# defineZYP/ADT

Measured on AMD Instinct MI355X. Metric: train sequences/sec, SASRec-ADT ml-1m (seq_len=200, d=64, 2 blocks), higher is better.
Workload: dtype bf16; 1 GPU; SASRec-ADT ml-1m shape, 2 blocks d=64 H=2 seq_len=200, global batch 256 (256 sequences on this GPU), dropout 0.5, full train step (fwd+loss+bwd+clip+Adam), ids resident in HBM; global_batch=256, seq_len=200, parallelism=dp1, hip_graph=True, table_gradients=sorted segmented sums, bit-reproducible (ADT_ITEM_SORT=1), world_size=1

## Files before the change

adt_amd/csrc/adt_attn_args.h:

```cpp
#pragma once
#include "adt_common.cuh"

namespace adt {

struct AttnArgs {
  const float* Q; int ldq;
  const float* K; int ldk;
  const float* V; int ldv;
  float* O; int ldo;
  float* LSE;
  int B, H, L;
  int causal;
  float scale;
  DropCfg drop;
  uint32_t bh_offset;
  const float* dO; int lddo;
  float* dQ; int lddq;
  float* dK; int lddk;
  float* dV; int lddv;
  uint32_t* mask;
  unsigned long long* stamps;
  int in_bf16;
  int out_bf16;
};

}
```

adt_amd/csrc/adt_bwdchain_args.h:

```cpp
#pragma once
#include "adt_common.cuh"

namespace adt {

struct BwdChainArgs {
  int T, L, B;
  const int* ids;
  DropCfg drop; uint32_t site1, site2; uint32_t row_offset;
  float ln_eps;
  const float* gy;
  const float* u;
  const float* xin;
  const float* o;
  const float* dqkv; int lddqkv;
  const float* dkv2;
  int grad_bf16;
  const float* dh;
  const float* f;
  const float* W0; const float* W1; const float* W2; const float* W3;
  const float* gamma; const float* beta;
  float* out0; int acc0;
  float* out1; int acc1;
  float* dW0; float* dW1; float* dW2; float* dW3;
  float* db0; float* db1; float* db2; float* db3;
  float* dgamma; float* dbeta;
  const float* rec; const float* drec; const float* Ws; float* dWs; float* dbs; int H;
  int ablate;
  int nrep; size_t rep_stride;
  float gy_scale;
  float* part[4]; size_t part_stride;
  int saved_bf16;
  unsigned long long* stamps;
  const float* wp_base; const void* wp_img;
  float* vpart;
  const float* lnl_x; const float* lnl_gamma; float lnl_eps; float* vpart2; float* lnl_dgamma; float* lnl_dbeta;
  int nsplit;
};

}
```

adt_amd/csrc/adt_sasrec.hip:

```cpp
#include "adt_host.h"
#include <string.h>
#include <mutex>
#include "adt_bwdchain_args.h"
#include "adt_fwdchain_args.h"
#include "adt_seq_args.h"
#include "adt_seqbwd_args.h"

namespace {

constexpr float LN_EPS = 1e-8f;
constexpr int NREPP = 16;
constexpr int LN_PART_BLOCKS = 1024;
constexpr int NREP = 16;

struct Layout {
  int64_t off[4 + 30 * 16];
  int64_t total;
  int nl;
  int64_t item() const { return off[0]; }
  int64_t posw() const { return off[1]; }
  int64_t lnl_w() const { return off[2]; }
  int64_t lnl_b() const { return off[3]; }
  int64_t enc(int i, int k) const { return off[4 + 14 * i + k]; }
  int64_t dec(int i, int k) const { return off[4 + 14 * nl + 16 * i + k]; }
};
enum { E_LN1W, E_LN1B, E_INW, E_INB, E_OW, E_OB, E_LN2W, E_LN2B, E_C1W, E_C1B, E_C2W, E_C2B, E_SW, E_SB };
enum { D_LNW, D_LNB, D_SINW, D_SINB, D_SOW, D_SOB, D_EINW, D_EINB, D_EOW, D_EOB, D_C1W, D_C1B, D_C2W, D_C2B, D_UW, D_UB };

int64_t up64(int64_t x) { return (x + 63) / 64 * 64; }

StepPlan step_plan(const adt_sasrec_cfg* c, int B) {
  const StepFacts f{c->prec, c->maxlen, c->hidden, c->num_heads, c->num_layers, B, c->item_num + 1, adt_item_sort_supported(c->item_num + 1) != 0,
                    c->num_heads > 0 ? adt_seq_attn_bwd_lds(c->maxlen, c->num_heads) : 0};
  return adt_step_plan(f, adt_seq_switches());
}

bool make_layout(const adt_sasrec_cfg* c, Layout* lo) {
  if (c->num_layers < 1 || c->num_layers > 16) return false;
  const int64_t d = c->hidden, H = c->num_heads, hd = d / H, L = c->maxlen, V = c->item_num;
  lo->nl = c->num_layers;
  int64_t o = 0;
  int n = 0;
  auto put = [&](int64_t sz) { lo->off[n++] = o; o += up64(sz); };
  put((V + 1) * d); put(L * d); put(d); put(d);
  for (int i = 0; i < c->num_layers; ++i) {
    put(d); put(d); put(3 * d * d); put(3 * d); put(d * d); put(d); put(d); put(d);
    put(d * d); put(d); put(d * d); put(d); put(H * hd); put(H);
  }
  for (int i = 0; i < c->num_layers; ++i) {
    put(d); put(d);
    put(3 * d * d); put(3 * d); put(d * d); put(d);
    put(3 * d * d); put(3 * d); put(d * d); put(d);
    put(d * d); put(d); put(d * d); put(d); put(d); put(d);
  }
  lo->total = o;
  return true;
}

struct WS {
  int64_t T, d, H, L, nl, B;
  int64_t enc_x, dec_x, f, posl, negl;
  int64_t e_qn, e_qkv, e_o, e_lse, e_h, e_h2, e_u, e_rec, e_mask, e_stride;
  int64_t d_dn, d_qkv, d_o1, d_lse1, d_a1, d_q2, d_kv2, d_o2, d_lse2, d_a2, d_u, d_mask1, d_mask2, d_stride;
  int64_t g_enc_x, g_dec_x, g_f, g_pos, g_neg, g_rec;
  int64_t s1, s2, s3, s4, s5;
  int64_t loss, norms, scal;
  int64_t rep, rep_stride;
  int64_t prep, prep_stride;
  int64_t wpack;
  int64_t part, part_stride;
  int64_t isort, isort_n;
  int64_t vpart, vcall, lnpart, gnpart;
  int64_t total;
};

void make_ws(const adt_sasrec_cfg* c, int B, const StepPlan& pl, WS* w) {
  w->B = B; w->d = c->hidden; w->H = c->num_heads; w->L = c->maxlen; w->nl = c->num_layers;
  w->T = (int64_t)B * w->L;
  const int64_t Td = up64(w->T * w->d), T1 = up64(w->T), lse = up64((int64_t)B * w->H * w->L);
  const int64_t rec = up64(w->T * w->H * w->H);
  int64_t o = 0;
  auto take = [&](int64_t n) { int64_t r = o; o += n; return r; };
  w->enc_x = take((w->nl + 1) * Td); w->dec_x = take((w->nl + 1) * Td); w->f = take(Td);
  w->posl = take(T1); w->negl = take(T1);
  {
    const int64_t s = o;
    w->e_qn = take(Td); w->e_qkv = take(3 * Td); w->e_o = take(Td); w->e_lse = take(lse); w->e_h = take(Td);
    w->e_h2 = take(Td); w->e_u = take(Td); w->e_rec = take(rec); w->e_mask = take(8 * lse);
    w->e_stride = o - s;
    o = s + w->e_stride * w->nl;
  }
  {
    const int64_t s = o;
    w->d_dn = take(Td); w->d_qkv = take(3 * Td); w->d_o1 = take(Td); w->d_lse1 = take(lse); w->d_a1 = take(Td);
    w->d_q2 = take(Td); w->d_kv2 = take(2 * Td); w->d_o2 = take(Td); w->d_lse2 = take(lse); w->d_a2 = take(Td);
    w->d_u = take(Td); w->d_mask1 = take(8 * lse); w->d_mask2 = take(8 * lse);
    w->d_stride = o - s;
    o = s + w->d_stride * w->nl;
  }
  w->g_enc_x = take((w->nl + 1) * Td); w->g_dec_x = take((w->nl + 1) * Td); w->g_f = take(Td);
  w->g_pos = take(T1); w->g_neg = take(T1); w->g_rec = take(rec * w->nl);
  w->s1 = take(Td); w->s2 = take(Td); w->s3 = take(3 * Td); w->s4 = take(2 * Td); w->s5 = take(Td);
  w->loss = take(64 * (2 + 2 * 16)); w->norms = take(64); w->scal = take(192);
  w->rep_stride = up64((int64_t)(c->item_num + 1) * w->d);
  w->rep = take(NREP * w->rep_stride);
  {
    Layout lo;
    make_layout(c, &lo);
    w->prep_stride = up64(lo.total - lo.posw());
    w->prep = take(NREPP * w->prep_stride);
    w->wpack = take(3 * w->prep_stride);
  }
  w->part_stride = pl.parts_area ? (int64_t)w->nl * 16 * 4096 : 0;
  w->part = take((int64_t)B * pl.seq_split * w->part_stride);
  w->isort_n = pl.sort_area ? adt_item_sort_work_ints(4, (int)w->T, c->item_num + 1) : 0;
  w->isort = take(up64(w->isort_n));
  w->vcall = (int64_t)B * pl.seq_split * 512;
  w->vpart = take(w->part_stride > 0 ? (5 * w->nl + 1) * w->vcall : 0);
  w->lnpart = take(LN_PART_BLOCKS * 128);
  w->gnpart = take(4096);
  w->total = o;
}

#define CK(call) do { int _r = (call); if (_r) return _r; } while (0)

struct SideStream {
  hipStream_t s = nullptr;
  hipEvent_t fork_ev[4] = {nullptr, nullptr, nullptr, nullptr}, join_ev[4] = {nullptr, nullptr, nullptr, nullptr};
};
SideStream* side_stream(const StepPlan& pl, hipStream_t main) {
  static SideStream g[16];
  static std::mutex mu;
  if (!pl.side_sites) return nullptr;
  int dev = 0;
  if (hipGetDevice(&dev) != hipSuccess || dev < 0 || dev >= 16) return nullptr;
  SideStream* sd = &g[dev];
  std::lock_guard<std::mutex> lock(mu);
  if (sd->s) return sd;
  hipStreamCaptureStatus cs = hipStreamCaptureStatusNone;
  if (hipStreamIsCapturing(main, &cs) != hipSuccess || cs != hipStreamCaptureStatusNone) { (void)hipGetLastError(); return nullptr; }
  hipStream_t s = nullptr;
  if (hipStreamCreateWithFlags(&s, hipStreamNonBlocking) != hipSuccess) { (void)hipGetLastError(); return nullptr; }
  for (int i = 0; i < 4; ++i)
    if (hipEventCreateWithFlags(&sd->fork_ev[i], hipEventDisableTiming) != hipSuccess ||
        hipEventCreateWithFlags(&sd->join_ev[i], hipEventDisableTiming) != hipSuccess) {
      (void)hipGetLastError();
      (void)hipStreamDestroy(s);
      return nullptr;
    }
  sd->s = s;
  return sd;
}
int side_mark(SideStream* sd, int k, void* main) {
  if (!sd) return 0;
  if (hipEventRecord(sd->fork_ev[k], (hipStream_t)main) != hipSuccess) return adt_set_error("backward: side-stream fork %d failed", k);
  return 0;
}
int side_enter(SideStream* sd, int k, void* main, void** out) {
  *out = main;
  if (!sd) return 0;
  if (hipStreamWaitEvent(sd->s, sd->fork_ev[k], 0) != hipSuccess) return adt_set_error("backward: side-stream fork %d failed", k);
  *out = sd->s;
  return 0;
}
int side_join(SideStream* sd, int k, void* main) {
  if (!sd) return 0;
  if (hipEventRecord(sd->join_ev[k], sd->s) != hipSuccess || hipStreamWaitEvent((hipStream_t)main, sd->join_ev[k], 0) != hipSuccess)
    return adt_set_error("backward: side-stream join %d failed", k);
  return 0;
}

int layout_ws(const adt_sasrec_cfg* c, int B, Layout* lo, WS* w, StepPlan* pl) {
  *pl = step_plan(c, B);
  if (pl->cfg_error[0]) return adt_set_error("%s", pl->cfg_error);
  make_layout(c, lo);
  make_ws(c, B, *pl, w);
  return 0;
}

adt::FwdChainArgs fwd_args(int T, int L, int B, int H, const int32_t* ids, float p, const uint32_t* seed, uint32_t row_offset) {
  adt::FwdChainArgs a;
  memset(&a, 0, sizeof(a));
  a.T = T; a.L = L; a.B = B; a.H = H; a.ids = ids; a.drop = adt_make_drop(p, seed, 0); a.row_offset = row_offset; a.ln_eps = LN_EPS;
  return a;
}

adt::BwdChainArgs bwd_args(int T, int L, int B, const int32_t* ids, float p, const uint32_t* seed, uint32_t row_offset) {
  adt::BwdChainArgs a;
  memset(&a, 0, sizeof(a));
  a.T = T; a.L = L; a.B = B; a.ids = ids; a.drop = adt_make_drop(p, seed, 0); a.row_offset = row_offset; a.ln_eps = LN_EPS;
  return a;
}

int pack_offsets(const adt_sasrec_cfg* c, const Layout& lo, int* offs) {
  if (c->prec != ADT_PREC_BF16) return 0;
  int n = 0;
  const int64_t base = lo.posw();
  const int dd = c->hidden * c->hidden;
  for (int i = 0; i < c->num_layers; ++i) {
    for (int j = 0; j < 3; ++j) offs[n++] = (int)(lo.enc(i, E_INW) + j * dd - base);
    offs[n++] = (int)(lo.enc(i, E_OW) - base); offs[n++] = (int)(lo.enc(i, E_C1W) - base); offs[n++] = (int)(lo.enc(i, E_C2W) - base);
    for (int j = 0; j < 3; ++j) offs[n++] = (int)(lo.dec(i, D_SINW) + j * dd - base);
    for (int j = 0; j < 3; ++j) offs[n++] = (int)(lo.dec(i, D_EINW) + j * dd - base);
// ... 187 lines not shown
SideStream* fwd_logits_stream(const StepPlan& pl, void* st) { return ((pl.side_sites & 1) && !pl.bce_merged) ? side_stream(pl, (hipStream_t)st) : nullptr; }
bool ring_prefetch_split(const adt::RingPrefetchArgs& rr, bool bce_by_forward, const StepPlan& pl) {
  return rr.ring && rr.staging && rr.state && bce_by_forward && pl.embed3_on;
}

struct LossPtrs { const float *A[4], *Bm[4], *rc[4]; float *GA[4], *GB[4], *lm[4], *dr[4], *ln[4]; };
AdtLossSeedsJob loss_terms(const WS& w, float* ws, const float* lambdas1, const float* lambdas2, bool all_seeds, LossPtrs* q) {
  const int nl = (int)w.nl, H = (int)w.H;
  const int64_t Td = up64(w.T * w.d), rec = up64(w.T * w.H * w.H);
  float* loss = ws + w.loss;
  for (int i = 0; i < nl; ++i) {
    q->A[i] = ws + w.enc_x + i * Td; q->Bm[i] = ws + w.dec_x + (nl - i) * Td;
    q->GA[i] = all_seeds ? ws + w.g_enc_x + i * Td : nullptr;
    q->GB[i] = (all_seeds || i == 0) ? ws + w.g_dec_x + (nl - i) * Td : nullptr;
    q->lm[i] = loss + 64 * (2 + i);
    q->rc[i] = ws + i * w.e_stride + w.e_rec; q->dr[i] = ws + w.g_rec + i * rec; q->ln[i] = loss + 64 * (2 + nl + i);
  }
  AdtLossSeedsJob j{};
  j.T = (int)w.T; j.norms = ws + w.norms; j.loss_bce = loss;
  j.nmse = nl; j.A = q->A; j.Bm = q->Bm; j.n = w.T * w.d; j.lambdas = lambdas1; j.GA = q->GA; j.GB = q->GB; j.loss_mse = q->lm;
  j.nnll = H > 1 ? nl : 0; j.rec = q->rc; j.n_rows = (int)w.T; j.H = H; j.lambda2 = lambdas2[nl - 1]; j.drec = q->dr; j.loss_nll = q->ln;
  return j;
}

int forward_loss_lean(const adt_sasrec_cfg* c, const Layout& lo, const WS& w, const StepPlan& pl, const float* P, float* ws, const int32_t* seq, const int32_t* dec,
                      const int32_t* pos, const int32_t* neg, bool bce_side, float p, const uint32_t* seed, uint32_t b_offset, const float* lambdas1,
                      const float* lambdas2, const adt::RingPrefetchArgs& rr, void* st) {
  const int hd = (int)(w.d / w.H), nl = c->num_layers;
  if (!pl.bce_deferred) return 1;
  for (int i = 0; i < nl; ++i) {
    adt::SeqFwdArgs a = enc_layer_seq_args(c, lo, w, pl, P, ws, seq, p, seed, b_offset, i, true, true);
    if (i == nl - 1) { a.lnl_gamma = P + lo.lnl_w(); a.lnl_beta = P + lo.lnl_b(); a.f_out = ws + w.f; }
    CK(adt_launch_seq_enc_fwd(hd, a, st));
  }
  for (int j = 0; j < nl; ++j) CK(dec_layer_seq_fwd(lo, w, pl, P, ws, dec, p, seed, b_offset, j, st));
  LossPtrs q;
  AdtLossSeedsJob job = loss_terms(w, ws, lambdas1, lambdas2, false, &q);
  job.ring = &rr; job.split = ring_prefetch_split(rr, bce_side, pl);
  const adt::LogitsBceArgs lb{ws + w.f, P + lo.item(), pos, neg, ws + w.norms, (int)w.T, ws + w.posl, ws + w.negl, ws + w.g_pos, ws + w.g_neg, ws + w.loss,
                              ws + w.g_f, pl.det ? nullptr : ws + w.rep, NREP, (size_t)w.rep_stride, pl.embed3_on ? 1 : 0};
  const bool merged = bce_side && pl.bce_merged;
  if (merged) job.logits = &lb;
  SideStream* const sd = (bce_side && !merged) ? fwd_logits_stream(pl, st) : nullptr;
  if (bce_side && !merged) CK(side_mark(sd, 0, st));
  CK(adt_loss_seeds_prefetch(job, st));
  if (bce_side && !merged) {
    void* s2 = nullptr;
    CK(side_enter(sd, 0, st, &s2));
    CK(adt_logits_bce_scatter_ex(lb.F, lb.E, pos, neg, lb.norms, lb.T, lb.pos_logits, lb.neg_logits, lb.dpos, lb.dneg, lb.loss, lb.dF, lb.rep, lb.nrep,
                                 w.rep_stride, lb.neg_only, s2));
    if (sd && hipEventRecord(sd->join_ev[0], sd->s) != hipSuccess) return adt_set_error("forward_loss: logits event");
  }
  return 0;
}

int g_time_which = 0, g_time_layer = 0;
hipEvent_t g_time_ev0 = nullptr, g_time_ev1 = nullptr;
inline void time_mark(int which, int layer, bool start, void* st) {
  if (!g_time_ev0 || !g_time_ev1 || g_time_layer != layer) return;
  if (g_time_which == 3 && which == 1 && start) {
    (void)hipEventRecord(g_time_ev0, (hipStream_t)st);
    (void)hipEventRecord(g_time_ev1, (hipStream_t)st);
  } else if (g_time_which == which) {
    (void)hipEventRecord(start ? g_time_ev0 : g_time_ev1, (hipStream_t)st);
  }
}

const char* const NO_FALLBACK = "backward: shape L=%d hd=%d left the per-sequence kernels although the partial-gradient path was chosen";

struct Bwd {
  const adt_sasrec_cfg* c; Layout lo; WS w;
  const float* P; float* G; float* ws;
  const int32_t *seq, *dec, *pos, *neg;
  float p; const uint32_t* seed; uint32_t b_offset, ro;
  void* st;
  BwdPlan plan;
  StepPlan sp;
  BwdCallPlan call;
  adt::RingPrefetchArgs ring;
  int T, d, H, hd, L, prec, nl;
  int64_t Td, recsz;
  float* Gq;
  float *s1, *s3, *s4, *s5, *gf;
  const float* f;
  SideStream *sd, *sd_sort;

  adt::BwdChainArgs BA(const int32_t* ids, float pp, const uint32_t* sdp) const {
    adt::BwdChainArgs a = bwd_args(T, L, (int)w.B, ids, pp, sdp, ro);
    a.nrep = NREPP; a.rep_stride = (size_t)w.prep_stride;
    a.wp_base = P + lo.posw(); a.wp_img = prec == ADT_PREC_BF16 ? (const void*)(ws + w.wpack) : nullptr;
    a.nsplit = sp.seq_split;
    return a;
  }
  float* PART(int layer, int slot) const { return sp.parts ? ws + w.part + (int64_t)(16 * layer + slot) * 4096 : nullptr; }
  float* VPART(int layer, int k) const { return call.late_parts ? ws + w.vpart + (int64_t)(5 * layer + k) * w.vcall : nullptr; }
  int logits_scatter(void* s) const {
    if (plan.bce_here)
      return adt_logits_bce_scatter_ex(f, P + lo.item(), pos, neg, ws + w.norms, T, ws + w.posl, ws + w.negl, ws + w.g_pos, ws + w.g_neg, ws + w.loss,
                                       gf, sp.det ? nullptr : ws + w.rep, NREP, w.rep_stride, call.embed3 ? 1 : 0, s);
    if (sp.det) return adt_logits_bwd_df(P + lo.item(), pos, neg, ws + w.g_pos, ws + w.g_neg, T, d, gf, d, s);
    return adt_logits_bwd_scatter(f, d, P + lo.item(), pos, neg, ws + w.g_pos, ws + w.g_neg, T, d, gf, d, ws + w.rep, NREP, w.rep_stride, s);
  }
  int zero_unless_prezeroed(int64_t at, size_t n, void* s) const {
    return (!plan.prep_zeroed && adt::zero_f32_async(ws + at, n, (hipStream_t)s)) ? adt_set_error("replica zero") : 0;
  }
};

int bwd_init(Bwd& x, const adt_sasrec_cfg* c, const float* P, float* G, float* ws, const int32_t* seq, const int32_t* dec, const int32_t* pos,
             const int32_t* neg, int B, int training, const uint32_t* seed, uint32_t b_offset, int phase, const adt::RingPrefetchArgs& ring, void* st) {
  CK(layout_ws(c, B, &x.lo, &x.w, &x.sp));
  if (const char* err = adt_bwd_plan(phase, x.sp.bce_deferred, &x.plan)) return adt_set_error("%s", err);
  x.call = adt_bwd_call_plan(x.sp, x.plan);
  const WS& w = x.w;
  x.c = c; x.P = P; x.G = G; x.ws = ws; x.seq = seq; x.dec = dec; x.pos = pos; x.neg = neg; x.seed = seed; x.b_offset = b_offset; x.st = st; x.ring = ring;
  x.T = (int)w.T; x.d = (int)w.d; x.H = (int)w.H; x.hd = x.d / x.H; x.L = (int)w.L; x.prec = c->prec; x.nl = c->num_layers;
  x.Td = up64(w.T * w.d); x.recsz = up64(w.T * w.H * w.H);
  x.p = training ? c->dropout : 0.f;
  x.ro = b_offset * (uint32_t)x.L;
  x.s1 = ws + w.s1; x.s3 = ws + w.s3; x.s4 = ws + w.s4; x.s5 = ws + w.s5; x.gf = ws + w.g_f; x.f = ws + w.f;
  x.Gq = ws + w.prep - x.lo.posw();
  x.sd_sort = x.sp.det ? side_stream(x.sp, (hipStream_t)st) : nullptr;
  x.sd = x.call.side ? side_stream(x.sp, (hipStream_t)st) : nullptr;
  return 0;
}

struct LogitsSide {
  enum { DONE, MARKED, ENQUEUED, BY_FORWARD } at = DONE;

  int begin(const Bwd& x) {
    const WS& w = x.w;
    if (x.plan.bce_fwd) {
      at = BY_FORWARD;
    } else if (x.sp.det) {
      CK(x.zero_unless_prezeroed(w.prep, (size_t)NREPP * w.prep_stride, x.st));
      CK(x.logits_scatter(x.st));
    } else if (x.sd && (x.sp.side_sites & 1)) {
      CK(side_mark(x.sd, 0, x.st));
      CK(x.zero_unless_prezeroed(w.prep, (size_t)NREPP * w.prep_stride, x.st));
      at = MARKED;
    } else {
      CK(x.zero_unless_prezeroed(w.rep, (size_t)NREP * w.rep_stride + (size_t)NREPP * w.prep_stride, x.st));
      CK(x.logits_scatter(x.st));
    }
    return 0;
  }
  int after_first_chain_kernel(const Bwd& x) {
    if (at != MARKED) return 0;
    void* s2 = nullptr;
    CK(side_enter(x.sd, 0, x.st, &s2));
    CK(x.zero_unless_prezeroed(x.w.rep, (size_t)NREP * x.w.rep_stride, s2));
    CK(x.logits_scatter(s2));
    at = ENQUEUED;
    return 0;
  }
  int join(const Bwd& x) {
    if (at == ENQUEUED) CK(side_join(x.sd, 0, x.st));
    if (at == BY_FORWARD) {
      SideStream* const sl = fwd_logits_stream(x.sp, x.st);
      if (sl && hipStreamWaitEvent((hipStream_t)x.st, sl->join_ev[0], 0) != hipSuccess) return adt_set_error("backward: logits join");
    }
    at = DONE;
    return 0;
  }
};

int dec_post_bwd(const Bwd& x, int i) {
  const WS& w = x.w; const Layout& lo = x.lo; const float* P = x.P; float* const Gq = x.Gq;
  float* base = x.ws + i * w.d_stride;
  adt::BwdChainArgs a = x.BA(x.dec, x.p, x.seed);
  a.site1 = dec_site(i, 2); a.site2 = dec_site(i, 3);
  a.gy = x.ws + w.g_dec_x + (i + 1) * x.Td; a.u = base + w.d_u; a.xin = base + w.d_a2; a.o = base + w.d_o2; a.saved_bf16 = x.sp.lean;
  a.W0 = P + lo.dec(i, D_C2W); a.W1 = P + lo.dec(i, D_C1W); a.W2 = P + lo.dec(i, D_EOW);
  a.dW0 = Gq + lo.dec(i, D_C2W); a.dW1 = Gq + lo.dec(i, D_C1W); a.dW2 = Gq + lo.dec(i, D_EOW);
  a.db0 = Gq + lo.dec(i, D_C2B); a.db1 = Gq + lo.dec(i, D_C1B); a.db2 = Gq + lo.dec(i, D_EOB);
  a.out0 = x.s1;
  a.part[0] = x.PART(i, PS_D_C2); a.part[1] = x.PART(i, PS_D_C1); a.part[2] = x.PART(i, PS_D_EO); a.part_stride = (size_t)w.part_stride;
  a.vpart = x.VPART(i, 0);
  const int rc = x.sp.use_seq ? adt_launch_seq_post_bwd(x.hd, 0, a, x.st) : 1;
  if (rc < 0) return rc;
  if (rc && x.sp.parts) return adt_set_error(NO_FALLBACK, x.L, x.hd);
  return rc ? adt_launch_bwdchain(x.prec, 1, a, x.st) : 0;
}

int dec_cross_attn_bwd(const Bwd& x, int i) {
  const WS& w = x.w; const int d = x.d, B = (int)w.B;
  float* base = x.ws + i * w.d_stride;
  float *q2 = base + w.d_q2, *kv2 = base + w.d_kv2, *o2 = base + w.d_o2, *lse2 = base + w.d_lse2, *s4 = x.s4;
  const uint32_t* mask2 = reinterpret_cast<const uint32_t*>(base + w.d_mask2);
  if (!x.sp.lean)
    return adt_attn_bwd(x.prec, q2, d, kv2, 2 * d, kv2 + d, 2 * d, o2, d, lse2, x.s1, d, B, x.H, x.L, x.hd, 1, x.p, x.seed, dec_site(i, 1), x.b_offset,
                        x.s5, d, s4, 2 * d, s4 + d, 2 * d, mask2, x.st);
  const uint16_t* kvb = reinterpret_cast<const uint16_t*>(kv2);
  return adt_attn_bwd_saved_bf16(q2, d, kvb, 2 * d, kvb + d, 2 * d, o2, d, lse2, x.s1, d, B, x.H, x.L, x.hd, x.p, x.seed, dec_site(i, 1), x.b_offset,
                                 x.s5, d, s4, 2 * d, x.sp.parts ? s4 + d / 2 : s4 + d, 2 * d, mask2, x.sp.parts ? 1 : 0, x.st);
}

adt::BwdChainArgs dec_mid_seq_args(const Bwd& x, int i) {
  const WS& w = x.w; const Layout& lo = x.lo; const float* P = x.P; float* const Gq = x.Gq;
  const int d = x.d, dd = d * d;
  float* base = x.ws + i * w.d_stride;
  const float* einw = P + lo.dec(i, D_EINW);
  float* geinw = Gq + lo.dec(i, D_EINW);
  float* geinb = Gq + lo.dec(i, D_EINB);
  adt::BwdChainArgs a = x.BA(x.dec, 0.f, nullptr);
  a.dqkv = x.s5; a.lddqkv = d; a.xin = base + w.d_a1; a.o = base + w.d_o1; a.saved_bf16 = x.sp.lean; a.dkv2 = x.s4; a.f = x.f;
  a.grad_bf16 = (x.sp.lean && x.sp.parts) ? 1 : 0;
  a.W0 = einw; a.W1 = P + lo.dec(i, D_SOW); a.W2 = einw + dd; a.W3 = einw + 2 * dd;
  a.dW0 = geinw; a.dW1 = Gq + lo.dec(i, D_SOW); a.dW2 = geinw + dd; a.dW3 = geinw + 2 * dd;
  a.db0 = geinb; a.db1 = Gq + lo.dec(i, D_SOB); a.db2 = geinb + d; a.db3 = geinb + 2 * d;
  a.out0 = x.s1; a.out1 = x.gf; a.acc1 = 1;
  a.part[0] = x.PART(i, PS_D_EIN); a.part[1] = x.PART(i, PS_D_SO); a.part[2] = x.PART(i, PS_D_EIN + 1); a.part[3] = x.PART(i, PS_D_EIN + 2);
  a.part_stride = (size_t)w.part_stride;
  a.vpart = x.VPART(i, 1);
  return a;
}

adt::AttnArgs dec_cross_attn_lean_args(const Bwd& x, int i) {
  const WS& w = x.w; const int d = x.d;
  float* base = x.ws + i * w.d_stride;
  const uint16_t* kvb = reinterpret_cast<const uint16_t*>(base + w.d_kv2);
  return adt_attn_bwd_saved_bf16_args(base + w.d_q2, d, kvb, 2 * d, kvb + d, 2 * d, base + w.d_o2, d, base + w.d_lse2, x.s1, d, (int)w.B, x.H, x.L, x.hd, x.p,
                                      x.seed, dec_site(i, 1), x.b_offset, x.s5, d, x.s4, 2 * d, x.s4 + d / 2, 2 * d,
                                      reinterpret_cast<const uint32_t*>(base + w.d_mask2), 1);
}

int dec_mid_bwd(const Bwd& x, int i) {
  const WS& w = x.w; const Layout& lo = x.lo; const float* P = x.P; float* const Gq = x.Gq;
  const int d = x.d, dd = d * d;
  float* base = x.ws + i * w.d_stride;
  float *o1 = base + w.d_o1, *a1 = base + w.d_a1;
  const float* einw = P + lo.dec(i, D_EINW);
  float* geinw = Gq + lo.dec(i, D_EINW);
  float* geinb = Gq + lo.dec(i, D_EINB);
  if (x.sp.use_seq) {
    const int rc = adt_launch_seq_mid_bwd(x.hd, dec_mid_seq_args(x, i), x.st);
    if (rc <= 0) return rc;
    if (x.sp.parts) return adt_set_error(NO_FALLBACK, x.L, x.hd);
  }
  {
    adt::BwdChainArgs a = x.BA(x.dec, 0.f, nullptr);
    a.dqkv = x.s5; a.lddqkv = d; a.xin = a1; a.o = o1; a.saved_bf16 = x.sp.lean;
    a.W0 = einw; a.W1 = P + lo.dec(i, D_SOW);
    a.dW0 = geinw; a.dW1 = Gq + lo.dec(i, D_SOW); a.db0 = geinb; a.db1 = Gq + lo.dec(i, D_SOB);
    a.out0 = x.s1;
    CK(adt_launch_bwdchain(x.prec, 4, a, x.st));
  }
  adt::BwdChainArgs a = x.BA(x.dec, 0.f, nullptr);
  a.dkv2 = x.s4; a.f = x.f;
  a.W0 = einw + dd; a.W1 = einw + 2 * dd;
  a.dW0 = geinw + dd; a.dW1 = geinw + 2 * dd; a.db0 = geinb + d; a.db1 = geinb + 2 * d;
  a.out0 = x.gf; a.acc0 = 1;
  return adt_launch_bwdchain(x.prec, 5, a, x.st);
}

int attn_block_bwd(const Bwd& x, int i, bool dec) {
  const WS& w = x.w; const Layout& lo = x.lo; const float* P = x.P; float* const Gq = x.Gq; float* const ws = x.ws;
  const int d = x.d, dd = d * d, nl = x.nl;
  const int32_t* ids = dec ? x.dec : x.seq;
  float* gy = ws + (dec ? w.g_dec_x : w.g_enc_x) + (i + 1) * x.Td;
  float* gx = ws + (dec ? w.g_dec_x : w.g_enc_x) + i * x.Td;
  const float* xi = ws + (dec ? w.dec_x : w.enc_x) + i * x.Td;
  float* base = ws + i * (dec ? w.d_stride : w.e_stride);
  float *qkv = base + (dec ? w.d_qkv : w.e_qkv), *o = base + (dec ? w.d_o1 : w.e_o), *lse = base + (dec ? w.d_lse1 : w.e_lse);
  const uint32_t* mask = reinterpret_cast<const uint32_t*>(base + (dec ? w.d_mask1 : w.e_mask));
  const int64_t lnw = dec ? lo.dec(i, D_LNW) : lo.enc(i, E_LN1W), lnb = dec ? lo.dec(i, D_LNB) : lo.enc(i, E_LN1B);
  const int64_t inw = dec ? lo.dec(i, D_SINW) : lo.enc(i, E_INW), inb = dec ? lo.dec(i, D_SINB) : lo.enc(i, E_INB);
  const uint32_t site = dec ? dec_site(i, 0) : enc_site(i, 0);
  const int acc = dec ? (i > 0 ? 1 : 0) : 1;
  if (x.sp.use_seq) {
    adt::SeqBwdArgs a = seq_bwd_args(x.L, (int)w.B, x.H, ids, x.p, x.seed, site, x.b_offset, x.hd);
    a.x = xi; a.gamma = P + lnw; a.beta = P + lnb; a.Win = P + inw; a.bin = P + inb;
    a.dO = x.s1; a.o = o; a.lse = lse; a.mask = mask; a.dres = dec ? gy : x.s5;
    a.gx = gx; a.acc = acc; a.dWin = Gq + inw; a.dbin = Gq + inb; a.dgamma = Gq + lnw; a.dbeta = Gq + lnb;
    if (x.plan.seeds_virtual && dec && i > 0) {
      a.acc = 0; a.seed_other = ws + w.enc_x + (nl - i) * x.Td; a.seed_coef = ws + w.norms + 8 + (nl - i);
    }
    if (x.plan.seeds_virtual && !dec) {
      a.acc = 0; a.seed_other = ws + w.dec_x + (nl - i) * x.Td; a.seed_coef = ws + w.norms + 8 + i;
      if (i > 0) { a.seed_loss = ws + w.loss + 64 * (2 + i); a.seed_norms = ws + w.norms; }
    }
    a.nrep = NREPP; a.rep_stride = (size_t)w.prep_stride; a.wp_base = P + lo.posw(); a.wp_img = ws + w.wpack; a.saved_bf16 = x.sp.lean;
    a.part = x.PART(i, dec ? PS_D_SIN : PS_E_IN); a.part_stride = (size_t)w.part_stride;
    a.vpart = x.VPART(i, dec ? 2 : 4);
    a.nsplit = a.part ? x.sp.attn_split : 1;
    time_mark(dec ? 2 : 1, i, true, x.st);
    const int rc = adt_launch_seq_attn_pre_bwd(x.hd, dec ? 1 : 0, a, x.st);
    time_mark(dec ? 2 : 1, i, false, x.st);
    if (rc <= 0) return rc;
    if (x.sp.lean) return adt_set_error("backward: the lean forward needs the fused attention-block backward (L=%d hd=%d)", x.L, x.hd);
  }
  CK(adt_attn_bwd(x.prec, qkv, 3 * d, qkv + d, 3 * d, qkv + 2 * d, 3 * d, o, d, lse, x.s1, d, (int)w.B, x.H, x.L, x.hd, 1, x.p, x.seed, site, x.b_offset,
                  x.s3, 3 * d, x.s3 + d, 3 * d, x.s3 + 2 * d, 3 * d, mask, x.st));
  adt::BwdChainArgs a = x.BA(ids, 0.f, nullptr);
  a.dqkv = x.s3; a.lddqkv = 3 * d; a.xin = xi;
  if (dec) a.gy = gy; else a.dh = x.s5;
  a.W0 = P + inw; a.W1 = P + inw + dd; a.W2 = P + inw + 2 * dd; a.gamma = P + lnw; a.beta = P + lnb;
  a.dW0 = Gq + inw; a.dW1 = Gq + inw + dd; a.dW2 = Gq + inw + 2 * dd; a.db0 = Gq + inb; a.db1 = Gq + inb + d; a.db2 = Gq + inb + 2 * d;
  a.dgamma = Gq + lnw; a.dbeta = Gq + lnb;
  a.out0 = gx; a.acc0 = acc;
  return adt_launch_bwdchain(x.prec, dec ? 3 : 2, a, x.st);
}

int dec_block_backward(const Bwd& x, int i, LogitsSide& logits) {
  CK(dec_post_bwd(x, i));
  CK(logits.after_first_chain_kernel(x));
  if (x.sp.use_seq && x.sp.lean && x.sp.parts) {
    const adt::AttnArgs at = dec_cross_attn_lean_args(x, i);
    const adt::BwdChainArgs mid = dec_mid_seq_args(x, i);
    if (adt_seq_xattn_mid_covered(x.hd, at, mid)) {
      CK(logits.join(x));
      const int rc = adt_launch_seq_xattn_mid_bwd(x.hd, at, mid, x.st);
      if (rc) return rc < 0 ? rc : adt_set_error("backward: the fused cross-attention + mid launch refused a shape it covers (L=%d hd=%d)", x.L, x.hd);
      return attn_block_bwd(x, i, true);
    }
  }
  CK(dec_cross_attn_bwd(x, i));
  CK(logits.join(x));
  CK(dec_mid_bwd(x, i));
  return attn_block_bwd(x, i, true);
}

struct DecSide {
  enum { NONE, MARKED, ENQUEUED } at = NONE;
  bool parts_done = false;

  int embed(const Bwd& x, void* s) const {
    const WS& w = x.w;
    return adt_embed_bwd_rep(x.dec, x.ws + w.g_dec_x, x.T, x.L, x.d, x.p, x.seed, SITE_EMB_DEC, x.ro, x.G + x.lo.posw(), x.ws + w.rep, NREP, w.rep_stride, s);
  }
  int begin(const Bwd& x) {
    const WS& w = x.w; const Layout& lo = x.lo;
    const int64_t dec_begin = lo.dec(0, 0);
    if (x.plan.phase == 0 && x.sd && (x.sp.side_sites & 2) && !(x.call.embed3 && (x.call.late_parts || !x.sp.parts))) {
      CK(side_mark(x.sd, 1, x.st));
      at = MARKED;
    } else if (x.plan.phase == 0) {
      if (!x.sp.det && !x.call.embed3) CK(embed(x, x.st));
    } else if (x.sp.det) {
      if (x.sp.parts) CK(reduce_partials(x.c, lo, w, x.sp, x.G, x.ws, false, true, x.st));
      CK(adt_replica_reduce(x.G + dec_begin, x.Gq + dec_begin, lo.total - dec_begin, NREPP, w.prep_stride, x.st));
    } else {
      void* s2 = nullptr;
      CK(side_mark(x.sd, 1, x.st));
      if (!x.call.embed3) CK(embed(x, x.st));
      CK(side_enter(x.sd, 1, x.st, &s2));
      if (x.sp.parts) CK(reduce_partials(x.c, lo, w, x.sp, x.G, x.ws, false, true, s2));
      CK(side_join(x.sd, 1, x.st));
      CK(adt_replica_reduce2(x.G + lo.item(), x.ws + w.rep, (int64_t)(x.c->item_num + 1) * x.d, NREP, w.rep_stride, x.G + dec_begin, x.Gq + dec_begin,
                             lo.total - dec_begin, NREPP, w.prep_stride, x.st));
    }
    return 0;
  }
  int enter(const Bwd& x) {
    if (at != MARKED) return 0;
    void* s2 = nullptr;
    CK(side_enter(x.sd, 1, x.st, &s2));
    if (!x.sp.det && !x.call.embed3) CK(embed(x, s2));
    if (x.sp.parts && !x.call.late_parts) { CK(reduce_partials(x.c, x.lo, x.w, x.sp, x.G, x.ws, false, true, s2)); parts_done = true; }
    at = ENQUEUED;
    return 0;
  }
  int join(const Bwd& x, bool covered) {
    if (at == ENQUEUED && !covered) CK(side_join(x.sd, 1, x.st));
    at = NONE;
    return 0;
  }
};

int last_layernorm_bwd(const Bwd& x) {
  const WS& w = x.w; const Layout& lo = x.lo; float* const ws = x.ws;
  const int d = x.d;
  if (x.sp.lnl_fused) return 0;
  if (x.call.late_parts) {
    const int nb = adt_layernorm_bwd_parts(x.gf, d, ws + w.enc_x + x.nl * x.Td, d, x.P + lo.lnl_w(), LN_EPS, x.T, d, ws + w.g_enc_x + x.nl * x.Td, d, 0,
                                           ws + w.lnpart, LN_PART_BLOCKS, x.st);
    return nb < 0 ? nb : 0;
  }
  return adt_layernorm_bwd_rep(x.gf, d, ws + w.enc_x + x.nl * x.Td, d, x.P + lo.lnl_w(), LN_EPS, x.T, d, ws + w.g_enc_x + x.nl * x.Td, d, 0,
                               x.Gq + lo.lnl_w(), x.Gq + lo.lnl_b(), NREPP, w.prep_stride, x.st);
}

int enc_post_bwd(const Bwd& x, int i) {
  const WS& w = x.w; const Layout& lo = x.lo; const float* P = x.P; float* const Gq = x.Gq; float* const ws = x.ws;
  const int H = x.H, nl = x.nl;
  float* base = ws + i * w.e_stride;
  adt::BwdChainArgs a = x.BA(x.seq, x.p, x.seed);
  a.site1 = enc_site(i, 1); a.site2 = enc_site(i, 2);
  a.gy = ws + w.g_enc_x + (i + 1) * x.Td; a.u = base + w.e_u; a.xin = base + w.e_h; a.o = base + w.e_o; a.saved_bf16 = x.sp.lean;
  a.W0 = P + lo.enc(i, E_C2W); a.W1 = P + lo.enc(i, E_C1W); a.W2 = P + lo.enc(i, E_OW);
  a.gamma = P + lo.enc(i, E_LN2W); a.beta = P + lo.enc(i, E_LN2B);
  a.dW0 = Gq + lo.enc(i, E_C2W); a.dW1 = Gq + lo.enc(i, E_C1W); a.dW2 = Gq + lo.enc(i, E_OW);
  a.db0 = Gq + lo.enc(i, E_C2B); a.db1 = Gq + lo.enc(i, E_C1B); a.db2 = Gq + lo.enc(i, E_OB);
  a.dgamma = Gq + lo.enc(i, E_LN2W); a.dbeta = Gq + lo.enc(i, E_LN2B);
  a.out0 = x.s5; a.out1 = x.s1;
  int which = 0;
  if (H > 1 && H <= 4) {
    which = H <= 2 ? 6 : 7;
    a.rec = base + w.e_rec; a.drec = ws + w.g_rec + i * x.recsz; a.Ws = P + lo.enc(i, E_SW); a.dWs = Gq + lo.enc(i, E_SW);
    a.dbs = Gq + lo.enc(i, E_SB); a.H = H;
  }
  a.part[0] = x.PART(i, PS_E_C2); a.part[1] = x.PART(i, PS_E_C1); a.part[2] = x.PART(i, PS_E_O); a.part_stride = (size_t)w.part_stride;
  a.vpart = x.VPART(i, 3);
  if (x.sp.lnl_fused && i == nl - 1) {
    a.gy = x.gf; a.lnl_x = ws + w.enc_x + nl * x.Td; a.lnl_gamma = P + lo.lnl_w(); a.lnl_eps = LN_EPS;
    a.vpart2 = x.call.late_parts ? ws + w.vpart + (int64_t)(5 * nl) * w.vcall : nullptr;
    a.lnl_dgamma = Gq + lo.lnl_w(); a.lnl_dbeta = Gq + lo.lnl_b();
  }
  const int rc = x.sp.use_seq ? adt_launch_seq_post_bwd(x.hd, 1, a, x.st) : 1;
  if (rc < 0) return rc;
  if (rc && x.sp.parts) return adt_set_error(NO_FALLBACK, x.L, x.hd);
  return rc ? adt_launch_bwdchain(x.prec, which, a, x.st) : 0;
}

int enc_block_backward(const Bwd& x, int i, DecSide& dec_side) {
  const WS& w = x.w; const Layout& lo = x.lo;
  CK(enc_post_bwd(x, i));
  if (x.sp.lnl_fused && i == x.nl - 1) CK(dec_side.enter(x));
  if (x.H > 4) {
    float* base = x.ws + i * w.e_stride;
    CK(adt_headcls_bwd(base + w.e_o, x.d, x.P + lo.enc(i, E_SW), base + w.e_rec, x.ws + w.g_rec + i * x.recsz, (int)w.B, x.L, x.H, x.hd, x.s1, x.d,
                       x.G + lo.enc(i, E_SW), x.G + lo.enc(i, E_SB), x.st));
  }
  return attn_block_bwd(x, i, false);
}

int table_gradients(const Bwd& x, DecSide& dec_side) {
  const WS& w = x.w; const Layout& lo = x.lo; float* const ws = x.ws; float* const G = x.G;
  const int phase = x.plan.phase;
  if (phase == 2 && !x.sp.det && adt::zero_f32_async(ws + w.rep, (size_t)NREP * w.rep_stride, (hipStream_t)x.st)) return adt_set_error("replica zero");
  SideStream* const sd2 = ((x.sp.side_sites & 4) && x.sp.parts && !x.call.late_parts) ? x.sd : nullptr;
  CK(dec_side.join(x, sd2 != nullptr));
  void* s2 = nullptr;
  CK(side_mark(sd2, 2, x.st));
  if (x.sp.det) {
    if (x.sd_sort && hipStreamWaitEvent((hipStream_t)x.st, x.sd_sort->join_ev[3], 0) != hipSuccess) return adt_set_error("backward: sort join");
    const uint32_t site4[4] = {SITE_EMB_SEQ, SITE_EMB_DEC, 0u, 0u};
    const int32_t* const ids2[2] = {x.seq, x.dec};
    const float* const dx2[2] = {ws + w.g_enc_x, ws + w.g_dec_x};
    CK(adt_item_segsum_posemb(reinterpret_cast<int32_t*>(ws + w.isort), 4, x.T, x.c->item_num + 1, 0xFu, site4, x.p, x.seed, sqrtf((float)x.d), G + lo.item(),
                              x.plan.prep_zeroed ? 0 : 1, ids2, dx2, site4, 2, (int)w.B, x.L, x.ro, G + lo.posw(), x.st));
  } else if (x.call.embed3) {
    const bool by_forward = phase == 2 ? x.plan.seeds_virtual : x.plan.bce_fwd;
    CK(adt_embed_bwd3_prefetch(x.seq, x.dec, x.pos, ws + w.g_enc_x, ws + w.g_dec_x, x.f, ws + w.g_pos, x.T, x.L, x.p, x.seed, SITE_EMB_SEQ, SITE_EMB_DEC, x.ro,
                               G + lo.posw(), ws + w.rep, NREP, w.rep_stride, ring_prefetch_split(x.ring, by_forward, x.sp) ? &x.ring : nullptr, x.st));
  } else {
    CK(adt_embed_bwd_rep(x.seq, ws + w.g_enc_x, x.T, x.L, x.d, x.p, x.seed, SITE_EMB_SEQ, x.ro, G + lo.posw(), ws + w.rep, NREP, w.rep_stride, x.st));
  }
  CK(side_enter(sd2, 2, x.st, &s2));
  if (x.sp.parts && !x.call.late_parts) CK(reduce_partials(x.c, lo, w, x.sp, G, ws, true, phase == 0 && !dec_side.parts_done, s2));
  CK(side_join(sd2, 2, x.st));
  if (x.plan.defer_fold) return 0;
  return adt_replica_reduce2(G + lo.item(), ws + w.rep, (int64_t)(x.c->item_num + 1) * x.d, x.sp.det ? 0 : NREP, w.rep_stride, G + lo.posw(), x.Gq + lo.posw(),
                             (phase == 0 ? lo.total : lo.dec(0, 0)) - lo.posw(), NREPP, w.prep_stride, x.st);
}

int item_sort_begin(const Bwd& x) {
  const WS& w = x.w; float* const ws = x.ws;
  const int32_t* const ids4[4] = {x.seq, x.dec, x.pos, x.neg};
  const float* const rows4[4] = {ws + w.g_enc_x, ws + w.g_dec_x, x.f, x.f};
  const float* const coef4[4] = {nullptr, nullptr, ws + w.g_pos, ws + w.g_neg};
  const int kind4[4] = {0, 0, 1, 1};
  void* s2 = x.st;
  if (x.sd_sort) { CK(side_mark(x.sd_sort, 3, x.st)); CK(side_enter(x.sd_sort, 3, x.st, &s2)); }
  CK(adt_item_sort(ids4, 4, x.T, x.c->item_num + 1, rows4, coef4, kind4, x.ro, reinterpret_cast<int32_t*>(ws + w.isort), s2));
  if (x.sd_sort && hipEventRecord(x.sd_sort->join_ev[3], x.sd_sort->s) != hipSuccess) return adt_set_error("backward: sort event");
  return 0;
}

int decoder_phase(const Bwd& x, DecSide& dec_side) {
  if (x.w.prep != x.w.rep + NREP * x.w.rep_stride) return adt_set_error("workspace layout: replica areas not adjacent");
  if (x.sp.det) CK(item_sort_begin(x));
  LogitsSide logits;
  CK(logits.begin(x));
  for (int i = x.nl - 1; i >= 0; --i) CK(dec_block_backward(x, i, logits));
  return dec_side.begin(x);
}

int encoder_phase(const Bwd& x, DecSide& dec_side) {
  CK(last_layernorm_bwd(x));
  if (!x.sp.lnl_fused) CK(dec_side.enter(x));
  for (int i = x.nl - 1; i >= 0; --i) CK(enc_block_backward(x, i, dec_side));
  return table_gradients(x, dec_side);
}

}
// ... 442 lines not shown
```

adt_amd/csrc/adt_seq.hip:

```cpp
#include "adt_host.h"
#include <limits.h>
#include <atomic>
#include "adt_seqfwd.cuh"
#include "adt_seqfwd_tt.cuh"
#include "adt_seqattn.cuh"
#include "adt_seqbwd_tt.cuh"
#include "adt_seqpost_tt.cuh"
#include "adt_seqxattn_tt.cuh"

using namespace adt;

template <class Args>
static int seq_launch(const void* fn, size_t smem, AdtLdsOptIn& slot, int grid, const Args* args, hipStream_t s, const char* what, int nwaves = SQ_NW,
                      size_t optin = 0) {
  return adt_launch_lds1(fn, dim3(grid), dim3(nwaves * 64), smem, *args, s, what, slot, optin);
}

__global__ __launch_bounds__(256) void k_pack_wimg(PackArgs a) { pack_wimg_block(a, blockIdx.x); }

extern "C" int adt_pack_wimg(const float* base, void* img, const int* offs, int n, void* stream) {
  if (n < 1 || n > 256) return adt_set_error("pack_wimg: %d blocks", n);
  PackArgs a;
  a.base = base; a.img = reinterpret_cast<__bf16*>(img); a.n = n;
  for (int i = 0; i < n; ++i) a.off[i] = offs[i];
  hipLaunchKernelGGL(k_pack_wimg, dim3(n), dim3(256), 0, (hipStream_t)stream, a);
  return adt_check_launch("pack_wimg");
}

static_assert(ADT_SEQ_MAXLEN == SQ_LP && ADT_SEQ_MAXLEN == SB_R, "adt_step_plan.h restates the image rows of these kernels");

const SeqSwitches& adt_seq_switches() {
  static const SeqSwitches sw = [] {
    SeqSwitches s;
    s.seq = adt_env_on("ADT_SEQ"); s.seq_lean = adt_env_on("ADT_SEQ_LEAN"); s.seq_tt = adt_env_on("ADT_SEQ_TT"); s.seq_bwd = adt_env_on("ADT_SEQ_BWD");
    s.seq_attn_bwd = adt_env_on("ADT_SEQ_ATTN_BWD"); s.seq_post_bwd = adt_env_on("ADT_SEQ_POST_BWD"); s.seq_partials = adt_env_on("ADT_SEQ_PARTIALS");
    s.xattn_fused = adt_env_on("ADT_XATTN_FUSED");
    s.seq_ablate = adt_env_int("ADT_SEQ_ABLATE", 0); s.seq_ablate_set = adt_env_int("ADT_SEQ_ABLATE", INT_MIN) != INT_MIN;
    s.seq_split = adt_env_int("ADT_SEQ_SPLIT", 0); s.attn_split = adt_env_on("ADT_ATTN_SPLIT");
    s.side_stream = adt_env_int("ADT_SIDE_STREAM", 7); s.side_stream_dp = adt_env_int("ADT_SIDE_STREAM_DP", 0) != 0;
    s.item_sort = adt_env_int("ADT_ITEM_SORT", 0) != 0;
    s.lnl_fused = adt_env_on("ADT_LNL_FUSED"); s.fold_parts = adt_env_on("ADT_FOLD_PARTS"); s.fwd_fused = adt_env_on("ADT_FWD_FUSED");
    s.embed3 = adt_env_on("ADT_EMBED3"); s.bce_merged = adt_env_on("ADT_BCE_MERGED");
    return s;
  }();
  return sw;
}

static SeqAttnFacts attn_facts(const AttnArgs& a) {
  return {a.L, a.H, a.B, a.causal != 0, a.in_bf16 != 0, a.out_bf16 != 0, a.ldq, a.ldk, a.ldv, a.ldo, a.lddo, a.drop.thr != 0, a.mask != nullptr,
          sab_lds_bytes(a.L, a.H), xm_lds_bytes(a.L, a.H)};
}
size_t adt_seq_attn_bwd_lds(int L, int H) { return sab_lds_bytes(L, H); }
static SeqChainFacts chain_facts(const BwdChainArgs& a) {
  return {a.L, a.H, a.B, a.T, a.wp_img != nullptr, a.saved_bf16 != 0, a.grad_bf16 != 0, a.part[0] && a.part[1] && a.part[2] && a.part[3], a.nsplit, a.ablate,
          a.drec != nullptr};
}

static unsigned long long* g_stamps = nullptr;

extern "C" int adt_seq_stamps_read(unsigned long long* out, int n) {
  if (!g_stamps) return -1;
  if (hipDeviceSynchronize() != hipSuccess) return -2;
  return hipMemcpy(out, g_stamps, (size_t)n * sizeof(unsigned long long), hipMemcpyDeviceToHost) == hipSuccess ? 0 : -3;
}

static int seq_stamps_mode() {
  static const int st = [] {
    const int v = adt_env_int("ADT_SEQ_STAMPS", 0);
    return (v && hipMalloc(&g_stamps, 16 * 16 * sizeof(unsigned long long)) != hipSuccess) ? 0 : v;
  }();
  return st;
}
static unsigned long long* seq_stamp_buffer(bool for_attention) { return seq_stamps_mode() == (for_attention ? 2 : 1) ? g_stamps : nullptr; }
static unsigned long long* seq_stamp_buffer_post() { return seq_stamps_mode() == 3 ? g_stamps : nullptr; }
static unsigned long long* seq_stamp_buffer_mode(int mode) { return seq_stamps_mode() == mode ? g_stamps : nullptr; }

static void seq_ablate(SeqFwdArgs& a) {
  a.stamps = seq_stamp_buffer(false);
  const int ab = adt_seq_switches().seq_ablate;
  a.ablate = ab;
  if (ab & 1) { a.qkv = nullptr; a.o = nullptr; a.h = nullptr; a.u = nullptr; a.a1 = nullptr; a.q2 = nullptr; a.kv2 = nullptr; a.o2 = nullptr; a.mask = nullptr; a.mask2 = nullptr; }
}

static bool seq_use_tt(const SeqFwdArgs& a) {
  return adt_seq_fwd_tt(adt_seq_switches(), a.wp_img != nullptr, a.L);
}

int adt_launch_seq_enc_fwd(int hd, const SeqFwdArgs& a, void* stream) {
  static AdtLdsOptIn optin[3], optin_tt[3];
  SeqFwdArgs args = a;
  seq_ablate(args);
  hipStream_t s = (hipStream_t)stream;
  if (seq_use_tt(args)) {
    const int nsp = args.nsplit > 1 ? args.nsplit : 1;
    const size_t smem_tt = SeqTtLds<6>::bytes;
    if (hd == 64) return seq_launch((const void*)k_seqtt_enc_fwd<64>, smem_tt, optin_tt[0], a.B * nsp, &args, s, "seqtt_enc_fwd<64>", TQ_FWD_NW);
    if (hd == 32) return seq_launch((const void*)k_seqtt_enc_fwd<32>, smem_tt, optin_tt[1], a.B * nsp, &args, s, "seqtt_enc_fwd<32>", TQ_FWD_NW);
    if (hd == 16) return seq_launch((const void*)k_seqtt_enc_fwd<16>, smem_tt, optin_tt[2], a.B * nsp, &args, s, "seqtt_enc_fwd<16>", TQ_FWD_NW);
  }
  args.nsplit = 0;
  const size_t smem = SeqFwdLds<6>::bytes;
  if (hd == 64) return seq_launch((const void*)k_seq_enc_fwd<64, 2>, smem, optin[0], a.B, &args, s, "seq_enc_fwd<64>");
  if (hd == 32) return seq_launch((const void*)k_seq_enc_fwd<32, 2>, smem, optin[1], a.B, &args, s, "seq_enc_fwd<32>");
  if (hd == 16) return seq_launch((const void*)k_seq_enc_fwd<16, 4>, smem, optin[2], a.B, &args, s, "seq_enc_fwd<16>");
  return adt_set_error("seq_enc_fwd: head size %d", hd);
}

int adt_launch_seq_dec_fwd(int hd, const SeqFwdArgs& a, void* stream) {
  static AdtLdsOptIn optin[3], optin_tt[3];
  SeqFwdArgs args = a;
  seq_ablate(args);
  hipStream_t s = (hipStream_t)stream;
  if (seq_use_tt(args)) {
    const int nsp = args.nsplit > 1 ? args.nsplit : 1;
    const size_t smem_tt = SeqTtLds<5>::bytes;
    if (hd == 64) return seq_launch((const void*)k_seqtt_dec_fwd<64>, smem_tt, optin_tt[0], a.B * nsp, &args, s, "seqtt_dec_fwd<64>", TQ_FWD_NW);
    if (hd == 32) return seq_launch((const void*)k_seqtt_dec_fwd<32>, smem_tt, optin_tt[1], a.B * nsp, &args, s, "seqtt_dec_fwd<32>", TQ_FWD_NW);
    if (hd == 16) return seq_launch((const void*)k_seqtt_dec_fwd<16>, smem_tt, optin_tt[2], a.B * nsp, &args, s, "seqtt_dec_fwd<16>", TQ_FWD_NW);
  }
  args.nsplit = 0;
  const size_t smem = SeqFwdLds<5>::bytes;
  if (hd == 64) return seq_launch((const void*)k_seq_dec_fwd<64>, smem, optin[0], a.B, &args, s, "seq_dec_fwd<64>");
  if (hd == 32) return seq_launch((const void*)k_seq_dec_fwd<32>, smem, optin[1], a.B, &args, s, "seq_dec_fwd<32>");
  if (hd == 16) return seq_launch((const void*)k_seq_dec_fwd<16>, smem, optin[2], a.B, &args, s, "seq_dec_fwd<16>");
  return adt_set_error("seq_dec_fwd: head size %d", hd);
}

int adt_launch_seq_attn_bwd(int hd, const AttnArgs& a, void* stream) {
  if (!adt_covers_attn_bwd(adt_seq_switches(), hd, attn_facts(a))) return 1;
  const size_t smem = sab_lds_bytes(a.L, a.H);
  const int mode = a.drop.thr == 0 ? 0 : (a.mask != nullptr ? 1 : 2);
  static AdtLdsOptIn optin[9];
  const void* fns[9] = {(const void*)k_seq_attn_bwd<64, 0>, (const void*)k_seq_attn_bwd<64, 1>, (const void*)k_seq_attn_bwd<64, 2>,
                        (const void*)k_seq_attn_bwd<32, 0>, (const void*)k_seq_attn_bwd<32, 1>, (const void*)k_seq_attn_bwd<32, 2>,
                        (const void*)k_seq_attn_bwd<16, 0>, (const void*)k_seq_attn_bwd<16, 1>, (const void*)k_seq_attn_bwd<16, 2>};
  const int slot = (hd == 64 ? 0 : hd == 32 ? 3 : 6) + mode;
  AttnArgs args = a;
  args.stamps = seq_stamp_buffer(true);
  if (!args.stamps) args.stamps = seq_stamp_buffer_mode(4);
  return adt_launch_lds1(fns[slot], dim3(a.B), dim3(SAB_NW * 64), smem, args, (hipStream_t)stream, "seq_attn_bwd", optin[slot], ADT_LDS_MAX);
}

template <int HD, bool DEC>
static int seq_attn_pre_bwd_t(int mode, const SeqBwdArgs& a, hipStream_t s) {
  constexpr int H = 64 / HD;
  const size_t smem = SeqBwdLds<H>::bytes;
  static AdtLdsOptIn optin[3];
  const void* fns[3] = {(const void*)k_seqtt_attn_pre_bwd<HD, 0, DEC>, (const void*)k_seqtt_attn_pre_bwd<HD, 1, DEC>,
                        (const void*)k_seqtt_attn_pre_bwd<HD, 2, DEC>};
  SeqBwdArgs args = a;
  args.stamps = seq_stamp_buffer(true);
  if (a.nsplit == 2 && !a.part) return adt_set_error("seqtt_attn_pre_bwd: two workgroups per sequence need the weight-gradient partials");
  if (a.nsplit != 2) args.nsplit = 1;
  return seq_launch(fns[mode], smem, optin[mode], a.B * args.nsplit, &args, s, "seqtt_attn_pre_bwd");
}

int adt_launch_seq_attn_pre_bwd(int hd, int dec, const SeqBwdArgs& a, void* stream) {
  SeqChainFacts f{};
  f.L = a.L; f.H = a.H; f.B = a.B; f.T = a.B * a.L; f.wimg = a.wp_img != nullptr;
  if (!adt_covers_attn_pre_bwd(adt_seq_switches(), hd, f)) return 1;
  const int mode = a.drop.thr == 0 ? 0 : (a.mask != nullptr ? 1 : 2);
  hipStream_t s = (hipStream_t)stream;
  if (hd == 32) return dec ? seq_attn_pre_bwd_t<32, true>(mode, a, s) : seq_attn_pre_bwd_t<32, false>(mode, a, s);
  if (hd == 64) return dec ? seq_attn_pre_bwd_t<64, true>(mode, a, s) : seq_attn_pre_bwd_t<64, false>(mode, a, s);
  return dec ? seq_attn_pre_bwd_t<16, true>(mode, a, s) : seq_attn_pre_bwd_t<16, false>(mode, a, s);
}

int adt_launch_seq_post_bwd(int hd, int enc, const BwdChainArgs& a, void* stream) {
  if (!adt_covers_post_bwd(adt_seq_switches(), hd, enc != 0, chain_facts(a))) return 1;
  static AdtLdsOptIn optin[6];
  const void* fns[6] = {(const void*)k_seqtt_post_bwd<64, false>, (const void*)k_seqtt_post_bwd<64, true>, (const void*)k_seqtt_post_bwd<32, false>,
                        (const void*)k_seqtt_post_bwd<32, true>, (const void*)k_seqtt_post_bwd<16, false>, (const void*)k_seqtt_post_bwd<16, true>};
  const int slot = (hd == 64 ? 0 : hd == 32 ? 2 : 4) + (enc ? 1 : 0);
  BwdChainArgs args = a;
  args.stamps = enc ? seq_stamp_buffer_post() : nullptr;
  return seq_launch(fns[slot], SeqPostLds<3>::bytes, optin[slot], a.B * (a.nsplit > 1 ? a.nsplit : 1), &args, (hipStream_t)stream, "seqtt_post_bwd", SP_NW);
}

int adt_launch_seq_mid_bwd(int hd, const BwdChainArgs& a, void* stream) {
  if (!adt_covers_mid_bwd(adt_seq_switches(), hd, chain_facts(a))) return 1;
  static AdtLdsOptIn optin;
  BwdChainArgs args = a;
  args.stamps = seq_stamp_buffer_mode(5);
  return seq_launch((const void*)k_seqtt_mid_bwd, SeqPostLds<4>::bytes, optin, a.B * (a.nsplit > 1 ? a.nsplit : 1), &args, (hipStream_t)stream, "seqtt_mid_bwd", SP_MID_NW);
}

static std::atomic<unsigned long long> g_xattn_fused_launches{0};
extern "C" unsigned long long adt_seq_xattn_fused_launches() { return g_xattn_fused_launches.load(); }

int adt_seq_xattn_mid_covered(int hd, const AttnArgs& at, const BwdChainArgs& ch) {
  const bool handover = ch.dqkv == at.dQ && ch.lddqkv == at.lddq && at.lddq == 64 && ch.dkv2 == at.dK && at.lddk == 128 && at.lddv == 128 &&
                        reinterpret_cast<const __bf16*>(at.dV) == reinterpret_cast<const __bf16*>(at.dK) + 64;
  return adt_covers_xattn_mid(adt_seq_switches(), hd, attn_facts(at), chain_facts(ch), handover);
}

int adt_launch_seq_xattn_mid_bwd(int hd, const AttnArgs& at, const BwdChainArgs& ch, void* stream) {
  if (!adt_seq_xattn_mid_covered(hd, at, ch)) return 1;
  XattnMidArgs a{};
  a.Q = reinterpret_cast<const __bf16*>(at.Q); a.K = reinterpret_cast<const __bf16*>(at.K); a.V = reinterpret_cast<const __bf16*>(at.V);
  a.O = reinterpret_cast<const __bf16*>(at.O); a.ldq = at.ldq; a.ldk = at.ldk; a.ldv = at.ldv; a.ldo = at.ldo;
  a.LSE = at.LSE; a.dO = at.dO; a.lddo = at.lddo; a.L = at.L; a.mask = at.mask; a.scale = at.scale; a.drop = at.drop;
  a.xin = ch.xin; a.o = ch.o; a.f = ch.f; a.wp_base = ch.wp_base; a.wp_img = ch.wp_img;
  a.W0 = ch.W0; a.W1 = ch.W1; a.W2 = ch.W2; a.W3 = ch.W3;
  a.out0 = ch.out0; a.out1 = ch.out1; a.acc1 = ch.acc1; a.nrep = ch.nrep; a.rep_stride = ch.rep_stride;
  a.db0 = ch.db0; a.db1 = ch.db1; a.db2 = ch.db2; a.db3 = ch.db3; a.vpart = ch.vpart;
  for (int k = 0; k < 4; ++k) a.part[k] = ch.part[k];
  a.part_stride = ch.part_stride;
  a.stamps = seq_stamp_buffer_mode(6);
  const int mode = at.drop.thr == 0 ? 0 : 1;
  static AdtLdsOptIn optin[6];
  const void* fns[6] = {(const void*)k_seqtt_xattn_mid_bwd<64, 0>, (const void*)k_seqtt_xattn_mid_bwd<64, 1>, (const void*)k_seqtt_xattn_mid_bwd<32, 0>,
                        (const void*)k_seqtt_xattn_mid_bwd<32, 1>, (const void*)k_seqtt_xattn_mid_bwd<16, 0>, (const void*)k_seqtt_xattn_mid_bwd<16, 1>};
  const int slot = (hd == 64 ? 0 : hd == 32 ? 2 : 4) + mode;
  const size_t most = xm_lds_bytes(ADT_SEQ_MAXLEN, at.H) <= ADT_LDS_MAX ? xm_lds_bytes(ADT_SEQ_MAXLEN, at.H) : xm_lds_bytes(128, at.H);
  const int rc = seq_launch(fns[slot], xm_lds_bytes(at.L, at.H), optin[slot], at.B, &a, (hipStream_t)stream, "seqtt_xattn_mid_bwd", XM_NW, most);
  if (rc == 0) ++g_xattn_fused_launches;
  return rc;
}

struct PartReduceArgs {
  float* G; const float* part; size_t stride; int nwg; int nslots;
  int slot[256]; int off[256];
  int nwg_slot[256];
};
constexpr int PR_SPLIT = 4;
__global__ __launch_bounds__(256) void k_dwpart_reduce(PartReduceArgs a) {
  typedef unsigned u4v __attribute__((ext_vector_type(4)));
  const int j = blockIdx.x, item = threadIdx.x;
  const int nwg = a.nwg_slot[j];
  const int per = (nwg + PR_SPLIT - 1) / PR_SPLIT, w0 = blockIdx.y * per, w1 = min(nwg, w0 + per);
  const __bf16* p = reinterpret_cast<const __bf16*>(a.part + (size_t)a.slot[j] * 4096) + item * 16;
  const size_t strideb = a.stride * 2;
  float sum[16];
#pragma unroll
  for (int i = 0; i < 16; ++i) sum[i] = 0.f;
  int wg = w0;
  for (; wg + 4 <= w1; wg += 4) {
    u4v lo[4], hi[4];
#pragma unroll
    for (int u = 0; u < 4; ++u) {
      const u4v* src = reinterpret_cast<const u4v*>(p + (size_t)(wg + u) * strideb);
      lo[u] = src[0]; hi[u] = src[1];
    }
#pragma unroll
    for (int u = 0; u < 4; ++u) {
      const unsigned wds[8] = {lo[u].x, lo[u].y, lo[u].z, lo[u].w, hi[u].x, hi[u].y, hi[u].z, hi[u].w};
#pragma unroll
      for (int i = 0; i < 8; ++i) { sum[2 * i] += __uint_as_float(wds[i] << 16); sum[2 * i + 1] += __uint_as_float(wds[i] & 0xFFFF0000u); }
    }
  }
  for (; wg < w1; ++wg) {
    const u4v* src = reinterpret_cast<const u4v*>(p + (size_t)wg * strideb);
    const u4v lo = src[0], hi = src[1];
    const unsigned wds[8] = {lo.x, lo.y, lo.z, lo.w, hi.x, hi.y, hi.z, hi.w};
#pragma unroll
    for (int i = 0; i < 8; ++i) { sum[2 * i] += __uint_as_float(wds[i] << 16); sum[2 * i + 1] += __uint_as_float(wds[i] & 0xFFFF0000u); }
  }
  const int tile = item >> 4, lane0 = (item & 15) * 4;
#pragma unroll
  for (int r = 0; r < 4; ++r) {
    float* dst = a.G + a.off[j] + (16 * (tile >> 2) + 4 * (lane0 >> 4) + r) * 64 + 16 * (tile & 3) + (lane0 & 15);
#pragma unroll
    for (int k = 0; k < 4; ++k) atomicAdd(dst + k, sum[4 * k + r]);
  }
}

int adt_dwpart_reduce(float* G, const float* part, size_t stride, int nwg, const int* slots, const int* offs, int nslots, void* stream) {
  return adt_dwpart_reduce_n(G, part, stride, nwg, nullptr, slots, offs, nslots, stream);
}
int adt_dwpart_reduce_n(float* G, const float* part, size_t stride, int nwg, const int* nwg_slot, const int* slots, const int* offs, int nslots, void* stream) {
  if (nslots < 1 || nslots > 256) return adt_set_error("dwpart_reduce: %d slots", nslots);
  PartReduceArgs a;
  a.G = G; a.part = part; a.stride = stride; a.nwg = nwg; a.nslots = nslots;
  for (int i = 0; i < nslots; ++i) { a.slot[i] = slots[i]; a.off[i] = offs[i]; a.nwg_slot[i] = nwg_slot ? nwg_slot[i] : nwg; }
  hipLaunchKernelGGL(k_dwpart_reduce, dim3(nslots, PR_SPLIT), dim3(256), 0, (hipStream_t)stream, a);
  return adt_check_launch("dwpart_reduce");
}
```

adt_amd/csrc/adt_seqattn.cuh:

```cuda
#pragma once
#include "adt_attn.cuh"
#include "adt_tt.cuh"

namespace adt {

constexpr int SAB_NW = 16;
ADT_DEVICE_INLINE int sab_rank16(int w) {
  const int cl = w & 3, k = w >> 2;
  return 4 * k + ((k & 1) ? 3 - cl : cl);
}

__host__ __device__ inline int sab_rows(int L) { return (L + 31) / 32 * 32; }
__host__ __device__ inline size_t sab_lds_bytes(int L, int H) {
  const size_t R = (size_t)((L + 31) / 32 * 32);
  return 4 * R * TT_RS * 2 + (size_t)H * R * 8 * 4 + 2 * (size_t)H * R * 4;
}

template <int HD>
ADT_DEVICE_INLINE bf16x8 sab_rowfrag(const __bf16* img, int row, int h, int kb, int g) {
  const __bf16* p = img + row * TT_RS + h * HD + 32 * kb + 4 * g;
  const bf16x4 lo = *reinterpret_cast<const bf16x4*>(p);
  bf16x4 hi;
  if constexpr (HD == 16) {
#pragma unroll
// ... 113 lines not shown
  const bf16x8 fp = tt_pack(pv[0], pv[1]), fds = tt_pack(ds[0], ds[1]);
#pragma unroll
  for (int nt = 0; nt < NT; ++nt) {
    dv[nt] = mfma_bf16(dv[nt], tt_trfrag(sdO, qp * 32, h * HD + nt * 16, c, g), fp);
    dk[nt] = mfma_bf16(dk[nt], tt_trfrag(sQ, qp * 32, h * HD + nt * 16, c, g), fds);
  }
}

template <int HD, int MODE>
ADT_DEVICE_INLINE void sab_pass_b(const __bf16* sQ, const __bf16* sdO, const bf16x8* fk, const bf16x8* fv, const float* lse_h, const float* del_h,
                                  const uint32_t* sM_h, int kt, int nqt, int h, const DropCfg& drop, uint32_t key_rng, uint32_t idx_bh, int L,
                                  int c, int g, f32x4 (&dk)[HD / 16], f32x4 (&dv)[HD / 16]) {
  constexpr int NT = HD / 16;
#pragma unroll
  for (int nt = 0; nt < NT; ++nt) {
    dk[nt] = f32x4{0.f, 0.f, 0.f, 0.f};
    dv[nt] = f32x4{0.f, 0.f, 0.f, 0.f};
  }
  const int q0 = kt >> 1;
  sab_pair_b<HD, MODE, true>(sQ, sdO, fk, fv, lse_h, del_h, sM_h, q0, kt, h, drop, key_rng, idx_bh, L, c, g, dk, dv);
#pragma unroll 2
  for (int qp = q0 + 1; 2 * qp < nqt; ++qp) sab_pair_b<HD, MODE, false>(sQ, sdO, fk, fv, lse_h, del_h, sM_h, qp, kt, h, drop, key_rng, idx_bh, L, c, g, dk, dv);
}

template <int HD, int MODE>
ADT_DEVICE_INLINE void sab_pass_b_heads(const __bf16* sQ, const __bf16* sdO, const bf16x8* fk, const bf16x8* fv, const float* sLse, const float* sDelta,
                                        const uint32_t* sM, int R, int kt, int nqt, const DropCfg& drop, uint32_t key_rng, uint32_t bh0, int L,
                                        int c, int g, f32x4 (&dk)[64 / 16], f32x4 (&dv)[64 / 16]) {
  constexpr int H = 64 / HD, NT = HD / 16, KB = (HD + 31) / 32;
#pragma unroll
  for (int i = 0; i < 4; ++i) {
    dk[i] = f32x4{0.f, 0.f, 0.f, 0.f};
    dv[i] = f32x4{0.f, 0.f, 0.f, 0.f};
  }
  const int q0 = kt >> 1;
#pragma unroll
  for (int h = 0; h < H; ++h)
    sab_pair_b<HD, MODE, true>(sQ, sdO, fk + h * KB, fv + h * KB, sLse + h * R, sDelta + h * R, sM + (size_t)h * R * 8, q0, kt, h, drop, key_rng,
                               (bh0 + (uint32_t)h) * (uint32_t)L, L, c, g, *reinterpret_cast<f32x4 (*)[NT]>(&dk[h * NT]), *reinterpret_cast<f32x4 (*)[NT]>(&dv[h * NT]));
#pragma unroll 1
  for (int qp = q0 + 1; 2 * qp < nqt; ++qp) {
#pragma unroll
    for (int h = 0; h < H; ++h)
      sab_pair_b<HD, MODE, false>(sQ, sdO, fk + h * KB, fv + h * KB, sLse + h * R, sDelta + h * R, sM + (size_t)h * R * 8, qp, kt, h, drop, key_rng,
                                  (bh0 + (uint32_t)h) * (uint32_t)L, L, c, g, *reinterpret_cast<f32x4 (*)[NT]>(&dk[h * NT]), *reinterpret_cast<f32x4 (*)[NT]>(&dv[h * NT]));
  }
}

template <int HD, int MODE>
__global__ __launch_bounds__(SAB_NW * 64) void k_seq_attn_bwd(AttnArgs a) {
  adt_prefetch_kernargs<(sizeof(AttnArgs) + 63) / 64 * 64 <= 512 ? sizeof(AttnArgs) : 512>();
  constexpr int H = 64 / HD, NT = HD / 16, KB = (HD + 31) / 32, MAXKT = 14, NW = SAB_NW;
  extern __shared__ __attribute__((aligned(16))) unsigned char smem_raw[];
  const int L = a.L, R = sab_rows(L);
  __bf16* sQ = reinterpret_cast<__bf16*>(smem_raw);
  __bf16* sK = sQ + R * TT_RS;
  __bf16* sV = sK + R * TT_RS;
  __bf16* sdO = sV + R * TT_RS;
  uint32_t* sM = reinterpret_cast<uint32_t*>(sdO + R * TT_RS);
  float* sLse = reinterpret_cast<float*>(sM + (size_t)H * R * 8);
  float* sDelta = sLse + H * R;
  const int b = blockIdx.x;
  const int lane = threadIdx.x & 63, w = threadIdx.x >> 6, c = lane & 15, g = lane >> 4;
  const size_t row_b = (size_t)b * L;
  constexpr bool use_bits = MODE == 1;
  const float qmul = a.scale * 1.4426950408889634f;
#define SAB_STAMP(k) do { if (a.stamps && blockIdx.x == 0 && lane == 0) a.stamps[w * 16 + (k)] = __builtin_amdgcn_s_memtime(); } while (0)
  SAB_STAMP(0);
  if constexpr (MODE == 1) {
    for (int i = threadIdx.x; i < H * R * 2; i += NW * 64) {
      const int hr = i >> 1, h = hr / R, r = hr - h * R;
      uint4 v = make_uint4(0u, 0u, 0u, 0u);
      if (r < L) v = reinterpret_cast<const uint4*>(a.mask + ((size_t)(b * H + h) * L + r) * 8)[i & 1];
      reinterpret_cast<uint4*>(sM + (size_t)hr * 8)[i & 1] = v;
    }
  }
  for (int i = threadIdx.x; i < H * R; i += NW * 64) {
    const int h = i / R, r = i - h * R;
    sLse[i] = r < L ? a.LSE[(size_t)(b * H + h) * L + r] * 1.4426950408889634f : INFINITY;
  }
  for (int i = threadIdx.x; i < R * 8; i += NW * 64) {
    const int r = i >> 3, c8 = (i & 7) * 8;
    float q[8], k[8], v[8], d[8], o[8];
#pragma unroll
    for (int j = 0; j < 8; ++j) q[j] = k[j] = v[j] = d[j] = o[j] = 0.f;
    if (r < L && a.in_bf16) {
      const __bf16* Qb = reinterpret_cast<const __bf16*>(a.Q); const __bf16* Kb = reinterpret_cast<const __bf16*>(a.K);
      const __bf16* Vb = reinterpret_cast<const __bf16*>(a.V); const __bf16* Ob = reinterpret_cast<const __bf16*>(a.O);
      const int pa = 16 * ((c8 >> 2) & 3) + 4 * (c8 >> 4), pb = pa + 16;
      typedef __bf16 bf16x4_t __attribute__((ext_vector_type(4)));
      const bf16x4_t qa = *reinterpret_cast<const bf16x4_t*>(Qb + (row_b + r) * a.ldq + pa), qc = *reinterpret_cast<const bf16x4_t*>(Qb + (row_b + r) * a.ldq + pb);
      const bf16x4_t ka = *reinterpret_cast<const bf16x4_t*>(Kb + (row_b + r) * a.ldk + pa), kc = *reinterpret_cast<const bf16x4_t*>(Kb + (row_b + r) * a.ldk + pb);
      const bf16x4_t va = *reinterpret_cast<const bf16x4_t*>(Vb + (row_b + r) * a.ldv + pa), vc = *reinterpret_cast<const bf16x4_t*>(Vb + (row_b + r) * a.ldv + pb);
      const bf16x4_t oa = *reinterpret_cast<const bf16x4_t*>(Ob + (row_b + r) * a.ldo + pa), oc = *reinterpret_cast<const bf16x4_t*>(Ob + (row_b + r) * a.ldo + pb);
      bf16x8 qb, kb, vb, ob;
#pragma unroll
      for (int j = 0; j < 4; ++j) { qb[j] = qa[j]; qb[4 + j] = qc[j]; kb[j] = ka[j]; kb[4 + j] = kc[j]; vb[j] = va[j]; vb[4 + j] = vc[j]; ob[j] = oa[j]; ob[4 + j] = oc[j]; }
      *reinterpret_cast<float4*>(d) = *reinterpret_cast<const float4*>(a.dO + (row_b + r) * a.lddo + c8);
      *reinterpret_cast<float4*>(d + 4) = *reinterpret_cast<const float4*>(a.dO + (row_b + r) * a.lddo + c8 + 4);
#pragma unroll
      for (int j = 0; j < 8; ++j) { q[j] = (float)qb[j]; k[j] = (float)kb[j]; v[j] = (float)vb[j]; o[j] = (float)ob[j]; }
    } else if (r < L) {
      *reinterpret_cast<float4*>(q) = *reinterpret_cast<const float4*>(a.Q + (row_b + r) * a.ldq + c8);
      *reinterpret_cast<float4*>(q + 4) = *reinterpret_cast<const float4*>(a.Q + (row_b + r) * a.ldq + c8 + 4);
      *reinterpret_cast<float4*>(k) = *reinterpret_cast<const float4*>(a.K + (row_b + r) * a.ldk + c8);
      *reinterpret_cast<float4*>(k + 4) = *reinterpret_cast<const float4*>(a.K + (row_b + r) * a.ldk + c8 + 4);
      *reinterpret_cast<float4*>(v) = *reinterpret_cast<const float4*>(a.V + (row_b + r) * a.ldv + c8);
      *reinterpret_cast<float4*>(v + 4) = *reinterpret_cast<const float4*>(a.V + (row_b + r) * a.ldv + c8 + 4);
      *reinterpret_cast<float4*>(d) = *reinterpret_cast<const float4*>(a.dO + (row_b + r) * a.lddo + c8);
      *reinterpret_cast<float4*>(d + 4) = *reinterpret_cast<const float4*>(a.dO + (row_b + r) * a.lddo + c8 + 4);
      *reinterpret_cast<float4*>(o) = *reinterpret_cast<const float4*>(a.O + (row_b + r) * a.ldo + c8);
      *reinterpret_cast<float4*>(o + 4) = *reinterpret_cast<const float4*>(a.O + (row_b + r) * a.ldo + c8 + 4);
    }
    float part = 0.f;
#pragma unroll
    for (int j = 0; j < 8; ++j) { part += d[j] * o[j]; q[j] *= qmul; d[j] *= a.drop.scale; }
    *reinterpret_cast<bf16x8*>(sQ + r * TT_RS + c8) = pack8(q);
    *reinterpret_cast<bf16x8*>(sK + r * TT_RS + c8) = pack8(k);
    *reinterpret_cast<bf16x8*>(sV + r * TT_RS + c8) = pack8(v);
    *reinterpret_cast<bf16x8*>(sdO + r * TT_RS + c8) = pack8(d);
#pragma unroll
    for (int off = HD / 16; off > 0; off >>= 1) part += __shfl_xor(part, off, 64);
    if (((i & 7) % (HD / 8)) == 0) sDelta[((i & 7) / (HD / 8)) * R + r] = part;
  }
  SAB_STAMP(1);
  __syncthreads();
  SAB_STAMP(2);
  const uint32_t key_rng = drop_key(a.drop);
  const int nqt = (L + 15) / 16;
  const float ln2 = 0.6931471805599453f;

  for (int rnd = 0; rnd * NW < nqt; ++rnd) {
    const int tix = rnd * NW + sab_rank16(w);
    if (tix >= nqt) continue;
    const int qt = nqt - 1 - tix;
    const int q = qt * 16 + c;
    const int nkt = qt + 1;
#pragma unroll 1
    for (int h = 0; h < H; ++h) {
      const float lse_q = sLse[h * R + q], delta_q = sDelta[h * R + q];
      bf16x8 fq[KB], fdo[KB];
#pragma unroll
      for (int kb = 0; kb < KB; ++kb) {
        fq[kb] = sab_rowfrag<HD>(sQ, q, h, kb, g);
        fdo[kb] = sab_rowfrag<HD>(sdO, q, h, kb, g);
      }
      f32x4 dq[NT];
      const uint32_t bh_rng = (uint32_t)(b * H + h) + a.bh_offset;
      const uint32_t idx_q = (bh_rng * (uint32_t)L + (uint32_t)q) * (uint32_t)L;
      sab_pass_a<HD, MODE>(sK, sV, fq, fdo, lse_q, delta_q, sM + ((size_t)h * R + q) * 8, qt, h, a.drop, key_rng, idx_q, c, g, dq);
      if (q < L && a.out_bf16) {
        __bf16* dst = reinterpret_cast<__bf16*>(a.dQ) + (row_b + q) * a.lddq + 16 * g + 4 * h * NT;
#pragma unroll
        for (int nt = 0; nt < NT; ++nt) {
          bf16x4 v;
#pragma unroll
          for (int r = 0; r < 4; ++r) v[r] = (__bf16)(dq[nt][r] * a.scale);
          *reinterpret_cast<bf16x4*>(dst + 4 * nt) = v;
        }
      } else if (q < L) {
#pragma unroll
        for (int nt = 0; nt < NT; ++nt)
          *reinterpret_cast<float4*>(a.dQ + (row_b + q) * a.lddq + h * HD + nt * 16 + 4 * g) =
              make_float4(dq[nt][0] * a.scale, dq[nt][1] * a.scale, dq[nt][2] * a.scale, dq[nt][3] * a.scale);
      }
    }
  }

  SAB_STAMP(3);
  for (int rnd = 0; rnd * NW < nqt; ++rnd) {
    const int kt = rnd * NW + sab_rank16(w);
    if (kt >= nqt) continue;
    const int key = kt * 16 + c;
#pragma unroll 1
    for (int h = 0; h < H; ++h) {
      bf16x8 fk[KB], fv[KB];
#pragma unroll
      for (int kb = 0; kb < KB; ++kb) {
        fk[kb] = sab_rowfrag<HD>(sK, key, h, kb, g);
        fv[kb] = sab_rowfrag<HD>(sV, key, h, kb, g);
      }
      f32x4 dk[NT], dv[NT];
      const uint32_t bh_rng = (uint32_t)(b * H + h) + a.bh_offset;
      sab_pass_b<HD, MODE>(sQ, sdO, fk, fv, sLse + h * R, sDelta + h * R, sM + (size_t)h * R * 8, kt, nqt, h, a.drop, key_rng, bh_rng * (uint32_t)L, L, c,
                           g, dk, dv);
      if (key < L && a.out_bf16) {
        __bf16* dstk = reinterpret_cast<__bf16*>(a.dK) + (row_b + key) * a.lddk + 16 * g + 4 * h * NT;
        __bf16* dstv = reinterpret_cast<__bf16*>(a.dV) + (row_b + key) * a.lddv + 16 * g + 4 * h * NT;
#pragma unroll
        for (int nt = 0; nt < NT; ++nt) {
          bf16x4 vk, vv;
#pragma unroll
          for (int r = 0; r < 4; ++r) { vk[r] = (__bf16)(dk[nt][r] * ln2); vv[r] = (__bf16)dv[nt][r]; }
          *reinterpret_cast<bf16x4*>(dstk + 4 * nt) = vk;
          *reinterpret_cast<bf16x4*>(dstv + 4 * nt) = vv;
        }
      } else if (key < L) {
#pragma unroll
        for (int nt = 0; nt < NT; ++nt) {
          *reinterpret_cast<float4*>(a.dK + (row_b + key) * a.lddk + h * HD + nt * 16 + 4 * g) =
              make_float4(dk[nt][0] * ln2, dk[nt][1] * ln2, dk[nt][2] * ln2, dk[nt][3] * ln2);
          *reinterpret_cast<float4*>(a.dV + (row_b + key) * a.lddv + h * HD + nt * 16 + 4 * g) =
              make_float4(dv[nt][0], dv[nt][1], dv[nt][2], dv[nt][3]);
        }
      }
// ... 7 lines not shown
```

adt_amd/csrc/adt_seqbwd_args.h:

```cpp
#pragma once
#include "adt_common.cuh"

namespace adt {

struct SeqBwdArgs {
  int L, B, H;
  const int* ids;
  DropCfg drop; uint32_t b_offset;
  float ln_eps, scale;
  const float* x;
  const float* gamma; const float* beta;
  const float* Win; const float* bin;
  const float* dO; const float* o;
  const float* lse; const uint32_t* mask;
  float dres_scale;
  const float* dres;
  float* gx; int acc;
  const float* seed_other; const float* seed_coef; float* seed_loss; const float* seed_norms;
  float* dWin; float* dbin; float* dgamma; float* dbeta;
  float* part; size_t part_stride;
  int nrep; size_t rep_stride;
  const float* wp_base; const void* wp_img;
  int saved_bf16;
  float* vpart;
  int nsplit;
  unsigned long long* stamps;
};

}
```

adt_amd/csrc/adt_seqbwd_tt.cuh:

```cuda
#pragma once
#include "adt_seqattn.cuh"
#include "adt_seqbwd_args.h"
#include "adt_seqfwd_tt.cuh"
#include "adt_tt.cuh"

namespace adt {

constexpr int SB_NW = 8;
constexpr int SB_R = 224;

template <int H>
struct SeqBwdLds {
  static constexpr size_t wbytes = 6 * (size_t)TT_WIMG * 2, ibytes = (size_t)SB_R * TT_RS * 2;
  static constexpr size_t mbytes = (size_t)H * SB_R * 8 * 4, sbytes = 2 * (size_t)H * SB_R * 4, rbytes = (320 + 320) * 4;
  static constexpr size_t pbytes = ibytes + 64 > wbytes / 2 ? ibytes + 64 : wbytes / 2;
  static constexpr size_t poff = wbytes / 2 + 2 * ibytes + 64  + mbytes + sbytes + rbytes;
  static constexpr size_t bytes = poff + pbytes;
};

template <int HD>
ADT_DEVICE_INLINE void sb_frags(const TT& t, float mul, bf16x8 (&f)[(64 / HD) * ((HD + 31) / 32)]) {
  if constexpr (HD >= 32) {
    f[0] = tt_pack(t.v[0], t.v[1], mul);
    f[1] = tt_pack(t.v[2], t.v[3], mul);
  } else {
    const f32x4 z = {0.f, 0.f, 0.f, 0.f};
#pragma unroll
    for (int h = 0; h < 4; ++h) f[h] = tt_pack(t.v[h], z, mul);
  }
}

template <int HD>
ADT_DEVICE_INLINE void sb_put_frags(__bf16* img, int token, const bf16x8 (&f)[(64 / HD) * ((HD + 31) / 32)], bool valid, int g) {
  constexpr int NF = (64 / HD) * ((HD + 31) / 32);
#pragma unroll
  for (int i = 0; i < NF; ++i) {
    bf16x4 lo, hi;
#pragma unroll
    for (int j = 0; j < 4; ++j) { lo[j] = valid ? f[i][j] : (__bf16)0.f; hi[j] = valid ? f[i][4 + j] : (__bf16)0.f; }
    if constexpr (HD >= 32) {
      *reinterpret_cast<bf16x4*>(img + token * TT_RS + 32 * i + 4 * g) = lo;
      *reinterpret_cast<bf16x4*>(img + token * TT_RS + 32 * i + 16 + 4 * g) = hi;
    } else {
      *reinterpret_cast<bf16x4*>(img + token * TT_RS + 16 * i + 4 * g) = lo;
    }
  }
}

struct TTLn { TT xhat; float rstd; };
ADT_DEVICE_INLINE TTLn tt_ln_stats(const TT& x, float eps) {
  float s = 0.f;
#pragma unroll
  for (int nt = 0; nt < 4; ++nt) s += (x.v[nt][0] + x.v[nt][1]) + (x.v[nt][2] + x.v[nt][3]);
  const float mu = tt_colsum(s) * (1.0f / 64);
  TTLn o;
  float q = 0.f;
#pragma unroll
  for (int nt = 0; nt < 4; ++nt)
#pragma unroll
    for (int r = 0; r < 4; ++r) { const float t = x.v[nt][r] - mu; o.xhat.v[nt][r] = t; q += t * t; }
  o.rstd = 1.0f / sqrtf(tt_colsum(q) * (1.0f / 64) + eps);
#pragma unroll
  for (int nt = 0; nt < 4; ++nt) o.xhat.v[nt] *= o.rstd;
  return o;
}
ADT_DEVICE_INLINE TT tt_ln_apply(const TT& xhat, const float* gamma, const float* beta, int g) {
  const TTV gm = tt_vec(gamma, g), bt = tt_vec(beta, g);
  TT y;
#pragma unroll
  for (int nt = 0; nt < 4; ++nt)
#pragma unroll
    for (int r = 0; r < 4; ++r) y.v[nt][r] = xhat.v[nt][r] * gm.v[nt][r] + bt.v[nt][r];
  return y;
}
ADT_DEVICE_INLINE TT tt_ln_bwd(const TT& dy, const TTLn& st, const float* gamma, TT& dgm, TT& dbt, int g) {
  const TTV gm = tt_vec(gamma, g);
  TT dx;
  float m1 = 0.f, m2 = 0.f;
#pragma unroll
  for (int nt = 0; nt < 4; ++nt)
#pragma unroll
    for (int r = 0; r < 4; ++r) {
      dgm.v[nt][r] += dy.v[nt][r] * st.xhat.v[nt][r];
      dbt.v[nt][r] += dy.v[nt][r];
      const float dxh = dy.v[nt][r] * gm.v[nt][r];
      dx.v[nt][r] = dxh;
      m1 += dxh;
      m2 += dxh * st.xhat.v[nt][r];
    }
  m1 = tt_colsum(m1) * (1.0f / 64);
  m2 = tt_colsum(m2) * (1.0f / 64);
#pragma unroll
  for (int nt = 0; nt < 4; ++nt)
#pragma unroll
    for (int r = 0; r < 4; ++r) dx.v[nt][r] = st.rstd * (dx.v[nt][r] - m1 - st.xhat.v[nt][r] * m2);
  return dx;
}

template <int NP, int STEP, bool BIAS>
ADT_DEVICE_INLINE void sb_dw_accumulate(const __bf16* sG, const __bf16* sX, int kt, int nt0, bool two, int c, int g, f32x4& acc0, f32x4& acc1, f32x4& b0, f32x4& b1) {
  bf16x8 ones;
#pragma unroll
  for (int j = 0; j < 8; ++j) ones[j] = (__bf16)1.0f;
#pragma unroll
  for (int kp = 0; kp < NP; ++kp) {
    const bf16x8 fx = tt_trfrag(sX, kp * 32, 16 * kt, c, g);
    const bf16x8 g0 = tt_trfrag(sG, kp * 32, 16 * nt0, c, g);
    acc0 = mfma_bf16(acc0, g0, fx);
    if (BIAS) b0 = mfma_bf16(b0, g0, ones);
    if (STEP > 0 && two) {
      const bf16x8 g1 = tt_trfrag(sG, kp * 32, 16 * (nt0 + STEP), c, g);
// ... 70 lines not shown
#pragma unroll
  for (int k = 0; k < N; ++k) {
    uint4* dst = reinterpret_cast<uint4*>(wimg + k * TT_WIMG);
    dst[threadIdx.x] = t.r0[k];
    if (i1 < CH) dst[i1] = t.r1[k];
  }
}

ADT_DEVICE_INLINE int sb_tile_b(int s, int w, int ntiles) {
  if (ntiles != 13) return tq_tile(s, w, ntiles);
  const int t0 = (0x0 << 0) | (0x1 << 4) | (0x2 << 8) | (0x3 << 12) | (0x7 << 16) | (0x5 << 20) | (0x6 << 24) | (0x4 << 28);
  const int t1 = (0xC << 12) | (0x8 << 16) | (0x9 << 20) | (0xA << 24) | (0xB << 28);
  if (s == 0) return (int)(((unsigned)t0 >> (4 * w)) & 15u);
  return w >= 3 ? (int)(((unsigned)t1 >> (4 * w)) & 15u) : -1;
}

#define SB_STAMP(k) do { if (a.stamps && blockIdx.x == 0 && lane == 0) a.stamps[w * 16 + (k)] = __builtin_amdgcn_s_memtime(); } while (0)

template <int HD, int MODE, bool DEC>
__global__ __launch_bounds__(SB_NW * 64) void k_seqtt_attn_pre_bwd(SeqBwdArgs a) {
  adt_prefetch_kernargs<(sizeof(SeqBwdArgs) + 63) / 64 * 64 <= 512 ? sizeof(SeqBwdArgs) : 512>();
  constexpr int H = 64 / HD, NT = HD / 16, KB = (HD + 31) / 32, NF = H * KB, NW = SB_NW, R = SB_R;
  extern __shared__ __attribute__((aligned(16))) unsigned char smem_raw[];
  typedef SeqBwdLds<H> Lds;
  __bf16* wtr = reinterpret_cast<__bf16*>(smem_raw);
  __bf16* wpl = reinterpret_cast<__bf16*>(smem_raw + Lds::poff);
  __bf16* img2 = wpl;
  __bf16* img0 = reinterpret_cast<__bf16*>(smem_raw + Lds::wbytes / 2);
  __bf16* img1 = reinterpret_cast<__bf16*>(smem_raw + Lds::wbytes / 2 + Lds::ibytes);
  uint32_t* sM = reinterpret_cast<uint32_t*>(smem_raw + Lds::wbytes / 2 + 2 * Lds::ibytes + 64);
  float* sLse = reinterpret_cast<float*>(reinterpret_cast<unsigned char*>(sM) + Lds::mbytes);
  float* sDelta = sLse + H * R;
  float* sRed = sDelta + H * R;
  float* sVec = sRed + 320;
  const float *vgamma = sVec, *vbeta = sVec + 64, *vbin = sVec + 128;
  const int lane = threadIdx.x & 63, w = threadIdx.x >> 6, c = lane & 15, g = lane >> 4;
  const int L = a.L, ntiles = (L + 15) / 16, npair = (L + 31) / 32;
  const bool split = a.nsplit == 2;
  const int b = split ? blockIdx.x >> 1 : blockIdx.x, wpart = split ? (blockIdx.x & 1) : 0;
  auto TM = [&](int s) {
    if (!split) return tq_tile(s, w, ntiles);
    const int t = (s == 0 ? wpart : 1 - wpart) + 2 * w;
    return t < ntiles ? t : -1;
  };
  auto TA = [&](int s) { return (split && s == 1) ? -1 : TM(s); };
  auto TB = [&](int s) { return split ? TA(s) : sb_tile_b(s, w, ntiles); };
  if (a.nrep > 1) {
    const size_t off = (size_t)(blockIdx.x % a.nrep) * a.rep_stride;
    a.dWin += off; a.dbin += off; a.dgamma += off; a.dbeta += off;
  }
  float* const part = a.part ? a.part + (size_t)blockIdx.x * a.part_stride : nullptr;
  SB_STAMP(0);
  constexpr int MI = (H * R * 2 + NW * 64 - 1) / (NW * 64), LI = (H * R + NW * 64 - 1) / (NW * 64);
  tt_u4 mreg[MI];
  float lreg[LI];
  typedef const tt_u4 __attribute__((address_space(1))) * gu4;
  typedef const float __attribute__((address_space(1))) * gf1;
  if constexpr (MODE == 1) {
    adt_static_for<MI>([&](auto k) {
      const int i = threadIdx.x + k * NW * 64, hr = i >> 1, h = hr / R, r = hr - h * R;
      const bool ok = i < H * R * 2 && r < L;
      const gu4 p = ok ? (gu4)(a.mask + ((size_t)(b * H + h) * L + r) * 8) + (i & 1) : (gu4)tt_zero_row;
      mreg[k] = *p;
    });
  }
  adt_static_for<LI>([&](auto k) {
    const int i = threadIdx.x + k * NW * 64, h = i / R, r = i - h * R;
    const bool ok = i < H * R && r < L;
    const float v = *(ok ? (gf1)(a.lse + (size_t)(b * H + h) * L + r) : (gf1)tt_zero_row);
    lreg[k] = ok ? v * 1.4426950408889634f : INFINITY;
  });
  float vreg = 0.f;
  {
    const int t = threadIdx.x;
    const gf1 p = t < 64 ? (gf1)(a.gamma + t) : t < 128 ? (gf1)(a.beta + (t - 64)) : t < 320 ? (gf1)(a.bin + (t - 128)) : (gf1)tt_zero_row;
    vreg = *p;
  }
  const __bf16* wsrc = reinterpret_cast<const __bf16*>(a.wp_img) + 6 * (a.Win - a.wp_base);
  const __bf16* const src6[6] = {wsrc + 2 * WPACK_IMG, wsrc + 6 * 4096 + 2 * WPACK_IMG, wsrc + 12 * 4096 + 2 * WPACK_IMG,
                                 wsrc + 3 * WPACK_IMG, wsrc + 6 * 4096 + 3 * WPACK_IMG, wsrc + 12 * 4096 + 3 * WPACK_IMG};
#pragma unroll
  for (int k = 0; k < 3; ++k) adt_glds_block<NW>(src6[k], wpl + k * TT_WIMG, TT_WIMG * 2);
  TT xa[2], doa[2], oa[2];
  int idv[2] = {1, 1};
#pragma unroll
  for (int s = 0; s < 2; ++s) {
    const int tile = TM(s);
    const int l = tile * 16 + c, row = b * L + l;
    xa[s] = tt_load(a.x + (size_t)row * 64, tile >= 0 && l < L, g);
    if (DEC) idv[s] = tt_load_id(a.ids, row, tile >= 0 && l < L);
  }
  SB_STAMP(11);
  {
    uint4* z = reinterpret_cast<uint4*>(img0);
    for (int i = threadIdx.x; i < (int)((2 * Lds::ibytes + 64) / 16); i += NW * 64) z[i] = make_uint4(0u, 0u, 0u, 0u);
    if (threadIdx.x < 320) sRed[threadIdx.x] = 0.f;
    SB_STAMP(12);
    if constexpr (MODE == 1) {
      adt_static_for<MI>([&](auto k) {
        const int i = threadIdx.x + k * NW * 64;
        if (i < H * R * 2) reinterpret_cast<tt_u4*>(sM + (size_t)(i >> 1) * 8)[i & 1] = mreg[k];
      });
    }
    adt_static_for<LI>([&](auto k) {
      const int i = threadIdx.x + k * NW * 64;
      if (i < H * R) { sLse[i] = lreg[k]; sDelta[i] = 0.f; }
    });
    if (threadIdx.x < 320) sVec[threadIdx.x] = vreg;
    SB_STAMP(13);
    adt_wait_vm0();
    SB_STAMP(14);
  }
  __syncthreads();
  SB_STAMP(1);
#pragma unroll
  for (int s = 0; s < 2; ++s) {
    const int tile = TM(s);
    const int l = tile * 16 + c, row = b * L + l;
    const bool valid = tile >= 0 && l < L;
    doa[s] = tt_load(a.dO + (size_t)row * 64, valid, g);
    oa[s] = tt_load_saved(a.o, row, valid, g, a.saved_bf16);
  }
#pragma unroll
  for (int k = 3; k < 6; ++k) adt_glds_block<NW>(src6[k], wtr + (k - 3) * TT_WIMG, TT_WIMG * 2);
  const float qmul = a.scale * 1.4426950408889634f;
  const uint32_t key_rng = drop_key(a.drop);
  bf16x8 fq[2][NF], fdo[2][NF];
  float delta[2][H];
#pragma unroll
  for (int s = 0; s < 2; ++s) {
    const int tile = TM(s);
    if (tile < 0) continue;
    const int l = tile * 16 + c;
    const bool valid = l < L;
    const TT& x = xa[s];
    const TT xn = tt_ln_apply(tt_ln_stats(x, a.ln_eps).xhat, vgamma, vbeta, g);
    const TTB bn = tt_bfrags(xn);
    TTB bx;
    if (!DEC) bx = tt_bfrags(x);
    TT q = tt_gemm(bn, wpl, c, g);
    tt_add_vec(q, vbin, g);
    sb_frags<HD>(q, qmul, fq[s]);
    TT k = tt_gemm(DEC ? bn : bx, wpl + TT_WIMG, c, g);
    tt_add_vec(k, vbin + 64, g);
    tt_put_rows(img0, l, k, valid, g);
    TT v = tt_gemm(DEC ? bn : bx, wpl + 2 * TT_WIMG, c, g);
    tt_add_vec(v, vbin + 128, g);
    tt_put_rows(img1, l, v, valid, g);
    const TT& dO = doa[s];
    const TT& o = oa[s];
    sb_frags<HD>(dO, a.drop.scale, fdo[s]);
#pragma unroll
    for (int h = 0; h < H; ++h) {
      float part = 0.f;
#pragma unroll
      for (int nt = 0; nt < NT; ++nt)
#pragma unroll
        for (int r = 0; r < 4; ++r) part += dO.v[h * NT + nt][r] * o.v[h * NT + nt][r];
      delta[s][h] = tt_colsum(part);
      if (g == 0 && valid) sDelta[h * R + l] = delta[s][h];
    }
  }
  __syncthreads();
  SB_STAMP(2);
  {
    uint4* z = reinterpret_cast<uint4*>(img2);
    for (int i = threadIdx.x; i < (int)((Lds::ibytes + 64) / 16); i += NW * 64) z[i] = make_uint4(0u, 0u, 0u, 0u);
  }
  TT dq[2], dk[2], dv[2];
  dq[1] = tt_zero();
#pragma unroll
  for (int s = 0; s < 2; ++s) {
    const int tile = TA(s);
    if (tile < 0) continue;
    const int q = tile * 16 + c;
#pragma unroll
    for (int h = 0; h < H; ++h) {
      f32x4 t[NT];
      const uint32_t bh_rng = (uint32_t)(b * H + h) + a.b_offset * (uint32_t)H;
      sab_pass_a<HD, MODE>(img0, img1, fq[s] + h * KB, fdo[s] + h * KB, sLse[h * R + q], delta[s][h], sM + ((size_t)h * R + q) * 8, tile, h, a.drop,
                           key_rng, (bh_rng * (uint32_t)L + (uint32_t)q) * (uint32_t)L, c, g, t);
#pragma unroll
      for (int nt = 0; nt < NT; ++nt) dq[s].v[h * NT + nt] = t[nt] * a.scale;
    }
  }
  bf16x8 fk[2][NF], fv[2][NF];
#pragma unroll
  for (int s = 0; s < 2; ++s) {
    const int tile = TB(s);
    const int row = (tile >= 0 ? tile : 0) * 16 + c;
#pragma unroll
    for (int h = 0; h < H; ++h)
#pragma unroll
      for (int kb = 0; kb < KB; ++kb) {
        fk[s][h * KB + kb] = sab_rowfrag<HD>(img0, row, h, kb, g);
        fv[s][h * KB + kb] = sab_rowfrag<HD>(img1, row, h, kb, g);
      }
  }
  adt_wait_vm0();
  __syncthreads();
  SB_STAMP(3);
#pragma unroll
  for (int s = 0; s < 2; ++s) {
    const int tile = TM(s);
    if (tile < 0) continue;
    const int l = tile * 16 + c;
    sb_put_frags<HD>(img0, l, fq[s], l < L, g);
    sb_put_frags<HD>(img1, l, fdo[s], l < L, g);
  }
  __syncthreads();
  TT xk[2];
#pragma unroll
  for (int s = 0; s < 2; ++s) {
    if (s == 1) {
#pragma unroll
      for (int s2 = 0; s2 < 2; ++s2) {
        const int tile2 = TM(s2);
        const int l2 = tile2 * 16 + c;
        xk[s2] = tt_load(a.x + (size_t)(b * L + l2) * 64, tile2 >= 0 && l2 < L, g);
      }
    }
    const int tile = TB(s);
    if (tile < 0) continue;
    {
      f32x4 tk[4], tv[4];
      sab_pass_b_heads<HD, MODE>(img0, img1, fk[s], fv[s], sLse, sDelta, sM, R, tile, ntiles, a.drop, key_rng,
                                 (uint32_t)(b * H) + a.b_offset * (uint32_t)H, L, c, g, tk, tv);
#pragma unroll
      for (int i = 0; i < 4; ++i) {
        dk[s].v[i] = tk[i] * 0.6931471805599453f;
        dv[s].v[i] = tv[i];
      }
    }
  }
  __syncthreads();
  SB_STAMP(4);
  {
#pragma unroll
    for (int s = 0; s < 2; ++s) {
      const int tile = TM(s);
      if (tile < 0) continue;
      const int l = tile * 16 + c;
      const bool valid = l < L;
      tt_put_rows(img0, l, dq[s], valid, g);
// ... 137 lines not shown
```

adt_amd/csrc/adt_seqpost_tt.cuh:

```cuda
#pragma once
#include "adt_bwdchain_args.h"
#include "adt_seqbwd_tt.cuh"

namespace adt {

template <int NWT>
struct SeqPostLds {
  static constexpr size_t wbytes = (size_t)NWT * TT_WIMG * 2, ibytes = (size_t)SB_R * TT_RS * 2;
  static constexpr size_t rbytes = (448 + 256) * 4;
  static constexpr int wvrow = 384;
  static constexpr size_t wvbytes = 8 * wvrow * 4;
  static constexpr size_t bytes = wbytes + 2 * ibytes + 64 + rbytes + wvbytes;
};

ADT_DEVICE_INLINE void sp_replica(BwdChainArgs& a) {
  if (a.nrep <= 1) return;
  const size_t off = (size_t)(blockIdx.x % a.nrep) * a.rep_stride;
  float** const ptrs[] = {&a.dW0, &a.dW1, &a.dW2, &a.dW3, &a.db0, &a.db1, &a.db2, &a.db3, &a.dgamma, &a.dbeta, &a.dWs, &a.dbs, &a.lnl_dgamma, &a.lnl_dbeta};
#pragma unroll
  for (int i = 0; i < 14; ++i)
    if (*ptrs[i]) *ptrs[i] += off;
}

template <int N, int NW>
ADT_DEVICE_INLINE void sp_wdma(const BwdChainArgs& a, const float* const (&W)[N], __bf16* wimg) {
#pragma unroll
  for (int j = 0; j < N; ++j)
    adt_glds_block<NW>(reinterpret_cast<const __bf16*>(a.wp_img) + 6 * (W[j] - a.wp_base) + 3 * WPACK_IMG, wimg + j * TT_WIMG, TT_WIMG * 2);
}
template <int NW>
ADT_DEVICE_INLINE void sp_zero_images(__bf16* img0) {
  constexpr size_t ibytes = (size_t)SB_R * TT_RS * 2;
  uint4* z = reinterpret_cast<uint4*>(img0);
  for (int i = threadIdx.x; i < (int)((2 * ibytes + 64) / 16); i += NW * 64) z[i] = make_uint4(0u, 0u, 0u, 0u);
}
constexpr int SP_NW = 8;
constexpr int SP_NS = (14 + SP_NW - 1) / SP_NW;

template <int HD, bool ENC>
__global__ __launch_bounds__(SP_NW * 64) void k_seqtt_post_bwd(BwdChainArgs a) {
  adt_prefetch_kernargs<(sizeof(BwdChainArgs) + 63) / 64 * 64 <= 512 ? sizeof(BwdChainArgs) : 512>();
  constexpr int H = 64 / HD, NT = HD / 16, NW = SP_NW, NS = SP_NS;
  typedef SeqPostLds<3> Lds;
  extern __shared__ __attribute__((aligned(16))) unsigned char smem_raw[];
  __bf16* wimg = reinterpret_cast<__bf16*>(smem_raw);
  __bf16* img0 = reinterpret_cast<__bf16*>(smem_raw + Lds::wbytes);
  __bf16* img1 = reinterpret_cast<__bf16*>(smem_raw + Lds::wbytes + Lds::ibytes);
  float* sRed = reinterpret_cast<float*>(smem_raw + Lds::wbytes + 2 * Lds::ibytes + 64);
  float* sVec = sRed + 448;
  float* sWave = sVec + 256;
  constexpr int WVR = Lds::wvrow;
  const float *vgamma = sVec, *vbeta = sVec + 64, *vws = sVec + 128, *vgl = sVec + 192;
  const bool lnl = ENC && a.lnl_x != nullptr;
  const int lane = threadIdx.x & 63, w = threadIdx.x >> 6, c = lane & 15, g = lane >> 4;
  const int nsp = a.nsplit > 1 ? a.nsplit : 1, b = blockIdx.x / nsp, part = blockIdx.x % nsp;
  const int L = a.L, ntiles = (L + 15) / 16, npair = (L + 31) / 32;
  auto tileof = [&](int s) { const int t = tq_tile(s, w, ntiles, NW); return (t >= 0 && t % nsp == part) ? t : -1; };
  const bool cls = ENC && H > 1 && a.drec != nullptr;
  sp_replica(a);
  SB_STAMP(0);
  const float* const ws3[3] = {a.W0, a.W1, a.W2};
  sp_wdma<3, NW>(a, ws3, wimg);
  TT dy[NS], xl[NS];
  TTSaved uraw[NS], hreq[NS];
  int idv[NS];
#pragma unroll
  for (int s = 0; s < NS; ++s) {
    const int tile = tileof(s);
    const int l = tile * 16 + c, row = b * L + l;
    const bool valid = tile >= 0 && l < L;
    dy[s] = tt_load(a.gy + (size_t)row * 64, valid, g);
    if (ENC) xl[s] = tt_load(a.lnl_x + (size_t)row * 64, valid && lnl, g);
    uraw[s] = tt_saved_request(a.u, row, valid, g, a.saved_bf16);
    hreq[s] = tt_saved_request(a.xin, row, valid, g, a.saved_bf16);
    idv[s] = tt_load_id(a.ids, row, valid);
  }
  if (a.gy_scale != 0.f) {
#pragma unroll
    for (int s = 0; s < NS; ++s)
#pragma unroll
      for (int nt = 0; nt < 4; ++nt) dy[s].v[nt] *= a.gy_scale;
  }
  {
    sp_zero_images<NW>(img0);
    if (threadIdx.x < 448) sRed[threadIdx.x] = 0.f;
    if (ENC) { tt_stage_vec<NW * 64>(sVec, a.gamma, 64); tt_stage_vec<NW * 64>(sVec + 64, a.beta, 64); }
    if (cls) tt_stage_vec<NW * 64>(sVec + 128, a.Ws, 64);
    if (lnl) tt_stage_vec<NW * 64>(sVec + 192, a.lnl_gamma, 64);
    adt_wait_vm0();
  }
  const uint32_t seedv = a.drop.thr ? *a.drop.seed : 0u;
  const uint32_t key1 = adt_site_key(seedv, a.site1), key2 = adt_site_key(seedv, a.site2);
  SB_STAMP(1);
  __syncthreads();
  SB_STAMP(2);
  TT dt[NS];
  if (ENC) {
    if (lnl) {
      TT dgl = tt_zero(), dbl = tt_zero();
#pragma unroll
      for (int s = 0; s < NS; ++s) {
        if (tileof(s) < 0) continue;
        dy[s] = tt_ln_bwd(dy[s], tt_ln_stats(xl[s], a.lnl_eps), vgl, dgl, dbl, g);
      }
      float* mine = sWave + w * WVR + 256;
#pragma unroll
      for (int nt = 0; nt < 4; ++nt)
#pragma unroll
        for (int r = 0; r < 4; ++r) {
          const float sg = tt_rowsum16(dgl.v[nt][r]), sb = tt_rowsum16(dbl.v[nt][r]);
          if (c == 0) { mine[16 * nt + 4 * g + r] = sg; mine[64 + 16 * nt + 4 * g + r] = sb; }
        }
    }
  }
#pragma unroll
  for (int s = 0; s < NS; ++s) {
    const int tile = tileof(s);
// ... 37 lines not shown
    const int l = tile * 16 + c, row = b * L + l;
    const bool valid = l < L;
    oreq[s] = tt_saved_request(a.o, row, valid, g, a.saved_bf16);
    if constexpr (H == 2) {
      if (cls) {
        typedef const f32x4 __attribute__((address_space(1))) * gf4;
        const size_t off = (size_t)(l * a.B + b) * (H * H);
        drq[s] = *(valid ? (gf4)(a.drec + off) : (gf4)tt_zero_row);
        rcq[s] = *(valid ? (gf4)(a.rec + off) : (gf4)tt_zero_row);
      }
    }
    const TT hraw_s = tt_saved_value(hreq[s], a.saved_bf16);
    tt_put_rows(img0, l, dt[s], valid, g);
    TT d = tt_gemm(tt_bfrags(dt[s]), wimg + TT_WIMG, c, g);
    tt_add(d, dy[s]);
    if (ENC) {
      const TTLn st = tt_ln_stats(hraw_s, a.ln_eps);
      tt_put_rows(img1, l, tt_ln_apply(st.xhat, vgamma, vbeta, g), valid, g);
      dh[s] = tt_ln_bwd(d, st, vgamma, dgm, dbt, g);
      tt_store(a.out0 + (size_t)row * 64, dh[s], valid, g);
    } else {
      tt_put_rows(img1, l, hraw_s, valid, g);
      dh[s] = d;
    }
  }
  SB_STAMP(9);
  __syncthreads();
  sb_dw_product16<NW>(img0, img1, npair, a.dW1, a.part[1] ? a.part[1] + (size_t)blockIdx.x * a.part_stride : nullptr, sRed + 320, w, c, g);
  SB_STAMP(10);
  __syncthreads();
  SB_STAMP(11);
  float dws[H][NT][4], dbs_acc[H];
#pragma unroll
  for (int cc = 0; cc < H; ++cc) {
    dbs_acc[cc] = 0.f;
#pragma unroll
    for (int nt = 0; nt < NT; ++nt)
#pragma unroll
      for (int r = 0; r < 4; ++r) dws[cc][nt][r] = 0.f;
  }
#pragma unroll
  for (int s = 0; s < NS; ++s) {
    const int tile = tileof(s);
    if (tile < 0) continue;
    const int l = tile * 16 + c, row = b * L + l;
    const bool valid = l < L;
    const TT oraw_s = tt_saved_value(oreq[s], a.saved_bf16);
    tt_put_rows(img0, l, dh[s], valid, g);
    tt_put_rows(img1, l, oraw_s, valid, g);
    TT dO = tt_gemm(tt_bfrags(dh[s]), wimg + 2 * TT_WIMG, c, g);
    if (cls) {
      const size_t off = (size_t)(l * a.B + b) * (H * H);
#pragma unroll
      for (int h = 0; h < H; ++h) {
        float dz[H], rcv[H], sd = 0.f;
        if constexpr (H == 2) {
          const float dr4[4] = {drq[s][0], drq[s][1], drq[s][2], drq[s][3]}, rc4[4] = {rcq[s][0], rcq[s][1], rcq[s][2], rcq[s][3]};
#pragma unroll
          for (int cc = 0; cc < H; ++cc) { dz[cc] = valid ? dr4[h * H + cc] : 0.f; rcv[cc] = rc4[h * H + cc]; sd += dz[cc]; }
        } else {
#pragma unroll
          for (int cc = 0; cc < H; ++cc) { dz[cc] = valid ? a.drec[off + h * H + cc] : 0.f; rcv[cc] = valid ? a.rec[off + h * H + cc] : 0.f; sd += dz[cc]; }
        }
#pragma unroll
        for (int cc = 0; cc < H; ++cc) {
          dz[cc] -= valid ? __expf(rcv[cc]) * sd : 0.f;
          if (g == 0) dbs_acc[cc] += dz[cc];
        }
#pragma unroll
        for (int nt = 0; nt < NT; ++nt) {
#pragma unroll
          for (int cc = 0; cc < H; ++cc) {
            const float4 wv = *reinterpret_cast<const float4*>(vws + cc * HD + 16 * nt + 4 * g);
            const f32x4 wq = {wv.x, wv.y, wv.z, wv.w};
#pragma unroll
            for (int r = 0; r < 4; ++r) {
              dO.v[h * NT + nt][r] += dz[cc] * wq[r];
              dws[cc][nt][r] += dz[cc] * oraw_s.v[h * NT + nt][r];
            }
          }
        }
      }
    }
    tt_store((ENC ? a.out1 : a.out0) + (size_t)row * 64, dO, valid, g);
  }
  SB_STAMP(12);
  __syncthreads();
  sb_dw_product16<NW>(img0, img1, npair, a.dW2, a.part[2] ? a.part[2] + (size_t)blockIdx.x * a.part_stride : nullptr, sRed + 384, w, c, g);
  SB_STAMP(13);
  if (ENC) {
    float* mine = sWave + w * WVR;
#pragma unroll
    for (int nt = 0; nt < 4; ++nt)
#pragma unroll
      for (int r = 0; r < 4; ++r) {
        const float sg = tt_rowsum16(dgm.v[nt][r]), sb = tt_rowsum16(dbt.v[nt][r]);
        if (c == 0) { mine[16 * nt + 4 * g + r] = sg; mine[64 + 16 * nt + 4 * g + r] = sb; }
      }
    if (cls) {
#pragma unroll
      for (int cc = 0; cc < H; ++cc) {
#pragma unroll
        for (int nt = 0; nt < NT; ++nt)
#pragma unroll
          for (int r = 0; r < 4; ++r) {
            const float sw = tt_rowsum16(dws[cc][nt][r]);
            if (c == 0) mine[128 + cc * HD + 16 * nt + 4 * g + r] = sw;
          }
        const float sb = tt_rowsum16(dbs_acc[cc]);
        if (c == 0 && g == 0) mine[192 + cc] = sb;
      }
    }
  }
  __syncthreads();
  {
    const int t = threadIdx.x;
    if (ENC && t < 196) {
      float sum = 0.f;
#pragma unroll
      for (int k = 0; k < NW; ++k) sum += sWave[k * WVR + t];
      sRed[t] = sum;
    }
    if (ENC) {
      if (lnl && t >= 256 && t < 384) {
        float sum = 0.f;
#pragma unroll
        for (int k = 0; k < NW; ++k) sum += sWave[k * WVR + t];
        if (a.vpart2) a.vpart2[(size_t)blockIdx.x * 512 + (t - 256)] = sum;
        else atomicAdd((t < 320 ? a.lnl_dgamma : a.lnl_dbeta - 64) + (t - 256), sum);
      }
    }
    const bool live = t < 128 ? ENC : (t < 192 + H ? cls : (t >= 256 && t < 448));
    if (a.vpart) {
      if (t < 448) a.vpart[(size_t)blockIdx.x * 512 + t] = live ? sRed[t] : 0.f;
    } else if (live) {
      float* dst = t < 64 ? a.dgamma + t : t < 128 ? a.dbeta + t - 64 : t < 192 ? a.dWs + t - 128 : t < 256 ? a.dbs + t - 192
                 : t < 320 ? a.db0 + t - 256 : t < 384 ? a.db1 + t - 320 : a.db2 + t - 384;
      atomicAdd(dst, sRed[t]);
    }
  }
  SB_STAMP(14);
}

constexpr int SP_MID_NW = 8;
__global__ __launch_bounds__(SP_MID_NW * 64) void k_seqtt_mid_bwd(BwdChainArgs a) {
  adt_prefetch_kernargs<(sizeof(BwdChainArgs) + 63) / 64 * 64 <= 512 ? sizeof(BwdChainArgs) : 512>();
  constexpr int NW = SP_MID_NW, NS = (14 + NW - 1) / NW;
  typedef SeqPostLds<4> Lds;
  extern __shared__ __attribute__((aligned(16))) unsigned char smem_raw[];
  __bf16* wimg = reinterpret_cast<__bf16*>(smem_raw);
  __bf16* img0 = reinterpret_cast<__bf16*>(smem_raw + Lds::wbytes);
  __bf16* img1 = reinterpret_cast<__bf16*>(smem_raw + Lds::wbytes + Lds::ibytes);
  float* sRed = reinterpret_cast<float*>(smem_raw + Lds::wbytes + 2 * Lds::ibytes + 64);
  const int lane = threadIdx.x & 63, w = threadIdx.x >> 6, c = lane & 15, g = lane >> 4;
  const int nsp = a.nsplit > 1 ? a.nsplit : 1, b = blockIdx.x / nsp, part = blockIdx.x % nsp;
  const int L = a.L, ntiles = (L + 15) / 16, npair = (L + 31) / 32;
  auto tileof = [&](int s) { const int t = tq_tile(s, w, ntiles, NW); return (t >= 0 && t % nsp == part) ? t : -1; };
  sp_replica(a);
  SB_STAMP(0);
  const float* const ws4[4] = {a.W0, a.W1, a.W2, a.W3};
  sp_wdma<4, NW>(a, ws4, wimg);
  TT dqa[NS];
  TTSaved a1req[NS], oreq[NS];
#pragma unroll
  for (int s = 0; s < NS; ++s) {
    const int tile = tileof(s);
    const int l = tile * 16 + c, row = b * L + l;
    const bool valid = tile >= 0 && l < L;
    dqa[s] = a.grad_bf16 ? tt_load_bf16(reinterpret_cast<const __bf16*>(a.dqkv) + (size_t)row * a.lddqkv, valid, g) : tt_load(a.dqkv + (size_t)row * a.lddqkv, valid, g);
    a1req[s] = tt_saved_request(a.xin, row, valid, g, a.saved_bf16);
    oreq[s] = tt_saved_request(a.o, row, valid, g, a.saved_bf16);
  }
  SB_STAMP(1);
  sp_zero_images<NW>(img0);
  if (threadIdx.x < 256) sRed[threadIdx.x] = 0.f;
  adt_wait_vm0();
  SB_STAMP(2);
  __syncthreads();
  SB_STAMP(3);
  TT da1[NS];
#pragma unroll
  for (int s = 0; s < NS; ++s) {
    const int tile = tileof(s);
    if (tile < 0) continue;
    const int l = tile * 16 + c;
    const bool valid = l < L;
    tt_put_rows(img0, l, dqa[s], valid, g);
    tt_put_rows(img1, l, tt_saved_value(a1req[s], a.saved_bf16), valid, g);
    da1[s] = tt_gemm(tt_bfrags(dqa[s]), wimg, c, g);
  }
  __syncthreads();
  sb_dw_product16<NW>(img0, img1, npair, a.dW0, a.part[0] ? a.part[0] + (size_t)blockIdx.x * a.part_stride : nullptr, sRed, w, c, g);
  __syncthreads();
  SB_STAMP(4);
  TT dk[NS], fx[NS];
#pragma unroll
  for (int s = 0; s < NS; ++s) {
    const int tile = tileof(s);
    if (tile < 0) continue;
    const int l = tile * 16 + c, row = b * L + l;
    const bool valid = l < L;
    dk[s] = a.grad_bf16 ? tt_load_bf16(reinterpret_cast<const __bf16*>(a.dkv2) + (size_t)row * 128, valid, g) : tt_load(a.dkv2 + (size_t)row * 128, valid, g);
    fx[s] = tt_load(a.f + (size_t)row * 64, valid, g);
    tt_put_rows(img0, l, da1[s], valid, g);
    tt_put_rows(img1, l, tt_saved_value(oreq[s], a.saved_bf16), valid, g);
    tt_store(a.out0 + (size_t)row * 64, tt_gemm(tt_bfrags(da1[s]), wimg + TT_WIMG, c, g), valid, g);
  }
  __syncthreads();
  sb_dw_product16<NW>(img0, img1, npair, a.dW1, a.part[1] ? a.part[1] + (size_t)blockIdx.x * a.part_stride : nullptr, sRed + 64, w, c, g);
  __syncthreads();
  SB_STAMP(5);
  TT df[NS], dv[NS], acc1v[NS];
#pragma unroll
  for (int s = 0; s < NS; ++s) {
    const int tile = tileof(s);
    if (tile < 0) continue;
    const int l = tile * 16 + c, row = b * L + l;
    const bool valid = l < L;
    dv[s] = a.grad_bf16 ? tt_load_bf16(reinterpret_cast<const __bf16*>(a.dkv2) + (size_t)row * 128 + 64, valid, g) : tt_load(a.dkv2 + (size_t)row * 128 + 64, valid, g);
    acc1v[s] = tt_load(a.out1 + (size_t)row * 64, valid && a.acc1, g);
    tt_put_rows(img0, l, dk[s], valid, g);
    tt_put_rows(img1, l, fx[s], valid, g);
    df[s] = tt_gemm(tt_bfrags(dk[s]), wimg + 2 * TT_WIMG, c, g);
  }
  __syncthreads();
  sb_dw_product16<NW>(img0, img1, npair, a.dW2, a.part[2] ? a.part[2] + (size_t)blockIdx.x * a.part_stride : nullptr, sRed + 128, w, c, g);
  __syncthreads();
  SB_STAMP(6);
#pragma unroll
  for (int s = 0; s < NS; ++s) {
    const int tile = tileof(s);
    if (tile < 0) continue;
    const int l = tile * 16 + c, row = b * L + l;
    const bool valid = l < L;
    tt_put_rows(img0, l, dv[s], valid, g);
    tt_add(df[s], tt_gemm(tt_bfrags(dv[s]), wimg + 3 * TT_WIMG, c, g));
    float* dst = a.out1 + (size_t)row * 64;
    tt_add(df[s], acc1v[s]);
    tt_store(dst, df[s], valid, g);
  }
  __syncthreads();
  sb_dw_product16<NW>(img0, img1, npair, a.dW3, a.part[3] ? a.part[3] + (size_t)blockIdx.x * a.part_stride : nullptr, sRed + 192, w, c, g);
  __syncthreads();
  SB_STAMP(7);
  {
    const int t = threadIdx.x;
    float* const dst[4] = {a.db0, a.db1, a.db2, a.db3};
    if (t < 256) {
      if (a.vpart) a.vpart[(size_t)blockIdx.x * 512 + t] = sRed[t];
      else atomicAdd(dst[t >> 6] + (t & 63), sRed[t]);
    }
  }
  SB_STAMP(8);
}

}
```

adt_amd/csrc/adt_seqxattn_tt.cuh:

```cuda
#pragma once
#include "adt_seqattn.cuh"
#include "adt_seqpost_tt.cuh"

namespace adt {

constexpr int XM_NW = 16;

struct XattnMidArgs {
  const __bf16* Q; const __bf16* K; const __bf16* V; const __bf16* O; int ldq, ldk, ldv, ldo;
  const float* LSE; const float* dO; int lddo; int L;
  const uint32_t* mask; float scale; DropCfg drop;
  const float* xin; const float* o; const float* f; const float* wp_base; const void* wp_img;
  const float* W0; const float* W1; const float* W2; const float* W3;
  float* out0; float* out1; int acc1; int nrep; size_t rep_stride;
  float* db0; float* db1; float* db2; float* db3; float* vpart;
  float* part[4]; size_t part_stride;
  unsigned long long* stamps;
};

__host__ __device__ inline int xm_rows(int L) { return (L + 31) / 32 <= 4 ? 128 : SB_R; }
__host__ __device__ inline size_t xm_lds_bytes(int L, int H) {
  const size_t R = (size_t)xm_rows(L);
  return 4 * R * TT_RS * 2 + (size_t)H * R * 8 * 4 + 2 * (size_t)H * R * 4 + 256 * 4;
}

ADT_DEVICE_INLINE TTB xm_zero() {
  TTB t;
#pragma unroll
  for (int kb = 0; kb < 2; ++kb)
#pragma unroll
    for (int j = 0; j < 8; ++j) t.kb[kb][j] = (__bf16)0.f;
  return t;
}
ADT_DEVICE_INLINE void xm_put_rows(__bf16* img, int token, const TTB& t) {
#pragma unroll
  for (int nt = 0; nt < 4; ++nt) {
    bf16x4 v;
#pragma unroll
    for (int r = 0; r < 4; ++r) v[r] = t.kb[nt >> 1][4 * (nt & 1) + r];
    *reinterpret_cast<bf16x4*>(img + token * TT_RS + 16 * nt + 4 * (int)((threadIdx.x & 63) >> 4)) = v;
  }
}

template <int HD, int MODE>
__global__ __launch_bounds__(XM_NW * 64) void k_seqtt_xattn_mid_bwd(XattnMidArgs a) {
  static_assert(sizeof(XattnMidArgs) <= 512, "kernel-argument prefetch covers 512 bytes");
  static_assert(MODE == 0 || MODE == 1, "no dropout, or keep bits saved by the forward");
  adt_prefetch_kernargs<sizeof(XattnMidArgs)>();
  constexpr int H = 64 / HD, NT = HD / 16, KB = (HD + 31) / 32, NF = H * KB, NW = XM_NW;
  extern __shared__ __attribute__((aligned(16))) unsigned char smem_raw[];
  const int L = a.L, R = xm_rows(L);
  __bf16* sK = reinterpret_cast<__bf16*>(smem_raw);
  __bf16* sV = sK + R * TT_RS;
  __bf16* sQ = sV + R * TT_RS;
  __bf16* sdO = sQ + R * TT_RS;
  uint32_t* sM = reinterpret_cast<uint32_t*>(sdO + R * TT_RS);
  float* sLse = reinterpret_cast<float*>(sM + (size_t)H * R * 8);
  float* sDelta = sLse + H * R;
  float* sRed = sDelta + H * R;
  __bf16* wimg = sK;
  __bf16* img0 = sQ;
  __bf16* img1 = sdO;
  const int b = blockIdx.x;
  const int lane = threadIdx.x & 63, w = threadIdx.x >> 6, c = lane & 15, g = lane >> 4;
  const size_t row_b = (size_t)b * L;
  const float qmul = a.scale * 1.4426950408889634f;
  const int nqt = (L + 15) / 16, npair = (L + 31) / 32;
#define XM_STAMP(k) do { if (a.stamps && blockIdx.x == 0 && lane == 0) a.stamps[w * 16 + (k)] = __builtin_amdgcn_s_memtime(); } while (0)
  XM_STAMP(0);
  if (a.nrep > 1) {
    const size_t off = (size_t)(blockIdx.x % a.nrep) * a.rep_stride;
    if (a.db0) a.db0 += off;
    if (a.db1) a.db1 += off;
    if (a.db2) a.db2 += off;
    if (a.db3) a.db3 += off;
  }
  constexpr int NTH = NW * 64;
  constexpr int MI = (H * SB_R * 2 + NTH - 1) / NTH, LI = (H * SB_R + NTH - 1) / NTH, II = (SB_R * 8 + NTH - 1) / NTH;
  typedef const tt_u4 __attribute__((address_space(1))) * gu4;
  typedef const float __attribute__((address_space(1))) * gf1;
  typedef const bf16x4 __attribute__((address_space(1))) * gb4;
  typedef const f32x4 __attribute__((address_space(1))) * gp4;
  tt_u4 mreg[MI];
  float lreg[LI];
  if constexpr (MODE == 1) {
    adt_static_for<MI>([&](auto k) {
      const int i = threadIdx.x + k * NTH, hr = i >> 1, h = hr / R, r = hr - h * R;
      const bool ok = i < H * R * 2 && r < L;
      const gu4 p = ok ? (gu4)(a.mask + ((size_t)(b * H + h) * L + r) * 8) + (i & 1) : (gu4)tt_zero_row;
      mreg[k] = *p;
    });
  }
  adt_static_for<LI>([&](auto k) {
    const int i = threadIdx.x + k * NTH, h = i / R, r = i - h * R;
    const bool ok = i < H * R && r < L;
    const float v = *(ok ? (gf1)(a.LSE + (size_t)(b * H + h) * L + r) : (gf1)tt_zero_row);
    lreg[k] = ok ? v * 1.4426950408889634f : INFINITY;
  });
  bf16x4 qa[II], qc[II], ka[II], kc[II], va[II], vc[II], oa[II], oc[II];
  f32x4 d0[II], d1[II];
  adt_static_for<II>([&](auto k) {
    const int i = threadIdx.x + k * NTH, r = i >> 3, c8 = (i & 7) * 8;
    const bool ok = r < L;
    const int pa = 16 * ((c8 >> 2) & 3) + 4 * (c8 >> 4);
    const size_t row = row_b + r;
    const gb4 zb = (gb4)tt_zero_row + (i & 7);
    const gb4 pq = ok ? (gb4)(a.Q + row * a.ldq + pa) : zb, pk = ok ? (gb4)(a.K + row * a.ldk + pa) : zb;
    const gb4 pv = ok ? (gb4)(a.V + row * a.ldv + pa) : zb, po = ok ? (gb4)(a.O + row * a.ldo + pa) : zb;
    const gp4 pd = ok ? (gp4)(a.dO + row * a.lddo + c8) : (gp4)tt_zero_row + (i & 7);
    qa[k] = pq[0]; qc[k] = pq[4]; ka[k] = pk[0]; kc[k] = pk[4]; va[k] = pv[0]; vc[k] = pv[4]; oa[k] = po[0]; oc[k] = po[4];
    d0[k] = pd[0]; d1[k] = pd[1];
  });
  XM_STAMP(1);
  if constexpr (MODE == 1) {
    adt_static_for<MI>([&](auto k) {
      const int i = threadIdx.x + k * NTH;
      if (i < H * R * 2) reinterpret_cast<tt_u4*>(sM + (size_t)(i >> 1) * 8)[i & 1] = mreg[k];
    });
  }
  adt_static_for<LI>([&](auto k) {
    const int i = threadIdx.x + k * NTH;
    if (i < H * R) sLse[i] = lreg[k];
  });
  if (threadIdx.x < 256) sRed[threadIdx.x] = 0.f;
  adt_static_for<II>([&](auto k) {
    const int i = threadIdx.x + k * NTH, r = i >> 3, c8 = (i & 7) * 8;
    float q[8], kk[8], v[8], d[8], o[8];
#pragma unroll
    for (int j = 0; j < 4; ++j) {
      q[j] = (float)qa[k][j]; q[4 + j] = (float)qc[k][j]; kk[j] = (float)ka[k][j]; kk[4 + j] = (float)kc[k][j];
      v[j] = (float)va[k][j]; v[4 + j] = (float)vc[k][j]; o[j] = (float)oa[k][j]; o[4 + j] = (float)oc[k][j];
      d[j] = d0[k][j]; d[4 + j] = d1[k][j];
    }
    float part = 0.f;
#pragma unroll
    for (int j = 0; j < 8; ++j) { part += d[j] * o[j]; q[j] *= qmul; d[j] *= a.drop.scale; }
    const bool in = i < R * 8;
    if (in) {
      *reinterpret_cast<bf16x8*>(sQ + r * TT_RS + c8) = pack8(q);
      *reinterpret_cast<bf16x8*>(sK + r * TT_RS + c8) = pack8(kk);
      *reinterpret_cast<bf16x8*>(sV + r * TT_RS + c8) = pack8(v);
      *reinterpret_cast<bf16x8*>(sdO + r * TT_RS + c8) = pack8(d);
    }
#pragma unroll
    for (int off = HD / 16; off > 0; off >>= 1) part += __shfl_xor(part, off, 64);
    if (in && ((i & 7) % (HD / 8)) == 0) sDelta[((i & 7) / (HD / 8)) * R + r] = part;
  });
  XM_STAMP(2);
  __syncthreads();
  XM_STAMP(3);
  const uint32_t key_rng = 0u;
  const float ln2 = 0.6931471805599453f;
  const int rk = sab_rank16(w);
  const bool has = rk < nqt;
  const int qt = has ? nqt - 1 - rk : 0, kt = has ? rk : 0;
  const int lA = qt * 16 + c, lB = kt * 16 + c;
  const bool validA = has && lA < L, validB = has && lB < L;
  const size_t rowA = row_b + lA, rowB = row_b + lB;

  TTB dq = xm_zero();
  bf16x4 fkl[NF], fkh[NF], fvl[NF], fvh[NF];
  if (has) {
#pragma unroll
    for (int h = 0; h < H; ++h) {
      const float lse_q = sLse[h * R + lA], delta_q = sDelta[h * R + lA];
      bf16x8 fq[KB], fdo[KB];
#pragma unroll
      for (int kb = 0; kb < KB; ++kb) {
        fq[kb] = sab_rowfrag<HD>(sQ, lA, h, kb, g);
        fdo[kb] = sab_rowfrag<HD>(sdO, lA, h, kb, g);
      }
      f32x4 t[NT];
      sab_pass_a<HD, MODE>(sK, sV, fq, fdo, lse_q, delta_q, sM + ((size_t)h * R + lA) * 8, qt, h, a.drop, key_rng, 0u, c, g, t);
#pragma unroll
      for (int nt = 0; nt < NT; ++nt)
#pragma unroll
        for (int r = 0; r < 4; ++r) dq.kb[(h * NT + nt) >> 1][4 * ((h * NT + nt) & 1) + r] = (__bf16)(validA ? t[nt][r] * a.scale : 0.f);
    }
#pragma unroll
    for (int h = 0; h < H; ++h)
#pragma unroll
      for (int kb = 0; kb < KB; ++kb) {
        const bf16x8 k8 = sab_rowfrag<HD>(sK, lB, h, kb, g), v8 = sab_rowfrag<HD>(sV, lB, h, kb, g);
#pragma unroll
        for (int j = 0; j < 4; ++j) { fkl[h * KB + kb][j] = k8[j]; fkh[h * KB + kb][j] = k8[4 + j]; fvl[h * KB + kb][j] = v8[j]; fvh[h * KB + kb][j] = v8[4 + j]; }
      }
  }
  XM_STAMP(4);
  __syncthreads();
  XM_STAMP(5);
  {
    const float* const ws4[4] = {a.W0, a.W1, a.W2, a.W3};
#pragma unroll
    for (int j = 0; j < 4; ++j)
      adt_glds_block<NW>(reinterpret_cast<const __bf16*>(a.wp_img) + 6 * (ws4[j] - a.wp_base) + 3 * WPACK_IMG, wimg + j * TT_WIMG, TT_WIMG * 2);
  }
  TTSaved a1req;
  if constexpr (HD != 16) a1req = tt_saved_request(a.xin, rowA, validA, g, 1);

  TTB dk = xm_zero(), dv = xm_zero();
  if (has) {
#pragma unroll
    for (int h = 0; h < H; ++h) {
      f32x4 tk[NT], tv[NT];
      bf16x8 fk[KB], fv[KB];
#pragma unroll
      for (int kb = 0; kb < KB; ++kb)
#pragma unroll
        for (int j = 0; j < 4; ++j) {
          fk[kb][j] = fkl[h * KB + kb][j]; fk[kb][4 + j] = HD == 16 ? (__bf16)0.f : fkh[h * KB + kb][j];
          fv[kb][j] = fvl[h * KB + kb][j]; fv[kb][4 + j] = HD == 16 ? (__bf16)0.f : fvh[h * KB + kb][j];
        }
      sab_pass_b<HD, MODE>(sQ, sdO, fk, fv, sLse + h * R, sDelta + h * R, sM + (size_t)h * R * 8, kt, nqt, h, a.drop, key_rng, 0u, L,
                           c, g, tk, tv);
#pragma unroll
      for (int nt = 0; nt < NT; ++nt)
#pragma unroll
        for (int r = 0; r < 4; ++r) {
          dk.kb[(h * NT + nt) >> 1][4 * ((h * NT + nt) & 1) + r] = (__bf16)(validB ? tk[nt][r] * ln2 : 0.f);
          dv.kb[(h * NT + nt) >> 1][4 * ((h * NT + nt) & 1) + r] = (__bf16)(validB ? tv[nt][r] : 0.f);
        }
    }
  }
  if constexpr (HD == 16) a1req = tt_saved_request(a.xin, rowA, validA, g, 1);
  XM_STAMP(6);
  adt_wait_vm0();
  __syncthreads();
  XM_STAMP(7);
  TT da1 = tt_zero();
  const TTSaved oreq = tt_saved_request(a.o, rowA, validA, g, 1);
  const TT fx = tt_load(a.f + rowB * 64, validB, g);
  if (has) {
    xm_put_rows(img0, lA, dq);
    tt_put_rows(img1, lA, tt_saved_value(a1req, 1), validA, g);
    da1 = tt_gemm(dq, wimg, c, g);
  }
  __syncthreads();
  sb_dw_product16<NW>(img0, img1, npair, nullptr, a.part[0] + (size_t)blockIdx.x * a.part_stride, sRed, w, c, g);
  __syncthreads();
  XM_STAMP(8);
  const TT acc1v = tt_load(a.out1 + rowB * 64, validB && a.acc1, g);
  if (has) {
    tt_put_rows(img0, lA, da1, validA, g);
    tt_put_rows(img1, lA, tt_saved_value(oreq, 1), validA, g);
    tt_store(a.out0 + rowA * 64, tt_gemm(tt_bfrags(da1), wimg + TT_WIMG, c, g), validA, g);
  }
  __syncthreads();
  sb_dw_product16<NW>(img0, img1, npair, nullptr, a.part[1] + (size_t)blockIdx.x * a.part_stride, sRed + 64, w, c, g);
  __syncthreads();
  XM_STAMP(9);
  TT df = tt_zero();
  if (has) {
    xm_put_rows(img0, lB, dk);
    tt_put_rows(img1, lB, fx, validB, g);
    df = tt_gemm(dk, wimg + 2 * TT_WIMG, c, g);
  }
  __syncthreads();
  sb_dw_product16<NW>(img0, img1, npair, nullptr, a.part[2] + (size_t)blockIdx.x * a.part_stride, sRed + 128, w, c, g);
  __syncthreads();
  XM_STAMP(10);
  if (has) {
    xm_put_rows(img0, lB, dv);
    tt_add(df, tt_gemm(dv, wimg + 3 * TT_WIMG, c, g));
    tt_add(df, acc1v);
    tt_store(a.out1 + rowB * 64, df, validB, g);
  }
  __syncthreads();
  sb_dw_product16<NW>(img0, img1, npair, nullptr, a.part[3] + (size_t)blockIdx.x * a.part_stride, sRed + 192, w, c, g);
  __syncthreads();
  XM_STAMP(11);
  {
    const int t = threadIdx.x;
    float* const dst[4] = {a.db0, a.db1, a.db2, a.db3};
    if (t < 256) {
      if (a.vpart) a.vpart[(size_t)blockIdx.x * 512 + t] = sRed[t];
      else atomicAdd(dst[t >> 6] + (t & 63), sRed[t]);
    }
  }
  XM_STAMP(12);
#undef XM_STAMP
}

}
```

adt_amd/csrc/adt_step_plan.h:

```cpp
#pragma once
#include <stddef.h>
#include <stdio.h>
#include "../../include/adt_hip.h"
#include "adt_bwd_plan.h"
#include "adt_wide_plan.h"

constexpr int ADT_SEQ_MAXLEN = 224;

struct SeqSwitches {
  bool seq = true;
  bool seq_lean = true;
  bool seq_tt = true;
  bool seq_bwd = true;
  bool seq_attn_bwd = true;
  bool seq_post_bwd = true;
  bool seq_partials = true;
  bool xattn_fused = true;
  int seq_ablate = 0;
  bool seq_ablate_set = false;
  int seq_split = 0;
  bool attn_split = true;
  int side_stream = 7;
  bool side_stream_dp = false;
  bool item_sort = false;
  bool lnl_fused = true;
  bool fold_parts = true;
  bool fwd_fused = true;
  bool embed3 = true;
  bool bce_merged = true;
};

constexpr bool adt_seq_head_ok(int hd) { return hd == 16 || hd == 32 || hd == 64; }

struct SeqAttnFacts {
  int L, H, B;
  bool causal, in_bf16, out_bf16;
  int ldq, ldk, ldv, ldo, lddo;
  bool dropout, keep_bits;
  size_t sab_lds, xm_lds;
};
struct SeqChainFacts {
  int L, H, B, T;
  bool wimg;
  bool saved_bf16, grad_bf16, parts4;
  int nsplit, ablate;
  bool drec;
};

static inline bool adt_covers_attn_bwd(const SeqSwitches& sw, int hd, const SeqAttnFacts& a) {
  if (!sw.seq_attn_bwd || !a.causal || a.H * hd != 64 || a.L > ADT_SEQ_MAXLEN) return false;
  if ((a.ldq % 4) || (a.ldk % 4) || (a.ldv % 4) || (a.ldo % 4)) return false;
  if (a.in_bf16 && ((a.ldq % 8) || (a.ldk % 8) || (a.ldv % 8) || (a.ldo % 8))) return false;
  return a.sab_lds <= ADT_LDS_MAX && adt_seq_head_ok(hd);
}
static inline bool adt_covers_attn_pre_bwd(const SeqSwitches& sw, int hd, const SeqChainFacts& a) {
  return sw.seq_bwd && a.wimg && a.L <= ADT_SEQ_MAXLEN && (a.L & 3) == 0 && a.H * hd == 64 && adt_seq_head_ok(hd);
}
static inline bool adt_covers_mid_bwd(const SeqSwitches& sw, int hd, const SeqChainFacts& a) {
  return sw.seq_post_bwd && a.wimg && a.L <= ADT_SEQ_MAXLEN && a.T == a.B * a.L && adt_seq_head_ok(hd);
}
static inline bool adt_covers_post_bwd(const SeqSwitches& sw, int hd, bool enc, const SeqChainFacts& a) {
  return adt_covers_mid_bwd(sw, hd, a) && !(enc && a.drec && a.H * hd != 64);
}
static inline bool adt_covers_xattn_mid(const SeqSwitches& sw, int hd, const SeqAttnFacts& at, const SeqChainFacts& ch, bool handover) {
  if (!sw.xattn_fused || !adt_covers_mid_bwd(sw, hd, ch)) return false;
  if (!at.in_bf16 || !at.out_bf16 || !ch.saved_bf16 || !ch.grad_bf16 || !ch.parts4) return false;
  if (ch.nsplit > 1 || ch.ablate) return false;
  if (!at.causal || at.H * hd != 64 || (at.L & 3) || at.L > ADT_SEQ_MAXLEN || at.L != ch.L || at.B != ch.B) return false;
  if (at.dropout && !at.keep_bits) return false;
  if ((at.ldq % 8) || (at.ldk % 8) || (at.ldv % 8) || (at.ldo % 8) || (at.lddo % 4)) return false;
  return handover && at.xm_lds <= ADT_LDS_MAX;
}
static inline bool adt_seq_fwd_tt(const SeqSwitches& sw, bool wimg, int L) { return sw.seq_tt && wimg && (L & 3) == 0; }

struct StepFacts {
  int prec, L, d, H, num_layers, B;
  int rows;
  bool item_sort_ok;
  size_t sab_lds;
};

struct StepPlan {
  char cfg_error[96];
  bool use_seq;
  bool lean;
  bool parts;
  bool fold_parts;
  bool parts_area, sort_area;
  bool det;
  bool embed3_on;
  bool lnl_fused;
  bool bce_deferred;
  bool bce_merged;
  int seq_split;
  int attn_split;
  int side_sites;
  bool side_dp;
  bool loss_one_launch;
};

static inline StepPlan adt_step_plan(const StepFacts& f, const SeqSwitches& sw) {
  StepPlan p{};
  const int nl = f.num_layers;
  const int hd = (f.H >= 1 && f.d % f.H == 0) ? f.d / f.H : 0;
  if (f.d != 64) snprintf(p.cfg_error, sizeof p.cfg_error, "sasrec: hidden=%d unsupported in this build (64)", f.d);
  else if (hd == 0) snprintf(p.cfg_error, sizeof p.cfg_error, "sasrec: bad num_heads");
  else if (!adt_seq_head_ok(hd)) snprintf(p.cfg_error, sizeof p.cfg_error, "sasrec: head_dim=%d unsupported (16/32/64)", hd);
  else if (f.L > ADT_SEQ_MAXLEN) snprintf(p.cfg_error, sizeof p.cfg_error, "sasrec: maxlen=%d > %d unsupported", f.L, ADT_SEQ_MAXLEN);
  else if (nl < 1 || nl > 16) snprintf(p.cfg_error, sizeof p.cfg_error, "sasrec: num_layers");

  const bool bf16 = f.prec == ADT_PREC_BF16;
  p.use_seq = sw.seq && bf16 && f.d == 64 && f.L <= ADT_SEQ_MAXLEN && adt_seq_head_ok(hd);
  p.lean = sw.seq_lean && sw.seq_tt && sw.seq_bwd && sw.seq_attn_bwd && !sw.seq_ablate_set && p.use_seq && (f.L & 3) == 0 &&
           f.sab_lds <= ADT_LDS_MAX;
  p.parts = sw.seq_partials && sw.seq_post_bwd && p.lean;
  p.fold_parts = sw.fold_parts && nl <= 2 && p.parts;
  p.parts_area = bf16 && f.d == 64;
  p.sort_area = f.d == 64 && f.item_sort_ok;
  p.det = sw.item_sort && p.sort_area;
  p.embed3_on = sw.embed3 && !p.det && f.d == 64;
  p.lnl_fused = p.parts && sw.lnl_fused;
  p.bce_deferred = sw.fwd_fused && f.d == 64 && nl <= 4 && p.lean;
  p.bce_merged = sw.bce_merged;
  p.seq_split = 1;
  if (sw.seq_split > 0) p.seq_split = sw.seq_split;
  else while (p.seq_split < 8 && f.B * p.seq_split * 2 <= 256) p.seq_split *= 2;
  p.attn_split = sw.attn_split && p.seq_split >= 2 ? 2 : 1;
  p.side_sites = sw.side_stream & 7;
  p.side_dp = sw.side_stream_dp;
  p.loss_one_launch = nl <= 4;
  return p;
}

struct BwdCallPlan {
  bool late_parts;
  bool embed3;
  bool side;
};
static inline BwdCallPlan adt_bwd_call_plan(const StepPlan& s, const BwdPlan& b) {
  BwdCallPlan p;
  p.late_parts = b.defer_fold && s.fold_parts;
  p.embed3 = b.seeds_virtual && s.embed3_on;
  p.side = s.side_sites != 0 && (b.phase == 0 || s.side_dp);
  return p;
}
```

adt_amd/csrc/adt_tt.cuh:

```cuda
#pragma once
#include "adt_attn_bf16.cuh"
#include "adt_wave.cuh"

namespace adt {

struct TT { f32x4 v[4]; };

constexpr int TT_RS = 72;
constexpr int TT_WIMG = 64 * TT_RS;

ADT_DEVICE_INLINE bf16x8 tt_pack(const f32x4& lo, const f32x4& hi, float mul = 1.0f) {
  bf16x8 o;
#pragma unroll
  for (int j = 0; j < 4; ++j) { o[j] = (__bf16)(lo[j] * mul); o[4 + j] = (__bf16)(hi[j] * mul); }
  return o;
}

struct TTB { bf16x8 kb[2]; };

ADT_DEVICE_INLINE TTB tt_bfrags(const TT& x, float mul = 1.0f) {
  TTB b;
  b.kb[0] = tt_pack(x.v[0], x.v[1], mul);
  b.kb[1] = tt_pack(x.v[2], x.v[3], mul);
  return b;
}

ADT_DEVICE_INLINE TT tt_gemm(const TTB& b, const __bf16* img, int c, int g) {
  int opaque_zero = 0;
  asm volatile("" : "+v"(opaque_zero));
  img += opaque_zero;
  TT y;
#pragma unroll
  for (int nt = 0; nt < 4; ++nt) {
    f32x4 acc = {0.f, 0.f, 0.f, 0.f};
#pragma unroll
    for (int kb = 0; kb < 2; ++kb)
      acc = mfma_bf16(acc, *reinterpret_cast<const bf16x8*>(img + (16 * nt + c) * TT_RS + 32 * kb + 8 * g), b.kb[kb]);
    y.v[nt] = acc;
  }
  return y;
}

struct TTV { f32x4 v[4]; };
ADT_DEVICE_INLINE TTV tt_vec(const float* p, int g) {
  TTV t;
#pragma unroll
  for (int nt = 0; nt < 4; ++nt) {
    const float4 x = *reinterpret_cast<const float4*>(p + 16 * nt + 4 * g);
    t.v[nt] = f32x4{x.x, x.y, x.z, x.w};
  }
  return t;
}
ADT_DEVICE_INLINE void tt_add_vec(TT& t, const float* p, int g) {
#pragma unroll
  for (int nt = 0; nt < 4; ++nt) {
    const float4 x = *reinterpret_cast<const float4*>(p + 16 * nt + 4 * g);
    t.v[nt] += f32x4{x.x, x.y, x.z, x.w};
  }
}
ADT_DEVICE_INLINE void tt_add(TT& a, const TT& b) {
#pragma unroll
  for (int nt = 0; nt < 4; ++nt) a.v[nt] += b.v[nt];
}
ADT_DEVICE_INLINE TT tt_zero() {
  TT t;
#pragma unroll
  for (int nt = 0; nt < 4; ++nt) t.v[nt] = f32x4{0.f, 0.f, 0.f, 0.f};
  return t;
}

static __device__ __attribute__((aligned(256))) const float tt_zero_row[64] = {};
ADT_DEVICE_INLINE int tt_load_id(const int* ids, int row, bool valid) {
  typedef const int __attribute__((address_space(1))) * gi;
  return *(valid ? (gi)(ids + row) : (gi)tt_zero_row);
}
ADT_DEVICE_INLINE TT tt_load(const float* row, bool valid, int g) {
  TT t;
  typedef const f32x4 __attribute__((address_space(1))) * gp4;
  const gp4 p = valid ? (gp4)(row + 4 * g) : (gp4)(tt_zero_row + 4 * g);
#pragma unroll
  for (int nt = 0; nt < 4; ++nt) t.v[nt] = p[4 * nt];
  return t;
}
ADT_DEVICE_INLINE TT tt_load_if(const float* row, bool valid, int g) {
  TT t;
#pragma unroll
  for (int nt = 0; nt < 4; ++nt) {
    float4 x = make_float4(0.f, 0.f, 0.f, 0.f);
    if (valid) x = *reinterpret_cast<const float4*>(row + 16 * nt + 4 * g);
    t.v[nt] = f32x4{x.x, x.y, x.z, x.w};
  }
  return t;
}
ADT_DEVICE_INLINE void tt_store(float* row, const TT& t, bool valid, int g) {
  if (!valid) return;
#pragma unroll
  for (int nt = 0; nt < 4; ++nt) *reinterpret_cast<float4*>(row + 16 * nt + 4 * g) = make_float4(t.v[nt][0], t.v[nt][1], t.v[nt][2], t.v[nt][3]);
}

ADT_DEVICE_INLINE void tt_store_bf16(__bf16* row, const TT& t, bool valid, int g) {
  if (!valid) return;
  *reinterpret_cast<bf16x8*>(row + 16 * g) = tt_pack(t.v[0], t.v[1]);
  *reinterpret_cast<bf16x8*>(row + 16 * g + 8) = tt_pack(t.v[2], t.v[3]);
}
ADT_DEVICE_INLINE TT tt_load_bf16(const __bf16* row, bool valid, int g) {
  TT t;
  typedef const bf16x8 __attribute__((address_space(1))) * gp8;
  const gp8 p = valid ? (gp8)(row + 16 * g) : (gp8)(tt_zero_row + 8 * g);
  const bf16x8 lo = p[0], hi = p[1];
#pragma unroll
  for (int r = 0; r < 4; ++r) { t.v[0][r] = (float)lo[r]; t.v[1][r] = (float)lo[4 + r]; t.v[2][r] = (float)hi[r]; t.v[3][r] = (float)hi[4 + r]; }
  return t;
}

ADT_DEVICE_INLINE void tt_save(float* buf, size_t row, const TT& t, bool valid, int g, int as_bf16) {
  if (!buf) return;
  if (as_bf16) tt_store_bf16(reinterpret_cast<__bf16*>(buf) + row * 64, t, valid, g);
  else tt_store(buf + row * 64, t, valid, g);
}
typedef unsigned tt_u4 __attribute__((ext_vector_type(4)));
struct TTSaved { tt_u4 q[4]; };
ADT_DEVICE_INLINE TTSaved tt_saved_request(const float* buf, size_t row, bool valid, int g, int as_bf16) {
  typedef const tt_u4 __attribute__((address_space(1))) * gq;
  TTSaved r;
  if (as_bf16) {
    const gq p = valid ? (gq)(reinterpret_cast<const __bf16*>(buf) + row * 64 + 16 * g) : (gq)tt_zero_row;
    r.q[0] = p[0]; r.q[1] = p[1];
    r.q[2] = r.q[3] = tt_u4{0u, 0u, 0u, 0u};
  } else {
    const gq p = valid ? (gq)(buf + row * 64 + 4 * g) : (gq)(tt_zero_row + 4 * g);
#pragma unroll
    for (int nt = 0; nt < 4; ++nt) r.q[nt] = p[4 * nt];
  }
  return r;
}
ADT_DEVICE_INLINE TT tt_saved_value(TTSaved r, int as_bf16) {
  uint32_t w0 = r.q[0].x, w1 = r.q[0].y, w2 = r.q[0].z, w3 = r.q[0].w, w4 = r.q[1].x, w5 = r.q[1].y, w6 = r.q[1].z, w7 = r.q[1].w;
  asm volatile("" : "+v"(w0), "+v"(w1), "+v"(w2), "+v"(w3), "+v"(w4), "+v"(w5), "+v"(w6), "+v"(w7));
  TT t;
  if (as_bf16) {
    union { tt_u4 u; bf16x8 b; } lo, hi;
    lo.u = tt_u4{w0, w1, w2, w3}; hi.u = tt_u4{w4, w5, w6, w7};
#pragma unroll
    for (int e = 0; e < 4; ++e) { t.v[0][e] = (float)lo.b[e]; t.v[1][e] = (float)lo.b[4 + e]; t.v[2][e] = (float)hi.b[e]; t.v[3][e] = (float)hi.b[4 + e]; }
  } else {
    t.v[0] = f32x4{__uint_as_float(w0), __uint_as_float(w1), __uint_as_float(w2), __uint_as_float(w3)};
    t.v[1] = f32x4{__uint_as_float(w4), __uint_as_float(w5), __uint_as_float(w6), __uint_as_float(w7)};
#pragma unroll
    for (int nt = 2; nt < 4; ++nt)
      t.v[nt] = f32x4{__uint_as_float(r.q[nt].x), __uint_as_float(r.q[nt].y), __uint_as_float(r.q[nt].z), __uint_as_float(r.q[nt].w)};
  }
  return t;
}
ADT_DEVICE_INLINE TT tt_load_saved_if(const float* buf, size_t row, bool valid, int g, int as_bf16) {
  if (as_bf16) {
    TT t = tt_zero();
    if (valid) {
      const __bf16* r = reinterpret_cast<const __bf16*>(buf) + row * 64;
      const bf16x8 lo = *reinterpret_cast<const bf16x8*>(r + 16 * g), hi = *reinterpret_cast<const bf16x8*>(r + 16 * g + 8);
#pragma unroll
      for (int e = 0; e < 4; ++e) { t.v[0][e] = (float)lo[e]; t.v[1][e] = (float)lo[4 + e]; t.v[2][e] = (float)hi[e]; t.v[3][e] = (float)hi[4 + e]; }
    }
    return t;
  }
  return tt_load_if(buf + row * 64, valid, g);
}
ADT_DEVICE_INLINE TT tt_load_saved(const float* buf, size_t row, bool valid, int g, int as_bf16) {
  if (as_bf16) return tt_load_bf16(reinterpret_cast<const __bf16*>(buf) + row * 64, valid, g);
  return tt_load(buf + row * 64, valid, g);
}

typedef unsigned tt_u2 __attribute__((ext_vector_type(2)));
ADT_DEVICE_INLINE unsigned tt_xor16u(unsigned u) {
  const tt_u2 r = __builtin_amdgcn_permlane16_swap(u, u, false, false);
  return (threadIdx.x & 16) ? r[0] : r[1];
}
ADT_DEVICE_INLINE unsigned tt_xor32u(unsigned u) {
  const tt_u2 r = __builtin_amdgcn_permlane32_swap(u, u, false, false);
  return (threadIdx.x & 32) ? r[0] : r[1];
}
ADT_DEVICE_INLINE float tt_xor16(float v) { return __uint_as_float(tt_xor16u(__float_as_uint(v))); }
ADT_DEVICE_INLINE float tt_xor32(float v) { return __uint_as_float(tt_xor32u(__float_as_uint(v))); }

ADT_DEVICE_INLINE float tt_colsum(float v) {
  v += tt_xor16(v);
  v += tt_xor32(v);
  return v;
}
ADT_DEVICE_INLINE float tt_colmax(float v) {
  v = fmaxf(v, tt_xor16(v));
  v = fmaxf(v, tt_xor32(v));
  return v;
}
ADT_DEVICE_INLINE uint32_t tt_color(uint32_t v) {
  v |= tt_xor16u(v);
  v |= tt_xor32u(v);
  return v;
}

ADT_DEVICE_INLINE float tt_rowsum16(float v) {
  v += __builtin_bit_cast(float, __builtin_amdgcn_mov_dpp(__builtin_bit_cast(int, v), 0xB1, 0xF, 0xF, true));
  v += __builtin_bit_cast(float, __builtin_amdgcn_mov_dpp(__builtin_bit_cast(int, v), 0x4E, 0xF, 0xF, true));
  v += __builtin_bit_cast(float, __builtin_amdgcn_mov_dpp(__builtin_bit_cast(int, v), 0x141, 0xF, 0xF, true));
  v += __builtin_bit_cast(float, __builtin_amdgcn_mov_dpp(__builtin_bit_cast(int, v), 0x140, 0xF, 0xF, true));
  return v;
}

template <int NTHREADS>
ADT_DEVICE_INLINE void tt_stage_vec(float* dst, const float* src, int n) {
  if (src == nullptr) return;
  for (int i = threadIdx.x; i < n; i += NTHREADS) dst[i] = src[i];
}

ADT_DEVICE_INLINE TT tt_layernorm(const TT& x, const float* gamma, const float* beta, float eps, int g) {
  float s = 0.f;
#pragma unroll
  for (int nt = 0; nt < 4; ++nt) s += (x.v[nt][0] + x.v[nt][1]) + (x.v[nt][2] + x.v[nt][3]);
  const float mu = tt_colsum(s) * (1.0f / 64);
  TT d;
  float q = 0.f;
#pragma unroll
  for (int nt = 0; nt < 4; ++nt)
#pragma unroll
    for (int r = 0; r < 4; ++r) { const float t = x.v[nt][r] - mu; d.v[nt][r] = t; q += t * t; }
  const float rstd = 1.0f / sqrtf(tt_colsum(q) * (1.0f / 64) + eps);
  const TTV gm = tt_vec(gamma, g), bt = tt_vec(beta, g);
#pragma unroll
  for (int nt = 0; nt < 4; ++nt)
#pragma unroll
    for (int r = 0; r < 4; ++r) d.v[nt][r] = d.v[nt][r] * rstd * gm.v[nt][r] + bt.v[nt][r];
  return d;
}

ADT_DEVICE_INLINE void tt_dropout(TT& t, uint32_t key, const DropCfg& d, uint32_t row_global, int g) {
  if (!d.thr) return;
#pragma unroll
  for (int nt = 0; nt < 4; ++nt) {
    const uint32_t bits = adt_keep4(key, row_global * 64u + (uint32_t)(16 * nt + 4 * g), d.thr);
#pragma unroll
    for (int r = 0; r < 4; ++r) t.v[nt][r] = ((bits >> r) & 1u) ? t.v[nt][r] * d.scale : 0.f;
  }
}

ADT_DEVICE_INLINE void tt_put_slot(__bf16* img, int token, const TT& t, bool valid, int g) {
#pragma unroll
  for (int nt = 0; nt < 4; ++nt) {
    bf16x4 b;
#pragma unroll
    for (int r = 0; r < 4; ++r) b[r] = (__bf16)(valid ? t.v[nt][r] : 0.f);
    *reinterpret_cast<bf16x4*>(img + token * TT_RS + 32 * (nt >> 1) + 8 * g + 4 * (nt & 1)) = b;
  }
}
ADT_DEVICE_INLINE void tt_put_rows(__bf16* img, int token, const TT& t, bool valid, int g) {
#pragma unroll
  for (int nt = 0; nt < 4; ++nt) {
    bf16x4 b;
#pragma unroll
    for (int r = 0; r < 4; ++r) b[r] = (__bf16)(valid ? t.v[nt][r] : 0.f);
    *reinterpret_cast<bf16x4*>(img + token * TT_RS + 16 * nt + 4 * g) = b;
  }
}

typedef short tt_s4 __attribute__((ext_vector_type(4)));
ADT_DEVICE_INLINE bf16x8 tt_trfrag(const __bf16* img, int row0, int col0, int c, int g) {
  const __bf16* p = img + (row0 + 4 * g + (c >> 2)) * TT_RS + col0 + 4 * (c & 3);
  const tt_s4 lo = __builtin_amdgcn_ds_read_tr16_b64_v4i16((tt_s4 __attribute__((address_space(3)))*)(p));
  const tt_s4 hi = __builtin_amdgcn_ds_read_tr16_b64_v4i16((tt_s4 __attribute__((address_space(3)))*)(p + 16 * TT_RS));
  union { struct { tt_s4 a, b; } s; bf16x8 v; } u;
  u.s.a = lo; u.s.b = hi;
  return u.v;
}

ADT_DEVICE_INLINE float tt_max3(float a, float b, float c) {
  float r;
  asm("v_max3_f32 %0, %1, %2, %3" : "=v"(r) : "v"(a), "v"(b), "v"(c));
  return r;
}
ADT_DEVICE_INLINE float tt_max_quad(float m, const f32x4& acc) { return tt_max3(m, fmaxf(acc[0], acc[1]), fmaxf(acc[2], acc[3])); }
template <int POS>
ADT_DEVICE_INLINE float tt_keep_if_bit(float x, uint32_t k) {
  float r;
  asm("v_bfe_i32 %0, %1, %3, 1\n\tv_and_b32 %0, %0, %2" : "=&v"(r) : "v"(k), "v"(x), "n"(POS));
// ... 225 lines not shown
```

Baseline: 430,100 sequences/s.

## Hand dO over as pre-scaled bf16 rows with precomputed delta to attention backward

```diff
diff --git a/adt_amd/csrc/adt_attn_args.h b/adt_amd/csrc/adt_attn_args.h
--- a/adt_amd/csrc/adt_attn_args.h
+++ b/adt_amd/csrc/adt_attn_args.h
@@ -22,6 +22,7 @@
   unsigned long long* stamps;
   int in_bf16;
   int out_bf16;
+  const void* do_bf16; const float* do_delta;
 };
 
 }
diff --git a/adt_amd/csrc/adt_bwdchain_args.h b/adt_amd/csrc/adt_bwdchain_args.h
--- a/adt_amd/csrc/adt_bwdchain_args.h
+++ b/adt_amd/csrc/adt_bwdchain_args.h
@@ -34,6 +34,7 @@
   const float* wp_base; const void* wp_img;
   float* vpart;
   const float* lnl_x; const float* lnl_gamma; float lnl_eps; float* vpart2; float* lnl_dgamma; float* lnl_dbeta;
+  void* do_bf16; float* do_delta; float do_scale; int do_hd;
   int nsplit;
 };
 
diff --git a/adt_amd/csrc/adt_sasrec.hip b/adt_amd/csrc/adt_sasrec.hip
--- a/adt_amd/csrc/adt_sasrec.hip
+++ b/adt_amd/csrc/adt_sasrec.hip
@@ -70,6 +70,7 @@
   int64_t wpack;
   int64_t part, part_stride;
   int64_t isort, isort_n;
+  int64_t dodelta;
   int64_t vpart, vcall, lnpart, gnpart;
   int64_t total;
 };
@@ -119,6 +120,7 @@
   w->vpart = take(w->part_stride > 0 ? (5 * w->nl + 1) * w->vcall : 0);
   w->lnpart = take(LN_PART_BLOCKS * 128);
   w->gnpart = take(4096);
+  w->dodelta = take(pl.do_handover ? up64(w->T * 4) : 0);
   w->total = o;
 }
 
@@ -472,6 +474,10 @@
   int64_t Td, recsz;
   float* Gq;
   float *s1, *s3, *s4, *s5, *gf;
+  void* do_rows() const { return sp.do_handover ? (void*)s3 : nullptr; }
+  void* do_rows_cross() const { return sp.do_handover ? (void*)s1 : nullptr; }
+  float* do_delta() const { return sp.do_handover ? ws + w.dodelta : nullptr; }
+  float do_scale(uint32_t site) const { return adt_make_drop(p, seed, site).scale; }
   const float* f;
   SideStream *sd, *sd_sort;
 
@@ -564,6 +570,7 @@
   a.dW0 = Gq + lo.dec(i, D_C2W); a.dW1 = Gq + lo.dec(i, D_C1W); a.dW2 = Gq + lo.dec(i, D_EOW);
   a.db0 = Gq + lo.dec(i, D_C2B); a.db1 = Gq + lo.dec(i, D_C1B); a.db2 = Gq + lo.dec(i, D_EOB);
   a.out0 = x.s1;
+  a.do_bf16 = x.do_rows_cross(); a.do_delta = x.do_delta(); a.do_scale = x.do_scale(dec_site(i, 1)); a.do_hd = x.hd;
   a.part[0] = x.PART(i, PS_D_C2); a.part[1] = x.PART(i, PS_D_C1); a.part[2] = x.PART(i, PS_D_EO); a.part_stride = (size_t)w.part_stride;
   a.vpart = x.VPART(i, 0);
   const int rc = x.sp.use_seq ? adt_launch_seq_post_bwd(x.hd, 0, a, x.st) : 1;
@@ -571,6 +578,8 @@
   if (rc && x.sp.parts) return adt_set_error(NO_FALLBACK, x.L, x.hd);
   return rc ? adt_launch_bwdchain(x.prec, 1, a, x.st) : 0;
 }
+
+adt::AttnArgs dec_cross_attn_lean_args(const Bwd& x, int i);
 
 int dec_cross_attn_bwd(const Bwd& x, int i) {
   const WS& w = x.w; const int d = x.d, B = (int)w.B;
@@ -580,6 +589,10 @@
   if (!x.sp.lean)
     return adt_attn_bwd(x.prec, q2, d, kv2, 2 * d, kv2 + d, 2 * d, o2, d, lse2, x.s1, d, B, x.H, x.L, x.hd, 1, x.p, x.seed, dec_site(i, 1), x.b_offset,
                         x.s5, d, s4, 2 * d, s4 + d, 2 * d, mask2, x.st);
+  if (x.sp.do_handover) {
+    const int rc = adt_launch_seq_attn_bwd(x.hd, dec_cross_attn_lean_args(x, i), x.st);
+    return rc == 1 ? adt_set_error(NO_FALLBACK, x.L, x.hd) : rc;
+  }
   const uint16_t* kvb = reinterpret_cast<const uint16_t*>(kv2);
   return adt_attn_bwd_saved_bf16(q2, d, kvb, 2 * d, kvb + d, 2 * d, o2, d, lse2, x.s1, d, B, x.H, x.L, x.hd, x.p, x.seed, dec_site(i, 1), x.b_offset,
                                  x.s5, d, s4, 2 * d, x.sp.parts ? s4 + d / 2 : s4 + d, 2 * d, mask2, x.sp.parts ? 1 : 0, x.st);
@@ -602,6 +615,7 @@
   a.part[0] = x.PART(i, PS_D_EIN); a.part[1] = x.PART(i, PS_D_SO); a.part[2] = x.PART(i, PS_D_EIN + 1); a.part[3] = x.PART(i, PS_D_EIN + 2);
   a.part_stride = (size_t)w.part_stride;
   a.vpart = x.VPART(i, 1);
+  a.do_bf16 = x.do_rows(); a.do_delta = x.do_delta(); a.do_scale = x.do_scale(dec_site(i, 0)); a.do_hd = x.hd;
   return a;
 }
 
@@ -609,9 +623,11 @@
   const WS& w = x.w; const int d = x.d;
   float* base = x.ws + i * w.d_stride;
   const uint16_t* kvb = reinterpret_cast<const uint16_t*>(base + w.d_kv2);
-  return adt_attn_bwd_saved_bf16_args(base + w.d_q2, d, kvb, 2 * d, kvb + d, 2 * d, base + w.d_o2, d, base + w.d_lse2, x.s1, d, (int)w.B, x.H, x.L, x.hd, x.p,
-                                      x.seed, dec_site(i, 1), x.b_offset, x.s5, d, x.s4, 2 * d, x.s4 + d / 2, 2 * d,
-                                      reinterpret_cast<const uint32_t*>(base + w.d_mask2), 1);
+  adt::AttnArgs a = adt_attn_bwd_saved_bf16_args(base + w.d_q2, d, kvb, 2 * d, kvb + d, 2 * d, base + w.d_o2, d, base + w.d_lse2, x.s1, d, (int)w.B, x.H, x.L,
+                                                 x.hd, x.p, x.seed, dec_site(i, 1), x.b_offset, x.s5, d, x.s4, 2 * d, x.s4 + d / 2, 2 * d,
+                                                 reinterpret_cast<const uint32_t*>(base + w.d_mask2), 1);
+  a.do_bf16 = x.do_rows_cross(); a.do_delta = x.do_delta();
+  return a;
 }
 
 int dec_mid_bwd(const Bwd& x, int i) {
@@ -661,6 +677,7 @@
     adt::SeqBwdArgs a = seq_bwd_args(x.L, (int)w.B, x.H, ids, x.p, x.seed, site, x.b_offset, x.hd);
     a.x = xi; a.gamma = P + lnw; a.beta = P + lnb; a.Win = P + inw; a.bin = P + inb;
     a.dO = x.s1; a.o = o; a.lse = lse; a.mask = mask; a.dres = dec ? gy : x.s5;
+    a.do_bf16 = x.do_rows(); a.do_delta = x.do_delta();
     a.gx = gx; a.acc = acc; a.dWin = Gq + inw; a.dbin = Gq + inb; a.dgamma = Gq + lnw; a.dbeta = Gq + lnb;
     if (x.plan.seeds_virtual && dec && i > 0) {
       a.acc = 0; a.seed_other = ws + w.enc_x + (nl - i) * x.Td; a.seed_coef = ws + w.norms + 8 + (nl - i);
@@ -679,6 +696,7 @@
     if (rc <= 0) return rc;
     if (x.sp.lean) return adt_set_error("backward: the lean forward needs the fused attention-block backward (L=%d hd=%d)", x.L, x.hd);
   }
+  if (x.sp.do_handover) return adt_set_error("backward: the staged attention backward was reached with the dO hand-over on (L=%d hd=%d)", x.L, x.hd);
   CK(adt_attn_bwd(x.prec, qkv, 3 * d, qkv + d, 3 * d, qkv + 2 * d, 3 * d, o, d, lse, x.s1, d, (int)w.B, x.H, x.L, x.hd, 1, x.p, x.seed, site, x.b_offset,
                   x.s3, 3 * d, x.s3 + d, 3 * d, x.s3 + 2 * d, 3 * d, mask, x.st));
   adt::BwdChainArgs a = x.BA(ids, 0.f, nullptr);
@@ -791,6 +809,7 @@
   }
   a.part[0] = x.PART(i, PS_E_C2); a.part[1] = x.PART(i, PS_E_C1); a.part[2] = x.PART(i, PS_E_O); a.part_stride = (size_t)w.part_stride;
   a.vpart = x.VPART(i, 3);
+  a.do_bf16 = x.do_rows(); a.do_delta = x.do_delta(); a.do_scale = x.do_scale(enc_site(i, 0)); a.do_hd = x.hd;
   if (x.sp.lnl_fused && i == nl - 1) {
     a.gy = x.gf; a.lnl_x = ws + w.enc_x + nl * x.Td; a.lnl_gamma = P + lo.lnl_w(); a.lnl_eps = LN_EPS;
     a.vpart2 = x.call.late_parts ? ws + w.vpart + (int64_t)(5 * nl) * w.vcall : nullptr;
diff --git a/adt_amd/csrc/adt_seq.hip b/adt_amd/csrc/adt_seq.hip
--- a/adt_amd/csrc/adt_seq.hip
+++ b/adt_amd/csrc/adt_seq.hip
@@ -34,7 +34,7 @@
     SeqSwitches s;
     s.seq = adt_env_on("ADT_SEQ"); s.seq_lean = adt_env_on("ADT_SEQ_LEAN"); s.seq_tt = adt_env_on("ADT_SEQ_TT"); s.seq_bwd = adt_env_on("ADT_SEQ_BWD");
     s.seq_attn_bwd = adt_env_on("ADT_SEQ_ATTN_BWD"); s.seq_post_bwd = adt_env_on("ADT_SEQ_POST_BWD"); s.seq_partials = adt_env_on("ADT_SEQ_PARTIALS");
-    s.xattn_fused = adt_env_on("ADT_XATTN_FUSED");
+    s.xattn_fused = adt_env_on("ADT_XATTN_FUSED"); s.do_bf16 = adt_env_on("ADT_DO_BF16");
     s.seq_ablate = adt_env_int("ADT_SEQ_ABLATE", 0); s.seq_ablate_set = adt_env_int("ADT_SEQ_ABLATE", INT_MIN) != INT_MIN;
     s.seq_split = adt_env_int("ADT_SEQ_SPLIT", 0); s.attn_split = adt_env_on("ADT_ATTN_SPLIT");
     s.side_stream = adt_env_int("ADT_SIDE_STREAM", 7); s.side_stream_dp = adt_env_int("ADT_SIDE_STREAM_DP", 0) != 0;
@@ -126,8 +126,12 @@
   return adt_set_error("seq_dec_fwd: head size %d", hd);
 }
 
+static std::atomic<unsigned long long> g_do_handover_launches{0};
+extern "C" unsigned long long adt_seq_do_handover_launches() { return g_do_handover_launches.load(); }
+
 int adt_launch_seq_attn_bwd(int hd, const AttnArgs& a, void* stream) {
   if (!adt_covers_attn_bwd(adt_seq_switches(), hd, attn_facts(a))) return 1;
+  if (a.do_bf16 && (!a.do_delta || !a.in_bf16)) return adt_set_error("seq_attn_bwd: handed-over dO rows need their delta and bf16 operand rows");
   const size_t smem = sab_lds_bytes(a.L, a.H);
   const int mode = a.drop.thr == 0 ? 0 : (a.mask != nullptr ? 1 : 2);
   static AdtLdsOptIn optin[9];
@@ -138,7 +142,9 @@
   AttnArgs args = a;
   args.stamps = seq_stamp_buffer(true);
   if (!args.stamps) args.stamps = seq_stamp_buffer_mode(4);
-  return adt_launch_lds1(fns[slot], dim3(a.B), dim3(SAB_NW * 64), smem, args, (hipStream_t)stream, "seq_attn_bwd", optin[slot], ADT_LDS_MAX);
+  const int rc = adt_launch_lds1(fns[slot], dim3(a.B), dim3(SAB_NW * 64), smem, args, (hipStream_t)stream, "seq_attn_bwd", optin[slot], ADT_LDS_MAX);
+  if (rc == 0 && a.do_bf16) ++g_do_handover_launches;
+  return rc;
 }
 
 template <int HD, bool DEC>
@@ -152,13 +158,16 @@
   args.stamps = seq_stamp_buffer(true);
   if (a.nsplit == 2 && !a.part) return adt_set_error("seqtt_attn_pre_bwd: two workgroups per sequence need the weight-gradient partials");
   if (a.nsplit != 2) args.nsplit = 1;
-  return seq_launch(fns[mode], smem, optin[mode], a.B * args.nsplit, &args, s, "seqtt_attn_pre_bwd");
+  const int rc = seq_launch(fns[mode], smem, optin[mode], a.B * args.nsplit, &args, s, "seqtt_attn_pre_bwd");
+  if (rc == 0 && a.do_bf16) ++g_do_handover_launches;
+  return rc;
 }
 
 int adt_launch_seq_attn_pre_bwd(int hd, int dec, const SeqBwdArgs& a, void* stream) {
   SeqChainFacts f{};
   f.L = a.L; f.H = a.H; f.B = a.B; f.T = a.B * a.L; f.wimg = a.wp_img != nullptr;
   if (!adt_covers_attn_pre_bwd(adt_seq_switches(), hd, f)) return 1;
+  if (a.do_bf16 && !a.do_delta) return adt_set_error("seqtt_attn_pre_bwd: handed-over dO rows without their delta");
   const int mode = a.drop.thr == 0 ? 0 : (a.mask != nullptr ? 1 : 2);
   hipStream_t s = (hipStream_t)stream;
   if (hd == 32) return dec ? seq_attn_pre_bwd_t<32, true>(mode, a, s) : seq_attn_pre_bwd_t<32, false>(mode, a, s);
@@ -206,6 +215,9 @@
   a.db0 = ch.db0; a.db1 = ch.db1; a.db2 = ch.db2; a.db3 = ch.db3; a.vpart = ch.vpart;
   for (int k = 0; k < 4; ++k) a.part[k] = ch.part[k];
   a.part_stride = ch.part_stride;
+  a.do_bf16 = ch.do_bf16; a.do_delta = ch.do_delta; a.do_scale = ch.do_scale;
+  a.dO_bf16 = reinterpret_cast<const __bf16*>(at.do_bf16); a.dO_delta = at.do_delta;
+  if (at.do_bf16 && !at.do_delta) return adt_set_error("seqtt_xattn_mid_bwd: handed-over dO rows without their delta");
   a.stamps = seq_stamp_buffer_mode(6);
   const int mode = at.drop.thr == 0 ? 0 : 1;
   static AdtLdsOptIn optin[6];
@@ -215,6 +227,7 @@
   const size_t most = xm_lds_bytes(ADT_SEQ_MAXLEN, at.H) <= ADT_LDS_MAX ? xm_lds_bytes(ADT_SEQ_MAXLEN, at.H) : xm_lds_bytes(128, at.H);
   const int rc = seq_launch(fns[slot], xm_lds_bytes(at.L, at.H), optin[slot], at.B, &a, (hipStream_t)stream, "seqtt_xattn_mid_bwd", XM_NW, most);
   if (rc == 0) ++g_xattn_fused_launches;
+  if (rc == 0 && at.do_bf16) ++g_do_handover_launches;
   return rc;
 }
 
diff --git a/adt_amd/csrc/adt_seqattn.cuh b/adt_amd/csrc/adt_seqattn.cuh
--- a/adt_amd/csrc/adt_seqattn.cuh
+++ b/adt_amd/csrc/adt_seqattn.cuh
@@ -219,6 +219,8 @@
   for (int i = threadIdx.x; i < R * 8; i += NW * 64) {
     const int r = i >> 3, c8 = (i & 7) * 8;
     float q[8], k[8], v[8], d[8], o[8];
+    float dlt = 0.f;
+    const bool hand = a.in_bf16 && a.do_bf16 != nullptr;
 #pragma unroll
     for (int j = 0; j < 8; ++j) q[j] = k[j] = v[j] = d[j] = o[j] = 0.f;
     if (r < L && a.in_bf16) {
@@ -229,12 +231,22 @@
       const bf16x4_t qa = *reinterpret_cast<const bf16x4_t*>(Qb + (row_b + r) * a.ldq + pa), qc = *reinterpret_cast<const bf16x4_t*>(Qb + (row_b + r) * a.ldq + pb);
       const bf16x4_t ka = *reinterpret_cast<const bf16x4_t*>(Kb + (row_b + r) * a.ldk + pa), kc = *reinterpret_cast<const bf16x4_t*>(Kb + (row_b + r) * a.ldk + pb);
       const bf16x4_t va = *reinterpret_cast<const bf16x4_t*>(Vb + (row_b + r) * a.ldv + pa), vc = *reinterpret_cast<const bf16x4_t*>(Vb + (row_b + r) * a.ldv + pb);
-      const bf16x4_t oa = *reinterpret_cast<const bf16x4_t*>(Ob + (row_b + r) * a.ldo + pa), oc = *reinterpret_cast<const bf16x4_t*>(Ob + (row_b + r) * a.ldo + pb);
       bf16x8 qb, kb, vb, ob;
 #pragma unroll
-      for (int j = 0; j < 4; ++j) { qb[j] = qa[j]; qb[4 + j] = qc[j]; kb[j] = ka[j]; kb[4 + j] = kc[j]; vb[j] = va[j]; vb[4 + j] = vc[j]; ob[j] = oa[j]; ob[4 + j] = oc[j]; }
-      *reinterpret_cast<float4*>(d) = *reinterpret_cast<const float4*>(a.dO + (row_b + r) * a.lddo + c8);
-      *reinterpret_cast<float4*>(d + 4) = *reinterpret_cast<const float4*>(a.dO + (row_b + r) * a.lddo + c8 + 4);
+      for (int j = 0; j < 4; ++j) { qb[j] = qa[j]; qb[4 + j] = qc[j]; kb[j] = ka[j]; kb[4 + j] = kc[j]; vb[j] = va[j]; vb[4 + j] = vc[j]; ob[j] = (__bf16)0.f; ob[4 + j] = (__bf16)0.f; }
+      if (hand) {
+        const __bf16* Db = reinterpret_cast<const __bf16*>(a.do_bf16) + (row_b + r) * 64;
+        const bf16x4_t da = *reinterpret_cast<const bf16x4_t*>(Db + pa), dc = *reinterpret_cast<const bf16x4_t*>(Db + pb);
+#pragma unroll
+        for (int j = 0; j < 4; ++j) { d[j] = (float)da[j]; d[4 + j] = (float)dc[j]; }
+        dlt = a.do_delta[(row_b + r) * 4 + (i & 7) / (HD / 8)];
+      } else {
+        const bf16x4_t oa = *reinterpret_cast<const bf16x4_t*>(Ob + (row_b + r) * a.ldo + pa), oc = *reinterpret_cast<const bf16x4_t*>(Ob + (row_b + r) * a.ldo + pb);
+#pragma unroll
+        for (int j = 0; j < 4; ++j) { ob[j] = oa[j]; ob[4 + j] = oc[j]; }
+        *reinterpret_cast<float4*>(d) = *reinterpret_cast<const float4*>(a.dO + (row_b + r) * a.lddo + c8);
+        *reinterpret_cast<float4*>(d + 4) = *reinterpret_cast<const float4*>(a.dO + (row_b + r) * a.lddo + c8 + 4);
+      }
 #pragma unroll
       for (int j = 0; j < 8; ++j) { q[j] = (float)qb[j]; k[j] = (float)kb[j]; v[j] = (float)vb[j]; o[j] = (float)ob[j]; }
     } else if (r < L) {
@@ -249,15 +261,17 @@
       *reinterpret_cast<float4*>(o) = *reinterpret_cast<const float4*>(a.O + (row_b + r) * a.ldo + c8);
       *reinterpret_cast<float4*>(o + 4) = *reinterpret_cast<const float4*>(a.O + (row_b + r) * a.ldo + c8 + 4);
     }
-    float part = 0.f;
-#pragma unroll
-    for (int j = 0; j < 8; ++j) { part += d[j] * o[j]; q[j] *= qmul; d[j] *= a.drop.scale; }
+    float part = hand ? dlt : tt_chunk_delta(d, o);
+#pragma unroll
+    for (int j = 0; j < 8; ++j) { q[j] *= qmul; if (!hand) d[j] *= a.drop.scale; }
     *reinterpret_cast<bf16x8*>(sQ + r * TT_RS + c8) = pack8(q);
     *reinterpret_cast<bf16x8*>(sK + r * TT_RS + c8) = pack8(k);
     *reinterpret_cast<bf16x8*>(sV + r * TT_RS + c8) = pack8(v);
     *reinterpret_cast<bf16x8*>(sdO + r * TT_RS + c8) = pack8(d);
-#pragma unroll
-    for (int off = HD / 16; off > 0; off >>= 1) part += __shfl_xor(part, off, 64);
+    if (!hand) {
+#pragma unroll
+      for (int off = HD / 16; off > 0; off >>= 1) part += __shfl_xor(part, off, 64);
+    }
     if (((i & 7) % (HD / 8)) == 0) sDelta[((i & 7) / (HD / 8)) * R + r] = part;
   }
   SAB_STAMP(1);
diff --git a/adt_amd/csrc/adt_seqbwd_args.h b/adt_amd/csrc/adt_seqbwd_args.h
--- a/adt_amd/csrc/adt_seqbwd_args.h
+++ b/adt_amd/csrc/adt_seqbwd_args.h
@@ -12,6 +12,7 @@
   const float* gamma; const float* beta;
   const float* Win; const float* bin;
   const float* dO; const float* o;
+  const void* do_bf16; const float* do_delta;
   const float* lse; const uint32_t* mask;
   float dres_scale;
   const float* dres;
diff --git a/adt_amd/csrc/adt_seqbwd_tt.cuh b/adt_amd/csrc/adt_seqbwd_tt.cuh
--- a/adt_amd/csrc/adt_seqbwd_tt.cuh
+++ b/adt_amd/csrc/adt_seqbwd_tt.cuh
@@ -27,6 +27,19 @@
     const f32x4 z = {0.f, 0.f, 0.f, 0.f};
 #pragma unroll
     for (int h = 0; h < 4; ++h) f[h] = tt_pack(t.v[h], z, mul);
+  }
+}
+
+template <int HD>
+ADT_DEVICE_INLINE void sb_frags_rows(const TTRowB& t, bf16x8 (&f)[(64 / HD) * ((HD + 31) / 32)]) {
+  if constexpr (HD >= 32) {
+    f[0] = t.lo;
+    f[1] = t.hi;
+  } else {
+#pragma unroll
+    for (int h = 0; h < 4; ++h)
+#pragma unroll
+      for (int j = 0; j < 4; ++j) { f[h][j] = (h < 2 ? t.lo : t.hi)[4 * (h & 1) + j]; f[h][4 + j] = (__bf16)0.f; }
   }
 }
 
@@ -263,6 +276,9 @@
 #pragma unroll
   for (int k = 0; k < 3; ++k) adt_glds_block<NW>(src6[k], wpl + k * TT_WIMG, TT_WIMG * 2);
   TT xa[2], doa[2], oa[2];
+  TTRowB dob[2];
+  float delta[2][H];
+  const bool hand = a.do_bf16 != nullptr;
   int idv[2] = {1, 1};
 #pragma unroll
   for (int s = 0; s < 2; ++s) {
@@ -299,15 +315,19 @@
     const int tile = TM(s);
     const int l = tile * 16 + c, row = b * L + l;
     const bool valid = tile >= 0 && l < L;
-    doa[s] = tt_load(a.dO + (size_t)row * 64, valid, g);
-    oa[s] = tt_load_saved(a.o, row, valid, g, a.saved_bf16);
+    if (hand) {
+      dob[s] = tt_load_bf16_raw(reinterpret_cast<const __bf16*>(a.do_bf16) + (size_t)row * 64, valid, g);
+      tt_delta_load<H>(a.do_delta, (size_t)row, valid, delta[s]);
+    } else {
+      doa[s] = tt_load(a.dO + (size_t)row * 64, valid, g);
+      oa[s] = tt_load_saved(a.o, row, valid, g, a.saved_bf16);
+    }
   }
 #pragma unroll
   for (int k = 3; k < 6; ++k) adt_glds_block<NW>(src6[k], wtr + (k - 3) * TT_WIMG, TT_WIMG * 2);
   const float qmul = a.scale * 1.4426950408889634f;
   const uint32_t key_rng = drop_key(a.drop);
   bf16x8 fq[2][NF], fdo[2][NF];
-  float delta[2][H];
 #pragma unroll
   for (int s = 0; s < 2; ++s) {
     const int tile = TM(s);
@@ -328,19 +348,15 @@
     TT v = tt_gemm(DEC ? bn : bx, wpl + 2 * TT_WIMG, c, g);
     tt_add_vec(v, vbin + 128, g);
     tt_put_rows(img1, l, v, valid, g);
-    const TT& dO = doa[s];
-    const TT& o = oa[s];
-    sb_frags<HD>(dO, a.drop.scale, fdo[s]);
-#pragma unroll
-    for (int h = 0; h < H; ++h) {
-      float part = 0.f;
-#pragma unroll
-      for (int nt = 0; nt < NT; ++nt)
-#pragma unroll
-        for (int r = 0; r < 4; ++r) part += dO.v[h * NT + nt][r] * o.v[h * NT + nt][r];
-      delta[s][h] = tt_colsum(part);
+    if (hand) {
+      sb_frags_rows<HD>(dob[s], fdo[s]);
+    } else {
+      sb_frags<HD>(doa[s], a.drop.scale, fdo[s]);
+      tt_head_delta<HD>(doa[s], oa[s], delta[s]);
+    }
+#pragma unroll
+    for (int h = 0; h < H; ++h)
       if (g == 0 && valid) sDelta[h * R + l] = delta[s][h];
-    }
   }
   __syncthreads();
   SB_STAMP(2);
diff --git a/adt_amd/csrc/adt_seqpost_tt.cuh b/adt_amd/csrc/adt_seqpost_tt.cuh
--- a/adt_amd/csrc/adt_seqpost_tt.cuh
+++ b/adt_amd/csrc/adt_seqpost_tt.cuh
@@ -33,6 +33,20 @@
   constexpr size_t ibytes = (size_t)SB_R * TT_RS * 2;
   uint4* z = reinterpret_cast<uint4*>(img0);
   for (int i = threadIdx.x; i < (int)((2 * ibytes + 64) / 16); i += NW * 64) z[i] = make_uint4(0u, 0u, 0u, 0u);
+}
+template <int HD, bool CHUNKS = false>
+ADT_DEVICE_INLINE void sp_hand_do(void* do_bf16, float* do_delta, float scale, size_t row, const TT& dO, const TT& o, bool valid, int g) {
+  float dl[64 / HD];
+  if constexpr (CHUNKS) tt_head_delta_chunks<HD>(dO, o, dl);
+  else tt_head_delta<HD>(dO, o, dl);
+  tt_store_bf16(reinterpret_cast<__bf16*>(do_bf16) + row * 64, dO, valid, g, scale);
+  tt_delta_store<64 / HD>(do_delta, row, dl, valid, g, CHUNKS ? 1 : 0);
+}
+ADT_DEVICE_INLINE void sp_store_do1(float* out0, void* do_bf16, float* do_delta, float scale, int hd, size_t row, const TT& dO, const TT& o, bool valid, int g) {
+  if (!do_bf16) { tt_store(out0 + row * 64, dO, valid, g); return; }
+  if (hd == 32) sp_hand_do<32>(do_bf16, do_delta, scale, row, dO, o, valid, g);
+  else if (hd == 64) sp_hand_do<64>(do_bf16, do_delta, scale, row, dO, o, valid, g);
+  else sp_hand_do<16>(do_bf16, do_delta, scale, row, dO, o, valid, g);
 }
 constexpr int SP_NW = 8;
 constexpr int SP_NS = (14 + SP_NW - 1) / SP_NW;
@@ -236,7 +250,11 @@
         }
       }
     }
-    tt_store((ENC ? a.out1 : a.out0) + (size_t)row * 64, dO, valid, g);
+    if (a.do_bf16) {
+      sp_hand_do<HD, !ENC>(a.do_bf16, a.do_delta, a.do_scale, (size_t)row, dO, oraw_s, valid, g);
+    } else {
+      tt_store((ENC ? a.out1 : a.out0) + (size_t)row * 64, dO, valid, g);
+    }
   }
   SB_STAMP(12);
   __syncthreads();
@@ -357,8 +375,9 @@
     dk[s] = a.grad_bf16 ? tt_load_bf16(reinterpret_cast<const __bf16*>(a.dkv2) + (size_t)row * 128, valid, g) : tt_load(a.dkv2 + (size_t)row * 128, valid, g);
     fx[s] = tt_load(a.f + (size_t)row * 64, valid, g);
     tt_put_rows(img0, l, da1[s], valid, g);
-    tt_put_rows(img1, l, tt_saved_value(oreq[s], a.saved_bf16), valid, g);
-    tt_store(a.out0 + (size_t)row * 64, tt_gemm(tt_bfrags(da1[s]), wimg + TT_WIMG, c, g), valid, g);
+    const TT o1 = tt_saved_value(oreq[s], a.saved_bf16);
+    tt_put_rows(img1, l, o1, valid, g);
+    sp_store_do1(a.out0, a.do_bf16, a.do_delta, a.do_scale, a.do_hd, (size_t)row, tt_gemm(tt_bfrags(da1[s]), wimg + TT_WIMG, c, g), o1, valid, g);
   }
   __syncthreads();
   sb_dw_product16<NW>(img0, img1, npair, a.dW1, a.part[1] ? a.part[1] + (size_t)blockIdx.x * a.part_stride : nullptr, sRed + 64, w, c, g);
diff --git a/adt_amd/csrc/adt_seqxattn_tt.cuh b/adt_amd/csrc/adt_seqxattn_tt.cuh
--- a/adt_amd/csrc/adt_seqxattn_tt.cuh
+++ b/adt_amd/csrc/adt_seqxattn_tt.cuh
@@ -15,6 +15,8 @@
   float* out0; float* out1; int acc1; int nrep; size_t rep_stride;
   float* db0; float* db1; float* db2; float* db3; float* vpart;
   float* part[4]; size_t part_stride;
+  void* do_bf16; float* do_delta; float do_scale;
+  const __bf16* dO_bf16; const float* dO_delta;
   unsigned long long* stamps;
 };
 
@@ -97,8 +99,10 @@
     const float v = *(ok ? (gf1)(a.LSE + (size_t)(b * H + h) * L + r) : (gf1)tt_zero_row);
     lreg[k] = ok ? v * 1.4426950408889634f : INFINITY;
   });
-  bf16x4 qa[II], qc[II], ka[II], kc[II], va[II], vc[II], oa[II], oc[II];
+  bf16x4 qa[II], qc[II], ka[II], kc[II], va[II], vc[II], oa[II], oc[II], da[II], dc[II];
   f32x4 d0[II], d1[II];
+  float dlt[II];
+  const bool hand = a.dO_bf16 != nullptr;
   adt_static_for<II>([&](auto k) {
     const int i = threadIdx.x + k * NTH, r = i >> 3, c8 = (i & 7) * 8;
     const bool ok = r < L;
@@ -107,9 +111,16 @@
     const gb4 zb = (gb4)tt_zero_row + (i & 7);
     const gb4 pq = ok ? (gb4)(a.Q + row * a.ldq + pa) : zb, pk = ok ? (gb4)(a.K + row * a.ldk + pa) : zb;
     const gb4 pv = ok ? (gb4)(a.V + row * a.ldv + pa) : zb, po = ok ? (gb4)(a.O + row * a.ldo + pa) : zb;
-    const gp4 pd = ok ? (gp4)(a.dO + row * a.lddo + c8) : (gp4)tt_zero_row + (i & 7);
-    qa[k] = pq[0]; qc[k] = pq[4]; ka[k] = pk[0]; kc[k] = pk[4]; va[k] = pv[0]; vc[k] = pv[4]; oa[k] = po[0]; oc[k] = po[4];
-    d0[k] = pd[0]; d1[k] = pd[1];
+    qa[k] = pq[0]; qc[k] = pq[4]; ka[k] = pk[0]; kc[k] = pk[4]; va[k] = pv[0]; vc[k] = pv[4];
+    if (hand) {
+      const gb4 pdb = ok ? (gb4)(a.dO_bf16 + row * 64 + pa) : zb;
+      da[k] = pdb[0]; dc[k] = pdb[4];
+      dlt[k] = *(ok ? (gf1)(a.dO_delta + row * 4 + (i & 7) / (HD / 8)) : (gf1)tt_zero_row);
+    } else {
+      const gp4 pd = ok ? (gp4)(a.dO + row * a.lddo + c8) : (gp4)tt_zero_row + (i & 7);
+      oa[k] = po[0]; oc[k] = po[4];
+      d0[k] = pd[0]; d1[k] = pd[1];
+    }
   });
   XM_STAMP(1);
   if constexpr (MODE == 1) {
@@ -125,25 +136,38 @@
   if (threadIdx.x < 256) sRed[threadIdx.x] = 0.f;
   adt_static_for<II>([&](auto k) {
     const int i = threadIdx.x + k * NTH, r = i >> 3, c8 = (i & 7) * 8;
-    float q[8], kk[8], v[8], d[8], o[8];
+    float q[8], kk[8], v[8];
 #pragma unroll
     for (int j = 0; j < 4; ++j) {
       q[j] = (float)qa[k][j]; q[4 + j] = (float)qc[k][j]; kk[j] = (float)ka[k][j]; kk[4 + j] = (float)kc[k][j];
-      v[j] = (float)va[k][j]; v[4 + j] = (float)vc[k][j]; o[j] = (float)oa[k][j]; o[4 + j] = (float)oc[k][j];
-      d[j] = d0[k][j]; d[4 + j] = d1[k][j];
-    }
-    float part = 0.f;
-#pragma unroll
-    for (int j = 0; j < 8; ++j) { part += d[j] * o[j]; q[j] *= qmul; d[j] *= a.drop.scale; }
+      v[j] = (float)va[k][j]; v[4 + j] = (float)vc[k][j];
+    }
+#pragma unroll
+    for (int j = 0; j < 8; ++j) q[j] *= qmul;
     const bool in = i < R * 8;
     if (in) {
       *reinterpret_cast<bf16x8*>(sQ + r * TT_RS + c8) = pack8(q);
       *reinterpret_cast<bf16x8*>(sK + r * TT_RS + c8) = pack8(kk);
       *reinterpret_cast<bf16x8*>(sV + r * TT_RS + c8) = pack8(v);
-      *reinterpret_cast<bf16x8*>(sdO + r * TT_RS + c8) = pack8(d);
-    }
-#pragma unroll
-    for (int off = HD / 16; off > 0; off >>= 1) part += __shfl_xor(part, off, 64);
+    }
+    float part;
+    if (hand) {
+      bf16x8 db;
+#pragma unroll
+      for (int j = 0; j < 4; ++j) { db[j] = da[k][j]; db[4 + j] = dc[k][j]; }
+      if (in) *reinterpret_cast<bf16x8*>(sdO + r * TT_RS + c8) = db;
+      part = dlt[k];
+    } else {
+      float d[8], o[8];
+#pragma unroll
+      for (int j = 0; j < 4; ++j) { o[j] = (float)oa[k][j]; o[4 + j] = (float)oc[k][j]; d[j] = d0[k][j]; d[4 + j] = d1[k][j]; }
+      part = tt_chunk_delta(d, o);
+#pragma unroll
+      for (int j = 0; j < 8; ++j) d[j] *= a.drop.scale;
+      if (in) *reinterpret_cast<bf16x8*>(sdO + r * TT_RS + c8) = pack8(d);
+#pragma unroll
+      for (int off = HD / 16; off > 0; off >>= 1) part += __shfl_xor(part, off, 64);
+    }
     if (in && ((i & 7) % (HD / 8)) == 0) sDelta[((i & 7) / (HD / 8)) * R + r] = part;
   });
   XM_STAMP(2);
@@ -242,8 +266,9 @@
   const TT acc1v = tt_load(a.out1 + rowB * 64, validB && a.acc1, g);
   if (has) {
     tt_put_rows(img0, lA, da1, validA, g);
-    tt_put_rows(img1, lA, tt_saved_value(oreq, 1), validA, g);
-    tt_store(a.out0 + rowA * 64, tt_gemm(tt_bfrags(da1), wimg + TT_WIMG, c, g), validA, g);
+    const TT o1 = tt_saved_value(oreq, 1);
+    tt_put_rows(img1, lA, o1, validA, g);
+    sp_store_do1(a.out0, a.do_bf16, a.do_delta, a.do_scale, HD, rowA, tt_gemm(tt_bfrags(da1), wimg + TT_WIMG, c, g), o1, validA, g);
   }
   __syncthreads();
   sb_dw_product16<NW>(img0, img1, npair, nullptr, a.part[1] + (size_t)blockIdx.x * a.part_stride, sRed + 64, w, c, g);
diff --git a/adt_amd/csrc/adt_step_plan.h b/adt_amd/csrc/adt_step_plan.h
--- a/adt_amd/csrc/adt_step_plan.h
+++ b/adt_amd/csrc/adt_step_plan.h
@@ -28,6 +28,7 @@
   bool fwd_fused = true;
   bool embed3 = true;
   bool bce_merged = true;
+  bool do_bf16{true};
 };
 
 constexpr bool adt_seq_head_ok(int hd) { return hd == 16 || hd == 32 || hd == 64; }
@@ -97,6 +98,7 @@
   int side_sites;
   bool side_dp;
   bool loss_one_launch;
+  bool do_handover;
 };
 
 static inline StepPlan adt_step_plan(const StepFacts& f, const SeqSwitches& sw) {
@@ -129,6 +131,7 @@
   p.side_sites = sw.side_stream & 7;
   p.side_dp = sw.side_stream_dp;
   p.loss_one_launch = nl <= 4;
+  p.do_handover = sw.do_bf16 && p.parts;
   return p;
 }
 
diff --git a/adt_amd/csrc/adt_tt.cuh b/adt_amd/csrc/adt_tt.cuh
--- a/adt_amd/csrc/adt_tt.cuh
+++ b/adt_amd/csrc/adt_tt.cuh
@@ -98,10 +98,10 @@
   for (int nt = 0; nt < 4; ++nt) *reinterpret_cast<float4*>(row + 16 * nt + 4 * g) = make_float4(t.v[nt][0], t.v[nt][1], t.v[nt][2], t.v[nt][3]);
 }
 
-ADT_DEVICE_INLINE void tt_store_bf16(__bf16* row, const TT& t, bool valid, int g) {
+ADT_DEVICE_INLINE void tt_store_bf16(__bf16* row, const TT& t, bool valid, int g, float mul = 1.0f) {
   if (!valid) return;
-  *reinterpret_cast<bf16x8*>(row + 16 * g) = tt_pack(t.v[0], t.v[1]);
-  *reinterpret_cast<bf16x8*>(row + 16 * g + 8) = tt_pack(t.v[2], t.v[3]);
+  *reinterpret_cast<bf16x8*>(row + 16 * g) = tt_pack(t.v[0], t.v[1], mul);
+  *reinterpret_cast<bf16x8*>(row + 16 * g + 8) = tt_pack(t.v[2], t.v[3], mul);
 }
 ADT_DEVICE_INLINE TT tt_load_bf16(const __bf16* row, bool valid, int g) {
   TT t;
@@ -198,6 +198,82 @@
   return v;
 }
 
+template <int HD> constexpr int TT_DELTA_FUSED = HD == 64 ? 6 : (HD == 32 ? 8 : 12);
+ADT_DEVICE_INLINE float tt_mul_then_add(float acc, float a, float b) {
+#pragma clang fp contract(off)
+  const float p = a * b;
+  return acc + p;
+}
+template <int HD>
+ADT_DEVICE_INLINE void tt_head_delta(const TT& dO, const TT& o, float (&delta)[64 / HD]) {
+  constexpr int H = 64 / HD, NT = HD / 16;
+#pragma unroll
+  for (int h = 0; h < H; ++h) {
+    float part = 0.f;
+#pragma unroll
+    for (int nt = 0; nt < NT; ++nt)
+#pragma unroll
+      for (int r = 0; r < 4; ++r) {
+        const float d = dO.v[h * NT + nt][r], x = o.v[h * NT + nt][r];
+        part = 4 * (h * NT + nt) + r < TT_DELTA_FUSED<HD> ? __builtin_fmaf(d, x, part) : tt_mul_then_add(part, d, x);
+      }
+    delta[h] = tt_colsum(part);
+  }
+}
+ADT_DEVICE_INLINE float tt_chunk_fma4(float part, const float* d, const float* o) {
+#pragma unroll
+  for (int j = 0; j < 4; ++j) part = __builtin_fmaf(d[j], o[j], part);
+  return part;
+}
+ADT_DEVICE_INLINE float tt_chunk_delta(const float (&d)[8], const float (&o)[8]) { return tt_chunk_fma4(tt_chunk_fma4(0.f, d, o), d + 4, o + 4); }
+template <int HD>
+ADT_DEVICE_INLINE void tt_head_delta_chunks(const TT& dO, const TT& o, float (&delta)[64 / HD]) {
+  constexpr int H = 64 / HD, NT = HD / 16;
+  float p[4];
+#pragma unroll
+  for (int nt = 0; nt < 4; ++nt) {
+    const float d4[4] = {dO.v[nt][0], dO.v[nt][1], dO.v[nt][2], dO.v[nt][3]}, o4[4] = {o.v[nt][0], o.v[nt][1], o.v[nt][2], o.v[nt][3]};
+    p[nt] = tt_chunk_fma4(tt_xor16(tt_chunk_fma4(0.f, d4, o4)), d4, o4);
+  }
+#pragma unroll
+  for (int h = 0; h < H; ++h) {
+#pragma unroll
+    for (int off = NT / 2; off > 0; off >>= 1)
+#pragma unroll
+      for (int nt = 0; nt < off; ++nt) p[h * NT + nt] += p[h * NT + nt + off];
+    delta[h] = p[h * NT] + tt_xor32(p[h * NT]);
+  }
+}
+template <int H>
+ADT_DEVICE_INLINE void tt_delta_store(float* delta, size_t row, const float (&d)[H], bool valid, int g, int gsrc = 0) {
+  if (!valid || g != gsrc) return;
+  float* p = delta + row * 4;
+  if constexpr (H == 4) *reinterpret_cast<float4*>(p) = make_float4(d[0], d[1], d[2], d[3]);
+  else if constexpr (H == 2) *reinterpret_cast<float2*>(p) = make_float2(d[0], d[1]);
+  else *p = d[0];
+}
+template <int H>
+ADT_DEVICE_INLINE void tt_delta_load(const float* delta, size_t row, bool valid, float (&d)[H]) {
+  typedef float tt_fH __attribute__((ext_vector_type(H == 1 ? 2 : H)));
+  if constexpr (H == 1) {
+    typedef const float __attribute__((address_space(1))) * gf1;
+    d[0] = *(valid ? (gf1)(delta + row * 4) : (gf1)tt_zero_row);
+  } else {
+    typedef const tt_fH __attribute__((address_space(1))) * gfh;
+    const tt_fH v = *(valid ? (gfh)(delta + row * 4) : (gfh)tt_zero_row);
+#pragma unroll
+    for (int h = 0; h < H; ++h) d[h] = v[h];
+  }
+}
+struct TTRowB { bf16x8 lo, hi; };
+ADT_DEVICE_INLINE TTRowB tt_load_bf16_raw(const __bf16* row, bool valid, int g) {
+  typedef const bf16x8 __attribute__((address_space(1))) * gp8;
+  const gp8 p = valid ? (gp8)(row + 16 * g) : (gp8)(tt_zero_row + 8 * g);
+  TTRowB t;
+  t.lo = p[0]; t.hi = p[1];
+  return t;
+}
+
 ADT_DEVICE_INLINE float tt_rowsum16(float v) {
   v += __builtin_bit_cast(float, __builtin_amdgcn_mov_dpp(__builtin_bit_cast(int, v), 0xB1, 0xF, 0xF, true));
   v += __builtin_bit_cast(float, __builtin_amdgcn_mov_dpp(__builtin_bit_cast(int, v), 0x4E, 0xF, 0xF, true));
```

New measurement: 438,300 sequences/s (median of 6 runs). 1.9% higher.
